# mrcabellom/InstantSfM

Hardware: AMD Instinct MI355X
Metric: LM-BA iterations/sec (+ final reprojection RMSE) (higher is better)
Workload: dtype f64

## Files before the change

include/insfm_ba_debug.h:

```cpp
#ifndef INSFM_BA_DEBUG_H
#define INSFM_BA_DEBUG_H

#include "insfm_ba.h"
#include "insfm_gp.h"

#ifdef __cplusplus
extern "C" {
#endif

int insfm_ba_debug_linearize(insfm_ba* h, const double* cam_params, const double* points);
int insfm_ba_debug_solve(insfm_ba* h, double f);
int64_t insfm_ba_debug_get(insfm_ba* h, int32_t which, double* host_out);
int insfm_ba_debug_time_kernel(insfm_ba* h, int32_t which, int32_t reps, double* us_per_launch);
int insfm_ba_debug_time_cgp(insfm_ba* h, int32_t reps, double* out);
int32_t insfm_ba_debug_stamps(insfm_ba* h, int64_t* host_out, int32_t max_steps);
int32_t insfm_ba_debug_clusters(const insfm_ba* h, int32_t* labels);
int64_t insfm_ba_nnzb(const insfm_ba* h);
int insfm_ba_debug_spd_inverse(int32_t m, const double* E, double* Einv, void* stream, int32_t reps,
                               double* us_per_inverse);

int insfm_gp_debug_linearize(insfm_ba* h, const double* positions, const double* points, const double* scales);
int64_t insfm_gp_debug_get_ds(insfm_ba* h, double* host_out);

int insfm_ba_cg_window(insfm_ba* h, void* ipc_handle);
int insfm_ba_cg_attach(insfm_ba* h, const void* handles);
int insfm_ba_cg_partition(const insfm_ba* h, int32_t* rows_begin_end);
int insfm_ba_debug_time_xchg(insfm_ba* h, int32_t reps, double* us);

#ifdef __cplusplus
}
#endif
#endif
```

instantsfm_amd/_capi.py:

```python
import ctypes
import os

_HERE = os.path.dirname(os.path.abspath(__file__))
LIB_PATH = os.path.join(_HERE, "_lib", "libinsfm_ba.so")

INSFM_BA_OK = 0
INSFM_BA_EINVAL = -22
INSFM_BA_ENOMEM = -12
INSFM_BA_EHIP = -100
INSFM_BA_ECOMM = -101
INSFM_BA_ESOLVER = -102

ALLREDUCE_FN = ctypes.CFUNCTYPE(ctypes.c_int, ctypes.c_void_p, ctypes.POINTER(ctypes.c_double), ctypes.c_int64)
ALLREDUCE_ASYNC_FN = ctypes.CFUNCTYPE(ctypes.c_int, ctypes.c_void_p, ctypes.POINTER(ctypes.c_double), ctypes.c_int64,
                                      ctypes.c_void_p)


class Desc(ctypes.Structure):
    _fields_ = [
        ("n_cams", ctypes.c_int32), ("n_points", ctypes.c_int32), ("n_obs", ctypes.c_int32),
        ("cam_model", ctypes.c_int32), ("optimize_poses", ctypes.c_int32), ("deterministic", ctypes.c_int32),
        ("huber_delta", ctypes.c_double),
        ("tr_radius", ctypes.c_double), ("tr_max", ctypes.c_double), ("tr_min", ctypes.c_double),
        ("tr_up", ctypes.c_double), ("tr_down", ctypes.c_double), ("tr_factor", ctypes.c_double),
        ("tr_high", ctypes.c_double), ("tr_low", ctypes.c_double),
        ("clamp_min", ctypes.c_double), ("clamp_max", ctypes.c_double),
        ("max_rejects", ctypes.c_int32), ("pcg_max_iter", ctypes.c_int32),
        ("pcg_tol", ctypes.c_double),
        ("world_size", ctypes.c_int32), ("rank", ctypes.c_int32),
        ("shard_point_begin", ctypes.c_int32), ("shard_point_end", ctypes.c_int32),
        ("allreduce", ALLREDUCE_FN), ("allreduce_ctx", ctypes.c_void_p),
        ("precond", ctypes.c_int32), ("cluster_size", ctypes.c_int32), ("schur_variant", ctypes.c_int32),
        ("allreduce_async", ALLREDUCE_ASYNC_FN), ("exchange_chunks", ctypes.c_int32),
    ]


class Stats(ctypes.Structure):
    _fields_ = [
        ("loss", ctypes.c_double), ("loss_before", ctypes.c_double), ("damping", ctypes.c_double),
        ("trials", ctypes.c_int32), ("rejects", ctypes.c_int32), ("pcg_iters_last", ctypes.c_int32),
        ("pcg_iters_total", ctypes.c_int32), ("solver_failed", ctypes.c_int32), ("cg_launches", ctypes.c_int32),
        ("time_ms", ctypes.c_double * 8), ("coarse_used", ctypes.c_int32),
    ]

    def as_dict(self):
        return dict(loss=self.loss, loss_before=self.loss_before, damping=self.damping, trials=self.trials,
                    rejects=self.rejects, pcg_iters=self.pcg_iters_last, pcg_total=self.pcg_iters_total,
                    failed=self.solver_failed, cg_launches=self.cg_launches, time_ms=list(self.time_ms),
                    coarse_used=self.coarse_used)


PUBLIC_SYMBOLS = ("insfm_build_info", "insfm_ba_default_desc", "insfm_ba_create", "insfm_ba_step", "insfm_ba_cost",
                  "insfm_ba_reset", "insfm_ba_destroy", "insfm_ba_last_error", "insfm_ba_exchange_count",
                  "insfm_ba_set_exchange", "insfm_ba_set_timing", "insfm_ba_release_cache",
                  "insfm_ba_set_ranks_per_device", "insfm_ba_cg_info", "insfm_ba_set_persistent_cg",
                  "insfm_ba_cg_fallbacks",
                  "insfm_gp_default_desc", "insfm_gp_create", "insfm_gp_step", "insfm_gp_cost",
                  "insfm_undistort", "insfm_filter_reproj_normalized", "insfm_filter_angle", "insfm_filter_tri_angle",
                  "insfm_filter_reproj_pixel", "insfm_reproj_candidates",
                  "insfm_tracks_establish", "insfm_covis_pairs", "insfm_pair_inliers")
DEBUG_SYMBOLS = ("insfm_ba_debug_linearize", "insfm_ba_debug_solve", "insfm_ba_debug_get", "insfm_ba_nnzb",
                 "insfm_ba_debug_time_kernel", "insfm_ba_debug_clusters", "insfm_ba_debug_spd_inverse",
                 "insfm_ba_debug_time_cgp", "insfm_ba_debug_stamps",
                 "insfm_gp_debug_linearize", "insfm_gp_debug_get_ds",
                 "insfm_ba_cg_window", "insfm_ba_cg_attach", "insfm_ba_cg_partition", "insfm_ba_debug_time_xchg")
SYMBOLS = PUBLIC_SYMBOLS + DEBUG_SYMBOLS

_lib = None


class BAError(RuntimeError):
    def __init__(self, code, msg):
        super().__init__(f"insfm_ba error {code}: {msg}")
        self.code = code


def build_info(L=None):
    L = L or load()
    L.insfm_build_info.argtypes = []
    L.insfm_build_info.restype = ctypes.c_char_p
    return L.insfm_build_info().decode()


def _check_provenance(L, path):
    from . import build as _b
    if not all(os.path.exists(p) for p in _b.SRCS + _b.HEADERS):
        return
    info = build_info(L)
    want = _b.source_hash()
    if f"src={want} " not in info + " ":
        raise RuntimeError(f"{path} was built from other sources ({info}; this tree hashes to src={want}): "
                           "rebuild it (python -c 'import __graft_entry__ as g; g.build()')")


def load(path=None):
    global _lib
    if _lib is not None:
        return _lib
    path = path or os.environ.get("INSFM_LIB") or LIB_PATH
    if not os.path.exists(path):
        raise RuntimeError(f"{path} not found: build the HIP extension first (python -c 'import __graft_entry__ as g; g.build()')")
    L = ctypes.CDLL(path)
    if not os.environ.get("INSFM_LIB"):
        _check_provenance(L, path)
    vp, dp = ctypes.c_void_p, ctypes.POINTER(ctypes.c_double)
    L.insfm_ba_default_desc.argtypes = [ctypes.POINTER(Desc)]
    L.insfm_ba_default_desc.restype = None
    L.insfm_ba_create.argtypes = [ctypes.POINTER(Desc), dp, ctypes.POINTER(ctypes.c_int32), ctypes.POINTER(ctypes.c_int32),
                                  dp, vp, ctypes.POINTER(vp)]
    L.insfm_ba_create.restype = ctypes.c_int
    L.insfm_ba_step.argtypes = [vp, vp, vp, ctypes.POINTER(Stats)]
    L.insfm_ba_step.restype = ctypes.c_int
    L.insfm_ba_cost.argtypes = [vp, vp, vp, dp, dp]
    L.insfm_ba_cost.restype = ctypes.c_int
    L.insfm_ba_reset.argtypes = [vp]
    L.insfm_ba_reset.restype = ctypes.c_int
    L.insfm_ba_destroy.argtypes = [vp]
    L.insfm_ba_destroy.restype = None
    L.insfm_ba_last_error.argtypes = [vp]
    L.insfm_ba_last_error.restype = ctypes.c_char_p
    L.insfm_ba_debug_linearize.argtypes = [vp, vp, vp]
    L.insfm_ba_debug_linearize.restype = ctypes.c_int
    L.insfm_ba_debug_solve.argtypes = [vp, ctypes.c_double]
    L.insfm_ba_debug_solve.restype = ctypes.c_int
    L.insfm_ba_debug_get.argtypes = [vp, ctypes.c_int32, dp]
    L.insfm_ba_debug_get.restype = ctypes.c_int64
    L.insfm_ba_nnzb.argtypes = [vp]
    L.insfm_ba_nnzb.restype = ctypes.c_int64
    L.insfm_ba_exchange_count.argtypes = [vp]
    L.insfm_ba_exchange_count.restype = ctypes.c_int64
    L.insfm_ba_set_exchange.argtypes = [vp, vp, ctypes.c_int64]
    L.insfm_ba_set_exchange.restype = ctypes.c_int
    L.insfm_ba_debug_time_kernel.argtypes = [vp, ctypes.c_int32, ctypes.c_int32, dp]
    L.insfm_ba_debug_time_kernel.restype = ctypes.c_int
    L.insfm_ba_debug_stamps.argtypes = [vp, ctypes.POINTER(ctypes.c_int64), ctypes.c_int32]
    L.insfm_ba_debug_stamps.restype = ctypes.c_int32
    L.insfm_ba_debug_time_cgp.argtypes = [vp, ctypes.c_int32, dp]
    L.insfm_ba_debug_time_cgp.restype = ctypes.c_int
    L.insfm_ba_set_timing.argtypes = [vp, ctypes.c_int32]
    L.insfm_ba_set_timing.restype = ctypes.c_int
    L.insfm_ba_debug_clusters.argtypes = [vp, ctypes.POINTER(ctypes.c_int32)]
    L.insfm_ba_debug_clusters.restype = ctypes.c_int32
    L.insfm_ba_debug_spd_inverse.argtypes = [ctypes.c_int32, vp, vp, vp, ctypes.c_int32, dp]
    L.insfm_ba_debug_spd_inverse.restype = ctypes.c_int
    L.insfm_ba_release_cache.argtypes = []
    L.insfm_ba_release_cache.restype = ctypes.c_int64
    L.insfm_ba_set_ranks_per_device.argtypes = [vp, ctypes.c_int32]
    L.insfm_ba_set_ranks_per_device.restype = ctypes.c_int
    L.insfm_ba_cg_info.argtypes = [vp, ctypes.POINTER(ctypes.c_int32)]
    L.insfm_ba_cg_info.restype = ctypes.c_int
    L.insfm_ba_set_persistent_cg.argtypes = [vp, ctypes.c_int32]
    L.insfm_ba_set_persistent_cg.restype = ctypes.c_int
    L.insfm_ba_cg_fallbacks.argtypes = [vp]
    L.insfm_ba_cg_fallbacks.restype = ctypes.c_int32
    L.insfm_ba_cg_window.argtypes = [vp, ctypes.c_char_p]
    L.insfm_ba_cg_window.restype = ctypes.c_int
    L.insfm_ba_cg_attach.argtypes = [vp, ctypes.c_char_p]
    L.insfm_ba_cg_attach.restype = ctypes.c_int
    L.insfm_ba_cg_partition.argtypes = [vp, ctypes.POINTER(ctypes.c_int32)]
    L.insfm_ba_cg_partition.restype = ctypes.c_int
    L.insfm_ba_debug_time_xchg.argtypes = [vp, ctypes.c_int32, dp]
    L.insfm_ba_debug_time_xchg.restype = ctypes.c_int
    ip = ctypes.POINTER(ctypes.c_int32)
    L.insfm_gp_default_desc.argtypes = [ctypes.POINTER(Desc)]
    L.insfm_gp_default_desc.restype = None
    L.insfm_gp_create.argtypes = [ctypes.POINTER(Desc), dp, ip, ip, dp, ip, vp, ctypes.POINTER(vp)]
    L.insfm_gp_create.restype = ctypes.c_int
    L.insfm_gp_step.argtypes = [vp, vp, vp, vp, ctypes.POINTER(Stats)]
    L.insfm_gp_step.restype = ctypes.c_int
    L.insfm_gp_cost.argtypes = [vp, vp, vp, vp, dp, dp]
    L.insfm_gp_cost.restype = ctypes.c_int
    L.insfm_gp_debug_linearize.argtypes = [vp, vp, vp, vp]
    L.insfm_gp_debug_linearize.restype = ctypes.c_int
    L.insfm_gp_debug_get_ds.argtypes = [vp, dp]
    L.insfm_gp_debug_get_ds.restype = ctypes.c_int64
    i64, f64, i32 = ctypes.c_int64, ctypes.c_double, ctypes.c_int32
    L.insfm_undistort.argtypes = [i64, vp, i32, vp, vp, vp, vp, vp]
    L.insfm_filter_reproj_normalized.argtypes = [i64, vp, vp, vp, vp, vp, vp, f64, vp, vp, vp]
    L.insfm_filter_angle.argtypes = [i64, vp, vp, vp, vp, vp, vp, f64, vp, vp]
    L.insfm_filter_tri_angle.argtypes = [i64, vp, vp, vp, vp, f64, vp, vp]
    L.insfm_filter_reproj_pixel.argtypes = [i64, vp, vp, vp, vp, i32, vp, vp, vp, vp, vp, f64, vp, vp, vp]
    L.insfm_reproj_candidates.argtypes = [i64, i32, vp, vp, vp, vp, i32, vp, vp, vp, f64, vp, vp, vp]
    L.insfm_tracks_establish.argtypes = [i64, vp, vp, i32, i64, vp, vp, f64, vp, vp, vp, vp, vp,
                                         ctypes.POINTER(ctypes.c_int64), vp]
    L.insfm_covis_pairs.argtypes = [i64, vp, vp, i32, i64, vp, vp, vp, vp, ctypes.POINTER(ctypes.c_int64), vp]
    L.insfm_covis_pairs.restype = ctypes.c_int
    L.insfm_pair_inliers.argtypes = [i64, vp, i64, vp, vp, i64, vp, i32, vp, i32, vp, vp, vp, vp, vp, vp, vp]
    L.insfm_pair_inliers.restype = ctypes.c_int
    for fn in ("insfm_tracks_establish", "insfm_undistort", "insfm_filter_reproj_normalized", "insfm_filter_angle", "insfm_filter_tri_angle",
               "insfm_filter_reproj_pixel", "insfm_reproj_candidates",
           "insfm_tracks_establish"):
        getattr(L, fn).restype = ctypes.c_int
    _lib = L
    return L


def default_desc():
    d = Desc()
    load().insfm_ba_default_desc(ctypes.byref(d))
    return d


def gp_default_desc():
    d = Desc()
    load().insfm_gp_default_desc(ctypes.byref(d))
    return d


def release_device_cache():
    return int(load().insfm_ba_release_cache())


def check(h, rc):
    if rc < 0:
        msg = load().insfm_ba_last_error(h).decode() if h else ""
        raise BAError(rc, msg)
    return rc
```

instantsfm_amd/csrc/ba_create.h:

```cpp
#pragma once
#include "ba_handle.h"
#include "cg_poll.h"
#include "create_plan.h"

namespace {

__global__ __launch_bounds__(kThreads) void k_derive_tracks(int Pl, const int* __restrict__ pt_ptr, const int* __restrict__ cam,
                                                            int* __restrict__ ptl, int* __restrict__ ustart) {
    const int p = blockIdx.x * kThreads + threadIdx.x;
    if (p >= Pl) return;
    const int b0 = pt_ptr[p], b1 = pt_ptr[p + 1];
    int u = b0, prev = -1;
    for (int o = b0; o < b1; ++o) {
        const int c = cam[o];
        if (c != prev) { u = o; prev = c; }
        ptl[o] = p;
        ustart[o] = u;
    }
}
__global__ __launch_bounds__(kThreads) void k_derive_cm(int Nl, const int* __restrict__ cam_obs, const int* __restrict__ ptl,
                                                        const int* __restrict__ ustart, const int* __restrict__ pt_ptr,
                                                        const double* __restrict__ uv, int4* __restrict__ sdesc,
                                                        int* __restrict__ cm_pt, double* __restrict__ cm_uv) {
    const int e = blockIdx.x * kThreads + threadIdx.x;
// ... 92 lines not shown
int upload_observations(insfm_ba* h, HostPool& pool, const double* obs, const double* cpar, const int32_t* sfree_in,
                        const TrackOrder& t, const CamMajor& cm) {
    const int C = h->C, Nl = h->Nl, Pl = h->Pl, kind = h->kind;
    const nivec<int>& lsrc = t.lsrc;
    int rc;
    if (kind == 1) {
        nivec<double> tl((size_t)3 * Nl);
        nivec<int> sl(Nl);
        pool.ranges(Nl, [&](int, long long a, long long b) {
            for (long long o = a; o < b; ++o) {
                for (int k = 0; k < 3; ++k) tl[3 * (size_t)o + k] = obs[3 * (size_t)lsrc[o] + k];
                sl[o] = sfree_in ? (sfree_in[lsrc[o]] != 0) : 1;
            }
        });
        if ((rc = upload(h, &h->trans, tl.data(), tl.size()))) return rc;
        if ((rc = upload(h, &h->sfree, sl.data(), sl.size()))) return rc;
        if ((rc = upload(h, &h->fcam, cpar, (size_t)C))) return rc;
        if ((rc = upload(h, &h->osrc, lsrc.data(), lsrc.size()))) return rc;
        h->osrc_host.assign(lsrc.begin(), lsrc.end());
        if ((rc = dd(h, &h->gobs, (size_t)Nl * kGO))) return rc;
        if ((rc = dd(h, &h->Up, (size_t)C * 9))) return rc;
        if ((rc = dd(h, &h->VY, (size_t)std::max(Pl, 1) * kVY))) return rc;
        if ((rc = dd(h, &h->gpc, (size_t)C * 3))) return rc;
        if ((rc = dd(h, &h->scl_cur, (size_t)std::max(Nl, 1)))) return rc;
        if ((rc = dd(h, &h->scl_new, (size_t)std::max(Nl, 1)))) return rc;
        if ((rc = dd(h, &h->ds, (size_t)std::max(Nl, 1)))) return rc;
    } else {
        nivec<double> uvl((size_t)2 * Nl);
        pool.ranges(Nl, [&](int, long long a, long long b) {
            for (long long o = a; o < b; ++o) {
                uvl[2 * (size_t)o] = obs[2 * (size_t)lsrc[o]];
                uvl[2 * (size_t)o + 1] = obs[2 * (size_t)lsrc[o] + 1];
            }
        });
        if ((rc = upload(h, &h->uv, uvl.data(), uvl.size()))) return rc;
        if ((rc = upload(h, &h->pp, cpar, (size_t)2 * C))) return rc;
    }
    if ((rc = upload(h, &h->cam, t.lcam.data(), t.lcam.size()))) return rc;
    if ((rc = upload(h, &h->pt_ptr, t.lptr.data(), t.lptr.size()))) return rc;
    if ((rc = upload(h, &h->cam_ptr, cm.cptr.data(), cm.cptr.size()))) return rc;
    if ((rc = upload(h, &h->cam_obs, cm.cobs.data(), cm.cobs.size()))) return rc;
    if ((rc = dalloc(h, (void**)&h->ptl, sizeof(int) * (size_t)std::max(Nl, 1)))) return rc;
    if ((rc = dalloc(h, (void**)&h->ustart, sizeof(int) * (size_t)std::max(Nl, 1)))) return rc;
    if ((rc = dalloc(h, (void**)&h->sdesc, sizeof(int4) * (size_t)std::max(Nl, 1)))) return rc;
    if (kind != 1) {
        if ((rc = dalloc(h, (void**)&h->cm_pt, sizeof(int) * (size_t)std::max(Nl, 1)))) return rc;
        if ((rc = dalloc(h, (void**)&h->cm_uv, sizeof(double) * 2 * (size_t)std::max(Nl, 1)))) return rc;
    }
    if (Pl > 0) k_derive_tracks<<<cdiv(Pl, kThreads), kThreads, 0, h->stream>>>(Pl, h->pt_ptr, h->cam, h->ptl, h->ustart);
    if (Nl > 0)
        k_derive_cm<<<cdiv(Nl, kThreads), kThreads, 0, h->stream>>>(Nl, h->cam_obs, h->ptl, h->ustart, h->pt_ptr,
                                                                    kind != 1 ? h->uv : nullptr, h->sdesc, h->cm_pt,
                                                                    h->cm_uv);
    return launch_err(h, "k_derive");
}

int device_pattern(insfm_ba* h, BlockPattern* out) {
    const int C = h->C;
    int rc;
    int *dcnt = nullptr, *doff = nullptr, *dnb = nullptr, *dwt = nullptr;
    const size_t lds = sizeof(int) * (size_t)C;
    std::vector<int> ulen(C), uoff(C + 1, 0);
    if ((rc = dalloc(h, (void**)&dcnt, sizeof(int) * (size_t)C))) return rc;
    if ((rc = dalloc(h, (void**)&doff, sizeof(int) * (size_t)(C + 1)))) return rc;
    hipError_t e = hipSuccess;
    {
        k_pattern<<<C, 256, lds, h->stream>>>(C, h->cam_ptr, h->cam_obs, h->ustart, h->ptl, h->pt_ptr, h->cam, dcnt,
                                              nullptr, nullptr, nullptr);
        e = hipGetLastError();
    }
    if (e == hipSuccess) e = hipMemcpyAsync(ulen.data(), dcnt, sizeof(int) * (size_t)C, hipMemcpyDeviceToHost, h->stream);
    if (e == hipSuccess) e = hipStreamSynchronize(h->stream);
    for (int i = 0; i < C && e == hipSuccess; ++i) uoff[i + 1] = uoff[i] + ulen[i];
    const int U = uoff[C];
    std::vector<int> unb(std::max(U, 1)), uwt(std::max(U, 1));
    if (e == hipSuccess && ((rc = dalloc(h, (void**)&dnb, sizeof(int) * (size_t)std::max(U, 1))) ||
                            (rc = dalloc(h, (void**)&dwt, sizeof(int) * (size_t)std::max(U, 1)))))
        return rc;
    if (e == hipSuccess) e = hipMemcpyAsync(doff, uoff.data(), sizeof(int) * (size_t)(C + 1), hipMemcpyHostToDevice, h->stream);
    if (e == hipSuccess) {
        k_pattern<<<C, 256, lds, h->stream>>>(C, h->cam_ptr, h->cam_obs, h->ustart, h->ptl, h->pt_ptr, h->cam, nullptr,
                                              doff, dnb, dwt);
        e = hipGetLastError();
    }
    if (e == hipSuccess && U > 0) e = hipMemcpyAsync(unb.data(), dnb, sizeof(int) * (size_t)U, hipMemcpyDeviceToHost, h->stream);
    if (e == hipSuccess && U > 0) e = hipMemcpyAsync(uwt.data(), dwt, sizeof(int) * (size_t)U, hipMemcpyDeviceToHost, h->stream);
    if (e == hipSuccess) e = hipStreamSynchronize(h->stream);
    if (e != hipSuccess) return create_err(h, INSFM_BA_EHIP, std::string("k_pattern: ") + hipGetErrorString(e));
    *out = plan_pattern_from_upper(C, ulen, uoff, unb, uwt);
    return 0;
}

int setup_exchange(insfm_ba* h, const std::vector<int>& rptr, const std::vector<Int4>& work) {
    ExchangeChunks x = plan_exchange(h->C, h->d.exchange_chunks, rptr, work);
    h->rptr_host = rptr;
    h->xr = std::move(x.xr);
    h->xw = std::move(x.xw);
    hipError_t e = hipStreamCreateWithFlags(&h->xstream, hipStreamNonBlocking);
    if (e == hipSuccess) e = hipEventCreateWithFlags(&h->ev_x, hipEventDisableTiming);
    if (e == hipSuccess) e = hipEventCreateWithFlags(&h->ev_xdone, hipEventDisableTiming);
    if (e != hipSuccess) return create_err(h, INSFM_BA_EHIP, std::string("exchange stream: ") + hipGetErrorString(e));
    return 0;
}

int setup_lin_stream(insfm_ba* h) {
    hipError_t e = helper_stream(1, 0, &h->aux);
    if (e == hipSuccess) e = hipEventCreateWithFlags(&h->ev_lin0, hipEventDisableTiming);
    if (e == hipSuccess) e = hipEventCreateWithFlags(&h->ev_lc, hipEventDisableTiming);
    if (e != hipSuccess) return create_err(h, INSFM_BA_EHIP, std::string("linearization stream: ") + hipGetErrorString(e));
    h->u_late = true;
    return 0;
}

int upload_structure(insfm_ba* h, const TrackOrder& t, const BlockPattern& pat, const LowerLists& low,
                     const NbrLists& nbr, const SchurWork& sw) {
    const int D = h->D;
    int rc;
    if (h->kind != 1) {
        const std::vector<int> lb = plan_lin_runs(h->Pl, t.lptr, kLinThreads);
        h->n_lin = (int)lb.size() - 1;
        if ((rc = upload(h, &h->lin_blk, lb.data(), lb.size()))) return rc;
    }
    if ((rc = upload(h, &h->row_ptr, pat.rptr.data(), pat.rptr.size()))) return rc;
    if ((rc = upload(h, &h->col, pat.cols.data(), pat.cols.size()))) return rc;
    if ((rc = upload(h, &h->blk_row, low.brow.data(), low.brow.size()))) return rc;
    if ((rc = upload(h, &h->nbr_ptr, nbr.nptr.data(), nbr.nptr.size()))) return rc;
    if ((rc = upload(h, &h->nbr_j, nbr.nj.data(), nbr.nj.size()))) return rc;
    if ((rc = upload(h, &h->pos_up, nbr.pup.data(), nbr.pup.size()))) return rc;
    h->pos_up_host = nbr.pup;
    if ((rc = upload(h, &h->pos_lo, nbr.plo.data(), nbr.plo.size()))) return rc;
    {
        const int DPd = D + (D & 1);
        const size_t snb = sizeof(double) * (size_t)std::max<int64_t>(h->n_nbr, 1) * D * DPd;
        if ((rc = dalloc(h, (void**)&h->Sn, snb))) return rc;
        if (hipMemsetAsync(h->Sn, 0, snb, h->stream) != hipSuccess) return create_err(h, INSFM_BA_EHIP, "Sn clear");
    }
    return upload_int4(h, &h->work, sw.work);
}

int alloc_numeric(insfm_ba* h) {
    const int C = h->C, D = h->D, Nl = h->Nl, Pl = h->Pl, kind = h->kind;
    const int maxit = h->d.pcg_max_iter;
    int rc;
    if ((rc = dd(h, &h->W, (size_t)Nl * D * 3 + 2))) return rc;
    if ((rc = dd(h, &h->V, (size_t)Pl * 6))) return rc;
    if ((rc = dd(h, &h->gp, (size_t)Pl * 3))) return rc;
    if ((rc = dd(h, &h->Vinv, (size_t)Pl * 6))) return rc;
    if ((rc = dd(h, &h->y, (size_t)Pl * 3))) return rc;
    if (kind == 0) {
        if ((rc = dd(h, &h->Rf, (size_t)Pl * 6))) return rc;
        if ((rc = dd(h, &h->Mp, (size_t)Pl * 6))) return rc;
    }
    if ((rc = dd(h, &h->dp, (size_t)Pl * 3))) return rc;
    h->xcount = (int64_t)h->nnzb * D * D + (int64_t)C * D + (int64_t)C * D * D + (int64_t)C * D + 8;
    if ((rc = dd(h, &h->xbuf, (size_t)h->xcount))) return rc;
    h->S = h->xbuf;
    h->b = h->S + (size_t)h->nnzb * D * D;
    h->U = h->b + (size_t)C * D;
    h->gc = h->U + (size_t)C * D * D;
    h->scal = h->gc + (size_t)C * D;
    if ((rc = dd(h, &h->Lf, (size_t)C * D * D))) return rc;
    if ((rc = dd(h, &h->Li, (size_t)C * D * D))) return rc;
    if ((rc = dd(h, &h->dc, (size_t)C * D))) return rc;
    h->cg_nwg = C;
    const size_t cd = (size_t)C * D;
    const size_t cgn = 8 * cd + 2 * 3 * (size_t)h->cg_nwg + 2 * ((size_t)maxit + 2) + 16;
    if ((rc = dd(h, &h->cgmem, cgn))) return rc;
    {
        double* m = h->cgmem;
        h->cg.r[0] = m; m += cd; h->cg.r[1] = m; m += cd;
        h->cg.w[0] = m; m += cd; h->cg.w[1] = m; m += cd;
        h->cg.s[0] = m; m += cd; h->cg.s[1] = m; m += cd;
        h->cg.p = m; m += cd; h->cg.x = m; m += cd;
        h->cg.part[0] = m; m += 3 * (size_t)h->cg_nwg; h->cg.part[1] = m; m += 3 * (size_t)h->cg_nwg;
        h->cg.hist = m; m += 2 * ((size_t)maxit + 2);
        h->cg.scal = m; m += 4;
    }
    if ((rc = dalloc(h, (void**)&h->cg.status, sizeof(int) * 4))) return rc;
    const int ST = h->stride;
    if ((rc = dd(h, &h->cams_cur, (size_t)C * ST))) return rc;
    if ((rc = dd(h, &h->cams_new, (size_t)C * ST))) return rc;
    if ((rc = dd(h, &h->pts_cur, (size_t)std::max(Pl, 1) * 3))) return rc;
    if ((rc = dd(h, &h->pts_new, (size_t)std::max(Pl, 1) * 3))) return rc;
    h->n_cost = std::max(1, cdiv(Nl, kind == 1 ? kThreads : kCostThreads));
    h->n_gp = std::max(1, cdiv(Pl, kThreads));
    h->n_gp_grp = std::max(1, cdiv((long long)Pl * kGPG, kThreads));
    if (kind == 1) h->n_gp = h->n_gp_grp;
    else h->n_gp = std::max(1, h->n_lin);
    h->n_gc = std::max(1, cdiv(C, kLinThreads));
    if ((rc = dd(h, &h->part_cost, 2 * (size_t)h->n_cost))) return rc;
    if ((rc = dd(h, &h->part_gp, (size_t)h->n_gp))) return rc;
    if ((rc = dd(h, &h->part_gc, (size_t)h->n_gc))) return rc;
    h->result = h->scal;
    return dalloc(h, (void**)&h->flags, sizeof(int) * 4);
}

int setup_host_sync(insfm_ba* h) {
    {
        hipError_t e = hipHostMalloc((void**)&h->host_res, 128, hipHostMallocDefault);
        if (e != hipSuccess) return create_err(h, INSFM_BA_ENOMEM, std::string("hipHostMalloc: ") + hipGetErrorString(e));
        void* pm = nullptr;
        if (hipHostMalloc(&pm, 16 * sizeof(double), hipHostMallocMapped) == hipSuccess) {
            void* dp = nullptr;
            if (hipHostGetDevicePointer(&dp, pm, 0) == hipSuccess) {
                h->pub_host = static_cast<double*>(pm);
                h->pub_dev = static_cast<double*>(dp);
                std::memset(pm, 0, 16 * sizeof(double));
            } else {
                (void)hipHostFree(pm);
            }
        }
    }
    for (auto& e : h->ev) {
        hipError_t x = hipEventCreate(&e);
        if (x != hipSuccess) return create_err(h, INSFM_BA_EHIP, std::string("hipEventCreate: ") + hipGetErrorString(x));
    }
    if (h->d.world_size > 1 || h->d.allreduce) {
        const hipError_t x = hipEventCreateWithFlags(&h->ev_pre, hipEventDisableTiming);
        if (x != hipSuccess) return create_err(h, INSFM_BA_EHIP, std::string("hipEventCreate: ") + hipGetErrorString(x));
    }
    {
        hipError_t e = hipMemsetAsync(h->part_gp, 0, sizeof(double) * h->n_gp, h->stream);
        if (e == hipSuccess) e = hipMemsetAsync(h->part_gc, 0, sizeof(double) * h->n_gc, h->stream);
        if (e == hipSuccess) e = hipMemsetAsync(h->flags, 0, sizeof(int) * 4, h->stream);
        if (e == hipSuccess) e = hipStreamSynchronize(h->stream);
        if (e != hipSuccess) return create_err(h, INSFM_BA_EHIP, std::string("init: ") + hipGetErrorString(e));
    }
    const bool det = h->d.deterministic != 0;
    for (const bool retry : {false, true})
        if (const SchurKernel k = schur_kernel(h->kind, h->D, det, retry))
            (void)hipFuncSetAttribute((const void*)k, hipFuncAttributeMaxDynamicSharedMemorySize, (int)h->schur_lds);
    if (h->kind == 1 && !det)
        (void)hipFuncSetAttribute((const void*)k_schur_gp<kSchurWaves, kGPSG>, hipFuncAttributeMaxDynamicSharedMemorySize,
                                  (int)h->schur_lds);
    return 0;
}

int upload_coarse_lists(insfm_ba* h, const CoarseLists& co) {
    TlBufs& tl = h->tl;
    int rc;
    int* ip = nullptr;
    if ((rc = upload(h, &ip, co.clp.data(), co.clp.size()))) return rc;
    tl.cl_ptr = ip;
    if ((rc = upload(h, &ip, co.clc.data(), co.clc.size()))) return rc;
    tl.cl_cams = ip;
    if ((rc = upload(h, &ip, co.cpos.data(), co.cpos.size()))) return rc;
    tl.cpos = ip;
    if ((rc = upload(h, &ip, co.alone.data(), co.alone.size()))) return rc;
    tl.alone = ip;
    if ((rc = upload(h, &ip, co.sperm.data(), co.sperm.size()))) return rc;
    tl.sperm = ip;
    if ((rc = upload(h, &ip, co.rsp.data(), co.rsp.size()))) return rc;
    tl.rseg_ptr = ip;
    if ((rc = upload(h, &ip, co.eptr.data(), co.eptr.size()))) return rc;
    tl.ered_ptr = ip;
    if ((rc = upload(h, &ip, co.eseg.data(), co.eseg.size()))) return rc;
    tl.ered_seg = ip;
    int4* sp = nullptr;
    if ((rc = upload_int4(h, &sp, co.segs))) return rc;
    tl.seg = sp;
    return 0;
}

int setup_two_level(insfm_ba* h, const Clusters& cl, const CoarseLists& co) {
    const int C = h->C, D = h->D, MC = D + 1, nc = cl.nc, m = nc * MC;
    const size_t cd = (size_t)C * D;
    const insfm_ba_desc* desc = &h->d;
    TlBufs& tl = h->tl;
    int rc;
    tl.nc = nc;
    tl.m = m;
    tl.maxmem = co.maxmem;
    const int ldE = gj_steps(m) * kGB;
    tl.ldE = ldE;
    if ((rc = upload_coarse_lists(h, co))) return rc;
    if ((rc = dd(h, &tl.u, cd))) return rc;
    if ((rc = dd(h, &tl.Zt, cd * MC))) return rc;
    if ((rc = dd(h, &tl.Ztc, cd * MC))) return rc;
    if ((rc = dd(h, &tl.vc, cd))) return rc;
    if ((rc = dd(h, &tl.Rc, (size_t)m))) return rc;
    if ((rc = dd(h, &tl.gd, 3 * (size_t)C))) return rc;
    {
        int* ip = nullptr;
        if ((rc = upload(h, &ip, cl.lab.data(), cl.lab.size()))) return rc;
        tl.clab = ip;
        tl.Racc = nullptr;
        tl.Gacc = nullptr;
        if (!desc->deterministic && desc->world_size <= 1 && !desc->allreduce) {
            if ((rc = hand(h, (void**)&tl.Racc, sizeof(double) * 3 * (size_t)m))) return rc;
            if ((rc = hand(h, (void**)&tl.Gacc, sizeof(double) * 3 * 3 * (size_t)nc))) return rc;
            if (hipMemsetAsync(tl.Racc, 0, sizeof(double) * 3 * (size_t)m, h->stream) != hipSuccess ||
                hipMemsetAsync(tl.Gacc, 0, sizeof(double) * 9 * (size_t)nc, h->stream) != hipSuccess)
                return create_err(h, INSFM_BA_EHIP, "Racc clear");
        }
    }
    if ((rc = dd(h, &tl.rowR, (size_t)C * MC + 2))) return rc;
    if ((rc = dd(h, &tl.Oseg, co.segs.size() * MC * MC))) return rc;
    {
        std::vector<double> eye((size_t)ldE * ldE, 0.0);
        for (int q = m; q < ldE; ++q) eye[(size_t)q * ldE + q] = 1.0;
        for (int sl = 0; sl < 2; ++sl) {
            if ((rc = upload(h, &h->Ebuf[sl], eye.data(), eye.size()))) return rc;
            if ((rc = dd(h, &h->Einvbuf[sl], (size_t)m * m))) return rc;
        }
    }
    if ((rc = dd(h, &h->gjW, (size_t)ldE * ldE))) return rc;
// ... 10 lines not shown
    int prio_lo = 0, prio_hi = 0;
    if (e == hipSuccess) e = hipDeviceGetStreamPriorityRange(&prio_lo, &prio_hi);
    const int side_prio = diag("side_hi") ? prio_hi : diag("side_normal") ? 0 : prio_lo;
    if (e == hipSuccess) e = helper_stream(0, side_prio, &h->side);
    if (e == hipSuccess) e = hipEventCreateWithFlags(&h->ev_E, hipEventDisableTiming);
    if (e == hipSuccess) e = hipEventCreateWithFlags(&h->ev_built, hipEventDisableTiming);
    for (int sl = 0; sl < 2 && e == hipSuccess; ++sl) e = hipEventCreateWithFlags(&h->ev_fact[sl], hipEventDisableTiming);
    if (e == hipSuccess) e = hipStreamSynchronize(h->stream);
    if (e != hipSuccess) return create_err(h, INSFM_BA_EHIP, std::string("two-level init: ") + hipGetErrorString(e));
    {
        const size_t fixed = sizeof(double) * ((size_t)MC * m + (size_t)m), budget = 144 * 1024;
        h->pc_rows = (int)std::min<size_t>((size_t)C, (budget - fixed) / (sizeof(double) * MC));
        h->pc_lds = fixed + sizeof(double) * (size_t)h->pc_rows * MC;
    }
    if (h->pc_lds > 150 * 1024)
        return create_err(h, INSFM_BA_EINVAL,
                          "two-level preconditioner: scene too connected for the LDS budget (use precond 0)");
    with_D(D, [&](auto dc_) -> int {
        constexpr int DV = decltype(dc_)::value;
        (void)hipFuncSetAttribute((const void*)k_tl_pc<DV>, hipFuncAttributeMaxDynamicSharedMemorySize,
                                  (int)h->pc_lds);
        return 0;
    });
    h->tlon = true;
    void* pm = nullptr;
    if (hipHostMalloc(&pm, sizeof(int) * 8, hipHostMallocMapped) == hipSuccess) {
        h->prog_host = static_cast<int*>(pm);
        void* dp = nullptr;
        if (hipHostGetDevicePointer(&dp, pm, 0) == hipSuccess) h->cg.prog = static_cast<int*>(dp);
        else { (void)hipHostFree(pm); h->prog_host = nullptr; }
    }
    return 0;
}

int setup_cgp(insfm_ba* h, const BlockPattern& pat, const LowerLists& low, const NbrLists& nbr, const CoarseLists& co) {
    const int C = h->C, D = h->D, MC = D + 1;
    const size_t cd = (size_t)C * D;
    TlBufs& tl = h->tl;
    int rc;
    const CgpFacts f = plan_cgp_facts(C, nbr, co, kCgpSegMax, diag("cgp128"));
    const int nb = f.nb, grid = (C + kCgpRows - 1) / kCgpRows;
    if (diag("create"))
        std::fprintf(stderr, "[insfm create] k_tl_cgp eligibility: D %d, atomic sums %d, progress %d, max row %d, "
                     "cluster order %d, max segments %d\n", D, tl.Racc != nullptr, h->prog_host != nullptr, f.maxlen,
                     (int)f.in_order, co.maxseg);
    const bool det = tl.Racc == nullptr || diag("cgp_det");
    const bool adef = h->d.precond == 2;
    if (!(D == 8 && h->prog_host && f.ok && !diag("no_cgp"))) return 0;
    int dev = 0, ncu = 0, per_cu = 0;
    hipError_t ce = hipGetDevice(&dev);
    if (ce == hipSuccess) ce = hipDeviceGetAttribute(&ncu, hipDeviceAttributeMultiprocessorCount, dev);
    if (ce == hipSuccess)
        ce = hipOccupancyMaxActiveBlocksPerMultiprocessor(&per_cu, (const void*)cgp_kernel(nb, det, adef), kCgpThreads, 0);
    if (!(ce == hipSuccess && per_cu >= 1 && grid <= ncu)) return 0;
    if ((rc = hand(h, (void**)&h->cgp_wx, sizeof(double) * 2 * cd))) return rc;
    if ((rc = hand(h, (void**)&h->cgp_yg, sizeof(unsigned long long) * 2 * kCoarseMax))) return rc;
    if (hipMemsetAsync(h->cgp_yg, 0, sizeof(unsigned long long) * 2 * kCoarseMax, h->stream) != hipSuccess)
        return create_err(h, INSFM_BA_EHIP, "cgp granules");
    if ((rc = hand(h, (void**)&h->cgp_sync, sizeof(unsigned) * kCgpSyncWords))) return rc;
    if (hipMemsetAsync(h->cgp_sync, 0, sizeof(unsigned) * kCgpSyncWords, h->stream) != hipSuccess)
        return create_err(h, INSFM_BA_EHIP, "cgp barrier words");
    if (diag("cgp_trace") && (rc = dd(h, &h->cgp_trace, kCgpTraceLen))) return rc;
    if ((rc = hand(h, (void**)&h->cgp_runs, sizeof(double) * 2 * 12 * (size_t)grid * kCgpRows))) return rc;
    {
        const std::vector<int> src = plan_cgp_src(pat.rptr, low, nbr, kCgpPadSlot);
        if ((rc = upload(h, &h->cgp_src, src.data(), src.size()))) return rc;
        if ((rc = dd(h, &tl.Gb, cd * MC))) return rc;
    }
    h->cgp_det = det;
    h->adef2 = adef;
    h->cgp_nb = nb;
    h->cgp_grid = grid;
    h->cgp_slots = per_cu * ncu;
    if (diag("create"))
        std::fprintf(stderr, "[insfm create] k_tl_cgp<%d>: %d workgroups, %d CUs, %d per CU\n", nb, grid, ncu, per_cu);
    return 0;
}

int create_impl(const insfm_ba_desc* desc, int kind, const double* obs, const int32_t* cam_idx, const int32_t* pt_idx,
                const double* cpar, const int32_t* sfree_in, void* stream, insfm_ba** out) {
    if (!desc || !out) return INSFM_BA_EINVAL;
    *out = nullptr;
    insfm_ba* h = new insfm_ba();
    h->d = *desc;
    h->kind = kind;
    h->stream = reinterpret_cast<hipStream_t>(stream);
    auto fail = [&](int rc, const std::string& msg) {
        if (!msg.empty()) h->err = msg;
        *out = h;
        return rc;
    };
    int rc;
    if ((rc = create_validate(h, desc, kind, obs, cam_idx, pt_idx, cpar))) return fail(rc, "");
    const int C = h->C, P = h->P, N = h->N, D = h->D;
    HostPool pool(host_pool_size());
    switch (plan_check_inputs(pool, C, P, N, cam_idx, pt_idx)) {
        case 1: return fail(INSFM_BA_EINVAL, "cam_idx out of range");
        case 2: return fail(INSFM_BA_EINVAL, "pt_idx out of range");
        case 3: return fail(INSFM_BA_EINVAL, "observations must be track-major (pt_idx nondecreasing)");
        default: break;
    }
    h->p0 = std::max(0, desc->shard_point_begin);
    h->p1 = desc->shard_point_end < 0 ? P : std::min(P, desc->shard_point_end);
    if (h->p1 < h->p0) return fail(INSFM_BA_EINVAL, "bad shard range");
    h->Pl = h->p1 - h->p0;
    static const bool ctrace = diag("create");
    const double ct0 = wall_seconds();
    auto tick = [&](const char* what) {
        if (ctrace) std::fprintf(stderr, "[insfm create] %-28s %8.1f ms\n", what, 1e3 * (wall_seconds() - ct0));
    };
    const TrackOrder trk = plan_track_order(pool, P, N, h->p0, h->p1, cam_idx, pt_idx);
    h->o0 = trk.o0;
    h->Nl = trk.Nl;
    const int o0 = h->o0, Nl = h->Nl, Pl = h->Pl;
    tick("local track order");
    const CamMajor cm = plan_cam_major(pool, C, trk, kSchurChunk * kSchurWaves * (64 / D));
    tick("camera-major lists");
    if ((rc = upload_observations(h, pool, obs, cpar, sfree_in, trk, cm))) return fail(rc, "");
    tick("uploads (observations)");
    static const bool pattern_host = diag("pattern_host");
    const bool gpu_pattern = !pattern_host && Pl == P && o0 == 0 && Nl == N && C <= kPatternMaxC && Nl > 0;
    BlockPattern pat;
    if (gpu_pattern) {
        if ((rc = device_pattern(h, &pat))) return fail(rc, "");
        pat.gcptr = cm.cptr;
    } else {
        pat = plan_pattern_host(pool, C, N, cam_idx, pt_idx, trk.gptr);
    }
    h->nnzb = pat.rptr[C];
    const LowerLists low = plan_lower(C, pat.rptr, pat.cols);
    if (gpu_pattern) plan_graph_from_upper(C, low, pat);
    tick("block pattern + covisibility");
    if (desc->precond < 0 || desc->precond > 2) return fail(INSFM_BA_EINVAL, "precond must be 0, 1 or 2");
    Clusters cl;
    if (desc->precond >= 1 && h->d.optimize_poses) cl = plan_clusters(pat.g, C, desc->cluster_size, D + 1, kCoarseMax);
    h->clab_host = cl.lab;
    tick("clusters");
    const NbrLists nbr = plan_nbr_lists(C, pat.rptr, pat.cols, low, cl.coarse_ok, cl.lab);
    h->nbr_stride = nbr.nbr_stride;
    h->n_nbr = nbr.n_nbr;
    tick("CG neighbour lists");
    const bool det_schur = desc->deterministic != 0;
    const SchurLimits lim{(size_t)kLdsBudget, det_schur ? (size_t)kLdsTargetDet : (size_t)kLdsTarget,
                          det_schur ? kDetWaves : kSchurWaves, schur_ws(D), schur_bs(D)};
    const SchurWork sw = plan_schur_work(C, D, lim, pat.gcptr, pat.rptr);
    if (!sw.fits) return fail(INSFM_BA_EINVAL, "too many cameras for LDS");
    h->nwork = (int)sw.work.size();
    h->max_chunk = sw.max_chunk;
    if (kind == 0 && desc->allreduce_async && (desc->world_size > 1 || desc->allreduce) && desc->exchange_chunks > 1 &&
        desc->optimize_poses && (rc = setup_exchange(h, pat.rptr, sw.work)))
        return fail(rc, "");
    h->schur_lds = sw.schur_lds;
    if (kind == 0 && desc->world_size <= 1 && !desc->allreduce && (rc = setup_lin_stream(h))) return fail(rc, "");
    if ((rc = upload_structure(h, trk, pat, low, nbr, sw))) return fail(rc, "");
    if ((rc = alloc_numeric(h))) return fail(rc, "");
    if ((rc = setup_host_sync(h))) return fail(rc, "");
    tick("uploads + allocations");
    if (cl.coarse_ok) {
        const CoarseLists co = plan_coarse(pool, C, cl.nc, cl.lab, nbr);
        tick("coarse segments");
        if ((rc = setup_two_level(h, cl, co))) return fail(rc, "");
        if ((rc = setup_cgp(h, pat, low, nbr, co))) return fail(rc, "");
    }
    tick("two-level setup (end)");
    if (kind == 0 && diag("stamps")) {
        const size_t n = (size_t)kStampSteps * kStKinds * 2;
        if ((rc = dalloc(h, (void**)&h->stamps, sizeof(long long) * n))) return fail(rc, "");
        if (hipMemsetAsync(h->stamps, 0, sizeof(long long) * n, h->stream) != hipSuccess) return fail(INSFM_BA_EHIP, "stamps");
    }
    h->damping = 1.0 / desc->tr_radius;
    h->down = desc->tr_down;
    *out = h;
    return INSFM_BA_OK;
}

}
```

instantsfm_amd/csrc/ba_debug_api.h:

```cpp
#pragma once
#include "ba_step.h"

extern "C" {

int32_t insfm_ba_debug_stamps(insfm_ba* h, int64_t* host_out, int32_t max_steps) {
    if (!h || !host_out || max_steps < 0) return INSFM_BA_EINVAL;
    if (!h->stamps) return 0;
    HIPCHK(hipStreamSynchronize(h->stream));
    const long long n = std::min<long long>(std::min<long long>(h->stamp_step, kStampSteps), max_steps);
    std::vector<long long> ring((size_t)kStampSteps * kStKinds * 2);
    HIPCHK(hipMemcpy(ring.data(), h->stamps, sizeof(long long) * ring.size(), hipMemcpyDeviceToHost));
    const long long first = h->stamp_step - n;
    for (long long q = 0; q < n; ++q) {
        const size_t src = (size_t)((first + q) % kStampSteps) * kStKinds * 2;
        std::memcpy(host_out + (size_t)q * kStKinds * 2, ring.data() + src, sizeof(long long) * kStKinds * 2);
    }
    return (int32_t)n;
}

int insfm_ba_cg_window(insfm_ba* h, void* ipc_handle) {
    if (!h || !ipc_handle) return INSFM_BA_EINVAL;
    if (h->kind != 0 || h->d.world_size < 2 || !h->tlon || h->tl.Racc || h->xwin) {
        h->err = "cg_window: needs a multi-rank two-level handle (precond 1) that has no window yet";
        return INSFM_BA_EINVAL;
// ... 58 lines not shown
    h->xq.assign(W + 1, C);
    h->xq[0] = 0;
    for (int r = 1; r < W; ++r) {
        const long long target = (long long)r * C / W;
        int best = bnd[0];
        for (int b : bnd)
            if (std::llabs(b - target) < std::llabs(best - target)) best = b;
        h->xq[r] = std::max(best, h->xq[r - 1]);
    }
    h->tl = tl_region(h, 1);
    HIPCHK(hipStreamSynchronize(h->stream));
    h->xpart = true;
    return INSFM_BA_OK;
}

int insfm_ba_debug_time_xchg(insfm_ba* h, int32_t reps, double* us) {
    if (!h || !us || !h->xpart || reps < 1) return INSFM_BA_EINVAL;
    HIPCHK(hipEventRecord(h->ev[kEvDebug], h->stream));
    for (int r = 0; r < reps; ++r) launch_xchg(h, 1);
    HIPCHK(hipEventRecord(h->ev[kEvDebugEnd], h->stream));
    HIPCHK(hipEventSynchronize(h->ev[kEvDebugEnd]));
    float ms = 0.0f;
    HIPCHK(hipEventElapsedTime(&ms, h->ev[kEvDebug], h->ev[kEvDebugEnd]));
    *us = 1e3 * ms / reps;
    return INSFM_BA_OK;
}

int insfm_ba_cg_partition(const insfm_ba* h, int32_t* rows_begin_end) {
    if (!h || !rows_begin_end || !h->xpart) return INSFM_BA_EINVAL;
    rows_begin_end[0] = h->xq[h->d.rank];
    rows_begin_end[1] = h->xq[h->d.rank + 1];
    return INSFM_BA_OK;
}

int insfm_ba_debug_linearize(insfm_ba* h, const double* cams, const double* pts) {
    if (!h || !cams || !pts || h->kind != 0) return INSFM_BA_EINVAL;
    cgp_drop_pending(h);
    h->keep_S = 1;
    HIPCHK(hipMemcpyAsync(h->cams_cur, cams, sizeof(double) * (size_t)h->C * h->stride, hipMemcpyDeviceToDevice, h->stream));
    if (h->Pl)
        HIPCHK(hipMemcpyAsync(h->pts_cur, pts + 3 * (size_t)h->p0, sizeof(double) * (size_t)h->Pl * 3, hipMemcpyDeviceToDevice,
                              h->stream));
    int rc = run_linearize(h, h->cams_cur, h->pts_cur);
    if (!rc) rc = lin_join(h);
    if (rc) return rc;
    HIPCHK(hipStreamSynchronize(h->stream));
    return 0;
}

int insfm_ba_debug_solve(insfm_ba* h, double f) {
    if (!h) return INSFM_BA_EINVAL;
    cgp_drop_pending(h);
    h->keep_S = 1;
    int it = run_solve(h, f, h->cams_cur, h->pts_cur, false);
    HIPCHK(hipStreamSynchronize(h->stream));
    return it;
}

int insfm_ba_debug_spd_inverse(int32_t m, const double* E, double* Einv, void* stream, int32_t reps,
                               double* us_per_inverse) {
    if (m < 1 || m > 4096 || !E || !Einv) return INSFM_BA_EINVAL;
    hipStream_t st = static_cast<hipStream_t>(stream);
    const int nB = gj_steps(m), ld = nB * kGB;
    const int n = reps > 0 && us_per_inverse ? reps : 1;
    std::vector<double> Eh((size_t)m * m), Ep((size_t)ld * ld, 0.0), dh(ld, 1.0);
    if (hipMemcpy(Eh.data(), E, sizeof(double) * Eh.size(), hipMemcpyDeviceToHost) != hipSuccess) return INSFM_BA_EHIP;
    for (int r = 0; r < ld; ++r)
        for (int c = 0; c < ld; ++c)
            Ep[(size_t)r * ld + c] = (r < m && c < m) ? Eh[(size_t)r * m + c] : (r == c ? 1.0 : 0.0);
    for (int r = 0; r < m; ++r) dh[r] = 1.0 / std::sqrt(Eh[(size_t)r * m + r]);
    double *Ew = nullptr, *Ww = nullptr, *dd = nullptr, *Pw = nullptr;
    int* ok = nullptr;
    hipEvent_t e0 = nullptr, e1 = nullptr;
    int okh = 0;
    float ms = 0.f;
    hipError_t e = hipMalloc(&Ew, sizeof(double) * (size_t)ld * ld);
    if (e == hipSuccess) e = hipMalloc(&Ww, sizeof(double) * (size_t)ld * ld);
    if (e == hipSuccess) e = hipMalloc(&dd, sizeof(double) * ld);
    if (e == hipSuccess) e = hipMalloc(&Pw, sizeof(double) * 2 * kGB * kGB);
    if (e == hipSuccess) e = hipMalloc(&ok, sizeof(int));
    if (e == hipSuccess) e = hipMemcpy(dd, dh.data(), sizeof(double) * ld, hipMemcpyHostToDevice);
    if (e == hipSuccess) e = hipEventCreate(&e0);
    if (e == hipSuccess) e = hipEventCreate(&e1);
    for (int r = 0; r < n && e == hipSuccess; ++r) {
        e = hipMemcpyAsync(Ew, Ep.data(), sizeof(double) * Ep.size(), hipMemcpyHostToDevice, st);
        if (e == hipSuccess) e = hipEventRecord(e0, st);
        for (int u = 0; u <= nB && e == hipSuccess; ++u) {
            launch_gj_unit(u, m, Ew, Ww, Pw, dd, Einv, ok, st);
            e = hipGetLastError();
        }
        if (e == hipSuccess) e = hipEventRecord(e1, st);
        if (e == hipSuccess) e = hipEventSynchronize(e1);
        float t = 0.f;
        if (e == hipSuccess) e = hipEventElapsedTime(&t, e0, e1);
        ms += t;
    }
    if (e == hipSuccess) e = hipMemcpy(&okh, ok, sizeof(int), hipMemcpyDeviceToHost);
    if (e0) (void)hipEventDestroy(e0);
    if (e1) (void)hipEventDestroy(e1);
    (void)hipFree(Ew); (void)hipFree(Ww); (void)hipFree(dd); (void)hipFree(Pw); (void)hipFree(ok);
    if (e != hipSuccess) return INSFM_BA_EHIP;
    if (us_per_inverse) *us_per_inverse = 1e3 * ms / n;
    return okh ? 1 : 0;
}

int insfm_ba_debug_time_kernel(insfm_ba* h, int32_t which, int32_t reps, double* us_per_launch) {
    if (!h || reps <= 0 || !us_per_launch || !h->d.optimize_poses) return INSFM_BA_EINVAL;
    HIPCHK(hipMemsetAsync(h->cg.status, 0, sizeof(int) * 4, h->stream));
    HIPCHK(hipMemsetAsync(h->cg.scal, 0, sizeof(double) * 4, h->stream));
    if (((which >= 2 && which <= 4) || which == 6 || which == 7) && !h->tlon) return INSFM_BA_EINVAL;
    if (which == 5 && (h->kind != 0 || !h->W)) return INSFM_BA_EINVAL;
    if (which < 0 || which > 7) return INSFM_BA_EINVAL;
    if (int rc0 = side_flush(h)) return rc0;
    if (int rc0 = lin_join(h)) return rc0;
    if (which != 1 && which != 5 && which != 6)
        if (int rc0 = ensure_sn(h)) return rc0;
    if (which == 2 && h->tl.Racc) {
        HIPCHK(hipMemsetAsync(h->tl.Racc + h->tl.m, 0, sizeof(double) * h->tl.m, h->stream));
        HIPCHK(hipMemsetAsync(h->tl.Gacc + 3 * h->tl.nc, 0, sizeof(double) * 3 * h->tl.nc, h->stream));
        with_D(h->D, [&](auto dc_) -> int {
            launch_pspmv<decltype(dc_)::value>(h, 0, h->C, h->tl);
            return 0;
        });
    }
    HIPCHK(hipEventRecord(h->ev[kEvDebug], h->stream));
    int rc = with_D(h->D, [&](auto dc_) -> int {
        constexpr int DV = decltype(dc_)::value;
        for (int r = 0; r < reps; ++r) {
            if (which == 2) {
                launch_tl_iter<DV>(h, 1, h->d.pcg_max_iter, 0.0);
            } else if (which == 3) {
                launch_pspmv<DV>(h, 1, h->C, h->tl);
            } else if (which == 4) {
                int rc2 = run_tl_basis(h, h->cams_cur, h->stream);
                if (!rc2) rc2 = run_tl_build(h, 0, h->stream);
                for (int u = 0; u <= gj_steps(h->tl.m) && !rc2; ++u) rc2 = run_tl_gj_unit(h, 0, u, h->stream);
                if (rc2) return rc2;
            } else if (which == 6) {
                for (int u = 1; u <= gj_steps(h->tl.m) + 1; ++u)
                    if (int rc2 = run_tl_gj_unit(h, 0, u - 1, h->stream)) return rc2;
            } else if (which == 7) {
                if (int rc2 = run_tl_build(h, 0, h->stream)) return rc2;
            } else if (which == 5 && h->kind == 0 && h->W) {
                with_model(h->model, [&](auto mc) -> int {
                    constexpr int M = decltype(mc)::value;
                    if (h->Pl > 0) launch_lin_points_w<M>(h, h->cams_new, h->pts_new, first_trial_prep(h));
                    return 0;
                });
            } else if (which == 0)
                k_cg_iter<DV><<<h->C, kCgThreads, 0, h->stream>>>(1, h->C, h->d.pcg_max_iter, 0.0, h->nbr_ptr, h->nbr_j, h->Sn,
                                                                h->Lf, h->cg);
            else {
                const int rc2 = launch_schur(h, 1.0, h->kind ? -1e308 : h->d.clamp_min,
                                             h->kind ? 1e308 : h->d.clamp_max, h->kind ? 1 : h->d.rank == 0, false);
                if (rc2) return rc2;
            }
        }
        return launch_err(h, "debug_time_kernel");
    });
    if (rc) return rc;
    HIPCHK(hipEventRecord(h->ev[kEvDebugEnd], h->stream));
    HIPCHK(hipEventSynchronize(h->ev[kEvDebugEnd]));
    float ms = 0.f;
    HIPCHK(hipEventElapsedTime(&ms, h->ev[kEvDebug], h->ev[kEvDebugEnd]));
    *us_per_launch = 1e3 * ms / reps;
    return INSFM_BA_OK;
}

int insfm_ba_debug_time_cgp(insfm_ba* h, int32_t reps, double* out) {
    if (!h || reps <= 0 || !out || !h->cgp_nb || h->kind != 0 || !h->prog_host) return INSFM_BA_EINVAL;
    cgp_drop_pending(h);
    if (int rc0 = side_flush(h)) return rc0;
    if (int rc0 = lin_join(h)) return rc0;
    double t_cg = 0.0, t_pc = 0.0, iters = 0.0;
    for (int r = 0; r < reps; ++r) {
        HIPCHK(hipMemsetAsync(h->cg.status, 0, sizeof(int) * 4, h->stream));
        if (int rc = refactor(h, h->last.basis_by_factor ? h->cams_new : nullptr)) return rc;
        if (!h->last.basis_by_factor)
            if (int rc = run_tl_basis(h, h->cams_new, h->stream)) return rc;
        volatile int* pg = h->prog_host;
        pg[0] = pg[1] = pg[2] = pg[3] = 0;
        std::atomic_thread_fence(std::memory_order_seq_cst);
        HIPCHK(hipEventRecord(h->ev[kEvDebug], h->stream));
        if (int rc2 = launch_tl_cgp(h, h->adef2, true)) return rc2;
        HIPCHK(hipEventRecord(h->ev[kEvDebugEnd], h->stream));
        HIPCHK(hipEventSynchronize(h->ev[kEvDebugEnd]));
        int st[3];
        if (int rc2 = cgp_complete(h, h->adef2, st)) return rc2;
        if (st[0] != 1) {
            h->err = "debug_time_cgp: the CG ended with status " + std::to_string(st[0]);
            return st[0] == 2 ? INSFM_BA_ESOLVER : INSFM_BA_EHIP;
        }
        float ms = 0.f;
        HIPCHK(hipEventElapsedTime(&ms, h->ev[kEvDebug], h->ev[kEvDebugEnd]));
        t_cg += ms;
        iters += st[1];
    }
    out[1] = t_pc;
    out[0] = 1e3 * t_cg / reps;
    out[2] = iters / reps;
    return INSFM_BA_OK;
}

int32_t insfm_ba_debug_clusters(const insfm_ba* h, int32_t* labels) {
    if (!h) return INSFM_BA_EINVAL;
    if (!h->tlon) return 0;
    if (labels) std::memcpy(labels, h->clab_host.data(), sizeof(int32_t) * h->C);
    return h->tl.nc;
}

int64_t insfm_ba_debug_get(insfm_ba* h, int32_t which, double* host) {
    if (!h || !host) return INSFM_BA_EINVAL;
    const size_t C = h->C, Pl = h->Pl, Nl = h->Nl, D = h->D;
    const double* src = nullptr;
    size_t n = 0;
    switch (which) {
        case 0: src = h->W; n = Nl * D * 3; break;
        case 1: src = h->V; n = Pl * 6; break;
        case 2: src = h->gp; n = Pl * 3; break;
        case 3: src = h->U; n = C * D * D; break;
        case 4: src = h->gc; n = C * D; break;
        case 5: {
            if (h->kind != 0 && h->kind != 1) return INSFM_BA_EINVAL;
            if (int rc0 = side_flush(h)) return rc0;
            if (int rc0 = ensure_sn(h)) return rc0;
            const size_t DP = D + (D & 1), nb = (size_t)h->nnzb;
            std::vector<double> sn((size_t)std::max<int64_t>(h->n_nbr, 1) * D * DP);
            if (h->n_nbr) HIPCHK(hipMemcpyAsync(sn.data(), h->Sn, sizeof(double) * h->n_nbr * D * DP, hipMemcpyDeviceToHost, h->stream));
            HIPCHK(hipStreamSynchronize(h->stream));
            std::vector<int> rp(C + 1);
            HIPCHK(hipMemcpy(rp.data(), h->row_ptr, sizeof(int) * (C + 1), hipMemcpyDeviceToHost));
            std::vector<char> diag_blk(nb, 0);
            for (size_t i = 0; i < C; ++i) diag_blk[rp[i]] = 1;
            for (size_t e = 0; e < nb; ++e)
                for (size_t a = 0; a < D; ++a)
                    for (size_t c = 0; c < D; ++c)
                        host[(e * D + a) * D + c] = diag_blk[e] ? (a == c ? 1.0 : 0.0)
                                                                : sn[((size_t)h->pos_up_host[e] * D + a) * DP + c];
            return (int64_t)(nb * D * D);
        }
        case 6: src = h->b; n = C * D; break;
        case 7: src = h->dc; n = C * D; break;
        case 8: src = h->dp; n = Pl * 3; break;
        case 9: src = h->tl.u; n = h->tlon ? C * D : 0; break;
        case 10: src = h->cg.w[0]; n = C * D; break;
        case 11: src = h->tl.rowR; n = h->tlon ? C * (D + 1) : 0; break;
        case 12: src = h->Einvbuf[0]; n = h->tlon ? (size_t)h->tl.m * h->tl.m : 0; break;
        case 13: src = h->Einvbuf[1]; n = h->tlon ? (size_t)h->tl.m * h->tl.m : 0; break;
        case 14: src = h->tl.gd; n = h->tlon ? 2 * C : 0; break;
        case 15: src = h->cg.r[0]; n = C * D; break;
        case 16: case 17: src = h->Ebuf[which - 16]; n = h->tlon ? (size_t)h->tl.ldE * h->tl.ldE : 0; break;
        default: return INSFM_BA_EINVAL;
    }
    if (int rc0 = side_flush(h)) return rc0;
    if (int rc0 = lin_join(h)) return rc0;
    if (n) HIPCHK(hipMemcpyAsync(host, src, n * sizeof(double), hipMemcpyDeviceToHost, h->stream));
    HIPCHK(hipStreamSynchronize(h->stream));
    return (int64_t)n;
}

int insfm_gp_debug_linearize(insfm_ba* h, const double* pos, const double* pts, const double* scales) {
    if (!h || !pos || !pts || !scales || h->kind != 1) return INSFM_BA_EINVAL;
    h->keep_S = 1;
    int rc = gp_io(h, 1, pos, pts, scales);
    if (rc) return rc;
    if ((rc = run_linearize(h, h->cams_cur, h->pts_cur))) return rc;
    HIPCHK(hipStreamSynchronize(h->stream));
    return 0;
}

int64_t insfm_gp_debug_get_ds(insfm_ba* h, double* host_out) {
    if (!h || !host_out || h->kind != 1) return INSFM_BA_EINVAL;
    std::vector<double> loc(h->Nl);
    if (h->Nl) HIPCHK(hipMemcpyAsync(loc.data(), h->ds, sizeof(double) * h->Nl, hipMemcpyDeviceToHost, h->stream));
    HIPCHK(hipStreamSynchronize(h->stream));
    std::memset(host_out, 0, sizeof(double) * (size_t)h->N);
    for (int o = 0; o < h->Nl; ++o) host_out[h->osrc_host[o]] = loc[o];
    return h->N;
}

}
```

instantsfm_amd/csrc/ba_handle.h:

```cpp
#pragma once
#include <hip/hip_runtime.h>

#include <algorithm>
#include <cstdint>
#include <cstdlib>
#include <cstring>
#include <map>
#include <mutex>
#include <string>
#include <type_traits>
#include <unordered_map>
#include <utility>
#include <vector>

#include "../../include/insfm_ba.h"
#include "ba_common.h"
#include "ba_twolevel.h"
#include "solve_policy.h"

struct SolveCarry {
    long long tl_solves = 0;
    bool tl_fresh = false;
    bool sn_valid = false;
    bool built_pending = false;
    bool lin_pending = false;
    bool flags_dirty = false;
    bool prep_valid = false;
    double prep_f = 0.0;
    bool chain_oseg = false;
    bool cgp_pending = false;
    bool cgp_lost = false;
    unsigned cgp_epochs = 0;
    unsigned cgp_tag = 1;
    int last_cg_iters = 16;
};

struct insfm_ba {
    insfm_ba_desc d{};
    int model = 0, ni = 0, D = 0, stride = 0;
    int C = 0, P = 0, N = 0;
    int p0 = 0, p1 = 0, Pl = 0, o0 = 0, Nl = 0;
    hipStream_t stream = nullptr;
    std::string err;
    double *uv = nullptr, *pp = nullptr;
    int *cam = nullptr, *ptl = nullptr, *pt_ptr = nullptr, *cam_ptr = nullptr, *cam_obs = nullptr;
    int *row_ptr = nullptr, *col = nullptr, *blk_row = nullptr, *ustart = nullptr;
    int *nbr_ptr = nullptr, *nbr_j = nullptr, *pos_up = nullptr, *pos_lo = nullptr;
    int4* sdesc = nullptr;
    int* cm_pt = nullptr;
    int* lin_blk = nullptr;
    int n_lin = 0;
    double* cm_uv = nullptr;
    double* Sn = nullptr;
    int64_t n_nbr = 0;
    int nbr_stride = 0;
    int keep_S = 0;
    std::vector<int> pos_up_host;
    int4* work = nullptr;
    int nwork = 0, nnzb = 0, max_chunk = 0;
    size_t schur_lds = 0;
    double *W = nullptr, *V = nullptr, *gp = nullptr, *Vinv = nullptr, *y = nullptr, *dp = nullptr;
    double *Rf = nullptr, *Mp = nullptr;
    double *xbuf = nullptr;
    double *S = nullptr, *b = nullptr, *U = nullptr, *gc = nullptr, *scal = nullptr;
    int64_t xcount = 0;
    double *Lf = nullptr, *Li = nullptr, *dc = nullptr;
    double* cgmem = nullptr;
    CgBufs cg{};
    int cg_nwg = 0;
    double *cams_cur = nullptr, *cams_new = nullptr, *pts_cur = nullptr, *pts_new = nullptr;
    bool ext_cur = false;
    bool trial_copied = false;
    double *part_cost = nullptr, *part_gp = nullptr, *part_gc = nullptr;
    int n_cost = 0, n_gp = 0, n_gc = 0;
    int n_gp_grp = 0;
    double* result = nullptr;
    int* flags = nullptr;
    double* host_res = nullptr;
    int* prog_host = nullptr;
    double* pub_host = nullptr;
    double* pub_dev = nullptr;
    unsigned pub_seq = 0;
    std::vector<void*> allocs;
    double damping = 0.0, down = 0.0, loss = 0.0;
    bool have_loss = false;
    SolveCarry ss;
    insfm::SolvePlan last;
    hipEvent_t ev[18]{};
    bool chain_timed[2]{};
    bool timing = false;
    double tms[8]{};
    int cg_launches = 0;
    bool want_timing = false;
    bool tlon = false;
    TlBufs tl{};
    std::vector<int> clab_host;
    size_t pc_lds = 0;
    int pc_rows = 0;
    int cgp_nb = 0, cgp_grid = 0;
    bool cgp_det = false;
    bool adef2 = false;
    int adef2_fallbacks = 0;
    double* cgp_runs = nullptr;
    int* cgp_src = nullptr;
    long long* stamps = nullptr;
    long long stamp_step = 0;
    int cgp_slots = 0;
    double* cgp_trace = nullptr;
    bool xpart = false;
    double* xwin = nullptr;
    size_t xwin_bytes = 0;
    long long xoff_region[2]{}, xoff_xg = 0, xoff_flags = 0;
    std::vector<void*> xopened;
    double** xbases = nullptr;
    unsigned** xpflags = nullptr;
    unsigned* xcnt = nullptr;
    std::vector<int> xq;
    double* cgp_wx = nullptr;
    unsigned long long* cgp_yg = nullptr;
    unsigned* cgp_sync = nullptr;
    double *Ebuf[2]{}, *Einvbuf[2]{};
    double* gjW = nullptr;
    double* gjP = nullptr;
    int* okbuf = nullptr;
    hipStream_t side = nullptr;
    hipEvent_t ev_E = nullptr, ev_built = nullptr, ev_fact[2]{};
    std::vector<int> xw, xr, rptr_host;
    hipStream_t xstream = nullptr;
    bool u_late = false;
    hipStream_t aux = nullptr;
    hipEvent_t ev_lin0 = nullptr, ev_lc = nullptr;
    hipEvent_t ev_x = nullptr, ev_xdone = nullptr;
    hipEvent_t ev_pre = nullptr;
    int coarse_used = 0;
    int kind = 0;
    double *trans = nullptr, *fcam = nullptr, *gobs = nullptr, *Up = nullptr, *gpc = nullptr, *VY = nullptr;
    int *sfree = nullptr, *osrc = nullptr;
    double *scl_cur = nullptr, *scl_new = nullptr, *ds = nullptr;
    std::vector<int> osrc_host;
    std::vector<std::pair<const char*, double>> hmarks;
};

namespace {

#define HIPCHK(expr)                                                                              \
    do {                                                                                          \
        hipError_t e_ = (expr);                                                                   \
        if (e_ != hipSuccess) {                                                                   \
            h->err = std::string(#expr) + " failed: " + hipGetErrorString(e_);                    \
            return INSFM_BA_EHIP;                                                                 \
        }                                                                                         \
    } while (0)

bool diag(const char* name) {
    static const std::string v = [] { const char* e = std::getenv("INSFM_DIAG"); return std::string(e ? e : ""); }();
    const size_t n = std::strlen(name);
    for (size_t a = 0; a <= v.size();) {
        size_t b = v.find(',', a);
        if (b == std::string::npos) b = v.size();
        if (b - a == n && v.compare(a, n, name) == 0) return true;
        a = b + 1;
    }
    return false;
}

struct DeviceCache {
    struct Buf {
        size_t bytes;
        int dev;
        bool uc;
    };
    std::mutex m;
    std::map<std::pair<int, size_t>, std::vector<void*>> free;
    size_t bytes = 0;
    std::unordered_map<void*, Buf> info;
};
DeviceCache& device_cache() {
    static DeviceCache* c = new DeviceCache();
    return *c;
}
size_t device_cache_cap() {
    static const size_t v = [] {
        const char* e = std::getenv("INSFM_DEVICE_CACHE_MB");
        return (size_t)(e ? std::max(0LL, std::atoll(e)) : 4096LL) << 20;
    }();
    return v;
}

size_t release_cache() {
    DeviceCache& c = device_cache();
    std::vector<std::pair<void*, int>> drop;
    size_t n = 0;
    {
        std::lock_guard<std::mutex> lk(c.m);
        for (auto& kv : c.free)
            for (void* q : kv.second) {
                drop.emplace_back(q, kv.first.first / 2);
                c.info.erase(q);
            }
        c.free.clear();
        n = c.bytes;
        c.bytes = 0;
    }
    int cur = 0;
    (void)hipGetDevice(&cur);
    for (auto& d : drop) {
        if (d.second != cur) (void)hipSetDevice(d.second);
        (void)hipFree(d.first);
        if (d.second != cur) (void)hipSetDevice(cur);
    }
    (void)hipGetLastError();
    return n;
}

std::mutex& stream_pool_mutex() {
// ... 158 lines not shown
```

instantsfm_amd/csrc/ba_lin.h:

```cpp
#pragma once
#include "ba_common.h"
#include "ba_device.h"

namespace {

constexpr int kLinThreads = 128;

struct PointPrep {
    double f = 1.0, cmin = 0.0, cmax = 0.0;
    double* Vinv = nullptr;
    double* y = nullptr;
    double* R = nullptr;
    int* flags = nullptr;
    int* status = nullptr;
};
__device__ __forceinline__ void point_prep_first(int p, const double V[6], const double g[3], const PointPrep& a,
                                                 double Ri[6]) {
    double s[6];
#pragma unroll
    for (int k = 0; k < 6; ++k) s[k] = V[k];
    s[0] = clampd(s[0], a.cmin, a.cmax) * a.f;
    s[3] = clampd(s[3], a.cmin, a.cmax) * a.f;
    s[5] = clampd(s[5], a.cmin, a.cmax) * a.f;
    double o[6], R[6];
    if (!spd3_factor(s, o, R, Ri)) {
        atomicOr(a.flags, 1);
#pragma unroll
        for (int k = 0; k < 6; ++k) o[k] = R[k] = Ri[k] = 0.0;
    }
#pragma unroll
    for (int k = 0; k < 6; ++k) a.Vinv[6 * (size_t)p + k] = o[k];
    if (a.R) {
#pragma unroll
        for (int k = 0; k < 6; ++k) a.R[6 * (size_t)p + k] = R[k];
        a.y[3 * (size_t)p + 0] = Ri[0] * g[0];
        a.y[3 * (size_t)p + 1] = Ri[1] * g[0] + Ri[3] * g[1];
        a.y[3 * (size_t)p + 2] = Ri[2] * g[0] + Ri[4] * g[1] + Ri[5] * g[2];
    } else {
        a.y[3 * (size_t)p + 0] = o[0] * g[0] + o[1] * g[1] + o[2] * g[2];
        a.y[3 * (size_t)p + 1] = o[1] * g[0] + o[3] * g[1] + o[4] * g[2];
        a.y[3 * (size_t)p + 2] = o[2] * g[0] + o[4] * g[1] + o[5] * g[2];
    }
}

template <int M>
__device__ __forceinline__ void lin_obs(int o, const int* __restrict__ cam, const int* __restrict__ ptl,
                                        const double* __restrict__ uv, const double* __restrict__ pp,
                                        const double* __restrict__ cams, const double* __restrict__ pts, double delta,
                                        double cv[9], double w[3 * kD<M>]) {
    constexpr int D = kD<M>, ST = kStride<M>;
    const int c = cam[o], p = ptl[o];
    const double X[3] = {pts[3 * (size_t)p], pts[3 * (size_t)p + 1], pts[3 * (size_t)p + 2]};
    const double2 z = reinterpret_cast<const double2*>(uv)[o];
    const double uvo[2] = {z.x, z.y};
    const double ppc[2] = {pp[2 * c], pp[2 * c + 1]};
    double r[2], Jc[2][D], Jp[2][3];
    eval_obs<M, true>(cams + (size_t)c * ST, X, ppc, uvo, r, Jc, Jp);
    const double sw = huber_weight_sqrt(r[0] * r[0] + r[1] * r[1], delta);
    r[0] *= sw; r[1] *= sw;
#pragma unroll
    for (int a = 0; a < D; ++a) { Jc[0][a] *= sw; Jc[1][a] *= sw; }
#pragma unroll
    for (int k = 0; k < 3; ++k) { Jp[0][k] *= sw; Jp[1][k] *= sw; }
    cv[0] = Jp[0][0] * Jp[0][0] + Jp[1][0] * Jp[1][0];
    cv[1] = Jp[0][0] * Jp[0][1] + Jp[1][0] * Jp[1][1];
    cv[2] = Jp[0][0] * Jp[0][2] + Jp[1][0] * Jp[1][2];
    cv[3] = Jp[0][1] * Jp[0][1] + Jp[1][1] * Jp[1][1];
    cv[4] = Jp[0][1] * Jp[0][2] + Jp[1][1] * Jp[1][2];
    cv[5] = Jp[0][2] * Jp[0][2] + Jp[1][2] * Jp[1][2];
#pragma unroll
    for (int k = 0; k < 3; ++k) cv[6 + k] = Jp[0][k] * r[0] + Jp[1][k] * r[1];
#pragma unroll
    for (int a = 0; a < D; ++a)
#pragma unroll
        for (int k = 0; k < 3; ++k) w[k * D + a] = Jc[0][a] * Jp[0][k] + Jc[1][a] * Jp[1][k];
}

template <int D>
__device__ __forceinline__ void y_from_w(double w[3 * D], const double Ri[6]) {
#pragma unroll
    for (int a = 0; a < D; ++a) {
        const double w0 = w[a], w1 = w[D + a], w2 = w[2 * D + a];
        w[a] = w0 * Ri[0];
        w[D + a] = w0 * Ri[1] + w1 * Ri[3];
        w[2 * D + a] = w0 * Ri[2] + w1 * Ri[4] + w2 * Ri[5];
    }
}

template <int WR, int WRP>
__device__ __forceinline__ void store_records(const double* wst, double* __restrict__ Y, int base, int n) {
    const int t = threadIdx.x;
    if constexpr ((WR & 1) == 0) {
        double2* dst = reinterpret_cast<double2*>(Y + (size_t)base * WR);
        for (int k2 = t; k2 < n * (WR / 2); k2 += kLinThreads) {
            const int k = 2 * k2, rec = k / WR, e = k - rec * WR;
            const double* src = wst + rec * WRP + e;
            typedef double nt_d2 __attribute__((ext_vector_type(2)));
            nt_d2 v2 = {src[0], src[1]};
            __builtin_nontemporal_store(v2, reinterpret_cast<nt_d2*>(dst + k2));
        }
    } else {
        double* dst = Y + (size_t)base * WR;
        for (int k = t; k < n * WR; k += kLinThreads) dst[k] = wst[(k / WR) * WRP + k % WR];
    }
}

template <int M>
__global__ __launch_bounds__(kLinThreads) void k_lin_points(const int* __restrict__ blk, const int* __restrict__ pt_ptr,
                                                         const int* __restrict__ cam, const int* __restrict__ ptl,
                                                         const double* __restrict__ uv, const double* __restrict__ pp,
                                                         const double* __restrict__ cams, const double* __restrict__ pts,
                                                         double delta, double* __restrict__ Y, double* __restrict__ V,
                                                         double* __restrict__ gp, PointPrep pp1, long long* stp) {
    constexpr int D = kD<M>, WR = 3 * D, WRP = WR | 1;
    static_assert(WRP >= 9, "the V / g terms reuse a record staging row");
    const StampScope stamp_(stp);
    __shared__ double wst[kLinThreads * WRP];
    const int t = threadIdx.x;
    const int tb = blk[blockIdx.x], te = blk[blockIdx.x + 1];
    const int ob = pt_ptr[tb], oe = pt_ptr[te];
    const bool one = oe - ob <= kLinThreads;
    double Vs[6] = {0, 0, 0, 0, 0, 0}, g[3] = {0, 0, 0};
    const int tr = tb + t;
    const int tlo = tr < te ? pt_ptr[tr] : 0, thi = tr < te ? pt_ptr[tr + 1] : 0;
    double w[WR];
    for (int base = ob; base < oe; base += kLinThreads) {
        const int o = base + t;
        double cv[9];
        if (o < oe) {
            lin_obs<M>(o, cam, ptl, uv, pp, cams, pts, delta, cv, w);
#pragma unroll
            for (int k = 0; k < 9; ++k) wst[(size_t)t * 9 + k] = cv[k];
        }
        __syncthreads();
        if (tr < te) {
            const int lo = max(tlo, base), hi = min(thi, base + kLinThreads);
            for (int q = lo; q < hi; ++q) {
                const double* cq = wst + (size_t)(q - base) * 9;
#pragma unroll
                for (int k = 0; k < 6; ++k) Vs[k] += cq[k];
#pragma unroll
                for (int k = 0; k < 3; ++k) g[k] -= cq[6 + k];
            }
        }
        __syncthreads();
    }
    double Ri[6];
    if (tr < te) {
#pragma unroll
        for (int k = 0; k < 6; ++k) V[6 * (size_t)tr + k] = Vs[k];
#pragma unroll
        for (int k = 0; k < 3; ++k) gp[3 * (size_t)tr + k] = g[k];
        point_prep_first(tr, Vs, g, pp1, Ri);
        if (Y) {
#pragma unroll
            for (int k = 0; k < 6; ++k) wst[(size_t)t * 6 + k] = Ri[k];
        }
    }
    if (blockIdx.x == 0 && threadIdx.x < 4) pp1.status[threadIdx.x] = 0;
    if (!Y) return;
    __syncthreads();
    if (one) {
        const int o = ob + t;
        if (o < oe) {
            const double* rq = wst + (size_t)(ptl[o] - tb) * 6;
            double r6[6];
#pragma unroll
            for (int k = 0; k < 6; ++k) r6[k] = rq[k];
            y_from_w<D>(w, r6);
        }
        __syncthreads();
        if (o < oe) {
#pragma unroll
            for (int a = 0; a < D; ++a)
#pragma unroll
                for (int k = 0; k < 3; ++k) wst[(size_t)t * WRP + k * D + a] = w[k * D + a];
        }
        __syncthreads();
        store_records<WR, WRP>(wst, Y, ob, oe - ob);
        return;
    }
    double r6[6];
#pragma unroll
    for (int k = 0; k < 6; ++k) r6[k] = wst[k];
    __syncthreads();
    for (int base = ob; base < oe; base += kLinThreads) {
        const int o = base + t;
        if (o < oe) {
            double cv[9];
            lin_obs<M>(o, cam, ptl, uv, pp, cams, pts, delta, cv, w);
            y_from_w<D>(w, r6);
#pragma unroll
            for (int a = 0; a < D; ++a)
#pragma unroll
                for (int k = 0; k < 3; ++k) wst[(size_t)t * WRP + k * D + a] = w[k * D + a];
        }
        __syncthreads();
        store_records<WR, WRP>(wst, Y, base, min(kLinThreads, oe - base));
        __syncthreads();
    }
}

template <int M>
__global__ __launch_bounds__(kThreads) void k_lin_cams(const int* __restrict__ cam_ptr, const int* __restrict__ cm_pt,
                                                       const double* __restrict__ cm_uv, const double* __restrict__ pp,
                                                       const double* __restrict__ cams, const double* __restrict__ pts,
                                                       double delta, double* __restrict__ U, double* __restrict__ gc) {
    constexpr int D = kD<M>, ST = kStride<M>;
    constexpr int RW = 2 * D + 2;
    constexpr int E = D * D + D;
    constexpr int EPT = (E + kThreads - 1) / kThreads;
    extern __shared__ __attribute__((aligned(16))) double sh[];
    const int c = blockIdx.x, t = threadIdx.x;
    const int eb = cam_ptr[c], ee = cam_ptr[c + 1];
    const double2* uv2 = reinterpret_cast<const double2*>(cm_uv);
    double camv[ST];
#pragma unroll
    for (int k = 0; k < ST; ++k) camv[k] = cams[(size_t)c * ST + k];
    const double ppc[2] = {pp[2 * c], pp[2 * c + 1]};
    double acc[EPT];
#pragma unroll
    for (int m = 0; m < EPT; ++m) acc[m] = 0.0;
    double X[3] = {0.0, 0.0, 0.0};
    double2 z = make_double2(0.0, 0.0), zn = z, znn = z;
    int pn = 0, pnn = 0;
    {
        const int e0 = eb + t, e1 = e0 + kThreads;
        if (e0 < ee) {
            const int p0 = cm_pt[e0];
            z = uv2[e0];
            X[0] = pts[3 * (size_t)p0]; X[1] = pts[3 * (size_t)p0 + 1]; X[2] = pts[3 * (size_t)p0 + 2];
        }
        if (e1 < ee) { pn = cm_pt[e1]; zn = uv2[e1]; }
    }
    for (int base = eb; base < ee; base += kThreads) {
        const int e = base + t;
        const bool has = e < ee, hn = e + kThreads < ee, hnn = e + 2 * kThreads < ee;
        double Xn[3] = {0.0, 0.0, 0.0};
        if (hn) { Xn[0] = pts[3 * (size_t)pn]; Xn[1] = pts[3 * (size_t)pn + 1]; Xn[2] = pts[3 * (size_t)pn + 2]; }
        if (hnn) { pnn = cm_pt[e + 2 * kThreads]; znn = uv2[e + 2 * kThreads]; }
        double* row = sh + (size_t)t * RW;
        if (has) {
            const double uvo[2] = {z.x, z.y};
            double r[2], Jc[2][D], Jp[2][3];
            eval_obs<M, true>(camv, X, ppc, uvo, r, Jc, Jp);
            const double sw = huber_weight_sqrt(r[0] * r[0] + r[1] * r[1], delta);
#pragma unroll
            for (int a = 0; a < D; ++a) { row[a] = Jc[0][a] * sw; row[D + a] = Jc[1][a] * sw; }
            row[2 * D] = r[0] * sw;
            row[2 * D + 1] = r[1] * sw;
        }
        __syncthreads();
        const int n = min(kThreads, ee - base);
#pragma unroll
        for (int m = 0; m < EPT; ++m) {
            const int ent = t + m * kThreads;
            if (ent < D * D) {
                const int a = ent / D, b = ent % D;
                double s = acc[m];
                for (int i = 0; i < n; ++i) {
                    const double* rw = sh + (size_t)i * RW;
                    s += rw[a] * rw[b] + rw[D + a] * rw[D + b];
                }
                acc[m] = s;
            } else if (ent < E) {
                const int a = ent - D * D;
                double s = acc[m];
                for (int i = 0; i < n; ++i) {
                    const double* rw = sh + (size_t)i * RW;
                    s -= rw[a] * rw[2 * D] + rw[D + a] * rw[2 * D + 1];
                }
                acc[m] = s;
            }
        }
        __syncthreads();
        X[0] = Xn[0]; X[1] = Xn[1]; X[2] = Xn[2];
        z = zn; pn = pnn; zn = znn;
    }
#pragma unroll
    for (int m = 0; m < EPT; ++m) {
        const int ent = t + m * kThreads;
        if (ent < D * D) U[(size_t)c * D * D + ent] = acc[m];
        else if (ent < E) gc[(size_t)c * D + (ent - D * D)] = acc[m];
    }
}

#ifndef LIN_CAMS_NT
#define LIN_CAMS_NT 128
#endif
template <int M, int NT = LIN_CAMS_NT>
__global__ __launch_bounds__(NT) void k_lin_cams_reg(const int* __restrict__ cam_ptr, const int* __restrict__ cm_pt,
                                                           const double* __restrict__ cm_uv, const double* __restrict__ pp,
                                                           const double* __restrict__ cams, const double* __restrict__ pts,
                                                           double delta, double* __restrict__ U, double* __restrict__ gc) {
    constexpr int D = kD<M>, ST = kStride<M>, NU = D * (D + 1) / 2, NE = NU + D;
    static_assert(D <= 9, "register accumulation is sized for D <= 9");
    constexpr int NW = NT / 64;
    __shared__ double red[NW][NE];
    const int c = blockIdx.x, t = threadIdx.x, lane = t & 63, wv = t >> 6;
    const int eb = cam_ptr[c], ee = cam_ptr[c + 1];
    const double2* uv2 = reinterpret_cast<const double2*>(cm_uv);
    double camv[ST];
#pragma unroll
    for (int k = 0; k < ST; ++k) camv[k] = cams[(size_t)c * ST + k];
    const double ppc[2] = {pp[2 * c], pp[2 * c + 1]};
    double acc[NE];
#pragma unroll
    for (int m = 0; m < NE; ++m) acc[m] = 0.0;
    double X[3] = {0.0, 0.0, 0.0};
    double2 z = make_double2(0.0, 0.0), zn = z, znn = z;
    int pn = 0, pnn = 0;
    {
        const int e0 = eb + t, e1 = e0 + NT;
        if (e0 < ee) {
            const int p0 = cm_pt[e0];
            z = uv2[e0];
            X[0] = pts[3 * (size_t)p0]; X[1] = pts[3 * (size_t)p0 + 1]; X[2] = pts[3 * (size_t)p0 + 2];
        }
        if (e1 < ee) { pn = cm_pt[e1]; zn = uv2[e1]; }
    }
    for (int e = eb + t; e < ee; e += NT) {
        const bool hn = e + NT < ee, hnn = e + 2 * NT < ee;
        double Xn[3] = {0.0, 0.0, 0.0};
        if (hn) { Xn[0] = pts[3 * (size_t)pn]; Xn[1] = pts[3 * (size_t)pn + 1]; Xn[2] = pts[3 * (size_t)pn + 2]; }
        if (hnn) { pnn = cm_pt[e + 2 * NT]; znn = uv2[e + 2 * NT]; }
        const double uvo[2] = {z.x, z.y};
        double r[2], Jc[2][D], Jp[2][3];
        eval_obs<M, true>(camv, X, ppc, uvo, r, Jc, Jp);
        const double sw = huber_weight_sqrt(r[0] * r[0] + r[1] * r[1], delta);
#pragma unroll
        for (int a = 0; a < D; ++a) { Jc[0][a] *= sw; Jc[1][a] *= sw; }
        r[0] *= sw; r[1] *= sw;
        int m = 0;
#pragma unroll
        for (int a = 0; a < D; ++a)
#pragma unroll
            for (int b = a; b < D; ++b, ++m) acc[m] += Jc[0][a] * Jc[0][b] + Jc[1][a] * Jc[1][b];
#pragma unroll
        for (int a = 0; a < D; ++a) acc[NU + a] -= Jc[0][a] * r[0] + Jc[1][a] * r[1];
        X[0] = Xn[0]; X[1] = Xn[1]; X[2] = Xn[2];
        z = zn; pn = pnn; zn = znn;
    }
#pragma unroll
    for (int m = 0; m < NE; ++m) {
        const double v = wave_sum(acc[m]);
        if (lane == 0) red[wv][m] = v;
    }
    __syncthreads();
    for (int m = t; m < NE; m += NT) {
        double s = red[0][m];
#pragma unroll
        for (int w = 1; w < NW; ++w) s += red[w][m];
        if (m < NU) {
            int a = 0, rem = m;
            while (rem >= D - a) { rem -= D - a; ++a; }
            const int b = a + rem;
            U[(size_t)c * D * D + a * D + b] = s;
            U[(size_t)c * D * D + b * D + a] = s;
        } else {
            gc[(size_t)c * D + (m - NU)] = s;
        }
    }
}

__global__ __launch_bounds__(kThreads) void k_point_prep(int Pl, const double* __restrict__ V, const double* __restrict__ gp,
                                                         double f, double cmin, double cmax, double* __restrict__ Vinv,
                                                         double* __restrict__ y, int* __restrict__ flags,
                                                         int* __restrict__ status, const double* __restrict__ R,
                                                         double* __restrict__ Mp) {
    const int p = blockIdx.x * kThreads + threadIdx.x;
    if (blockIdx.x == 0 && threadIdx.x < 4) status[threadIdx.x] = 0;
    if (p >= Pl) return;
    double s[6];
#pragma unroll
    for (int k = 0; k < 6; ++k) s[k] = V[6 * (size_t)p + k];
    s[0] = clampd(s[0], cmin, cmax) * f;
    s[3] = clampd(s[3], cmin, cmax) * f;
    s[5] = clampd(s[5], cmin, cmax) * f;
    double o[6];
    if (!spd3_inverse(s, o)) {
        atomicOr(flags, 1);
#pragma unroll
        for (int k = 0; k < 6; ++k) o[k] = 0.0;
    }
#pragma unroll
    for (int k = 0; k < 6; ++k) Vinv[6 * (size_t)p + k] = o[k];
    const double g0 = gp[3 * (size_t)p], g1 = gp[3 * (size_t)p + 1], g2 = gp[3 * (size_t)p + 2];
    const double y0 = o[0] * g0 + o[1] * g1 + o[2] * g2;
    const double y1 = o[1] * g0 + o[3] * g1 + o[4] * g2;
    const double y2 = o[2] * g0 + o[4] * g1 + o[5] * g2;
    if (!R) {
        y[3 * (size_t)p + 0] = y0;
        y[3 * (size_t)p + 1] = y1;
        y[3 * (size_t)p + 2] = y2;
        return;
    }
    const double* r = R + 6 * (size_t)p;
    const double r00 = r[0], r10 = r[1], r20 = r[2], r11 = r[3], r21 = r[4], r22 = r[5];
    const double Rm[3][3] = {{r00, 0.0, 0.0}, {r10, r11, 0.0}, {r20, r21, r22}};
    const double O[3][3] = {{o[0], o[1], o[2]}, {o[1], o[3], o[4]}, {o[2], o[4], o[5]}};
    double T[3][3];
#pragma unroll
    for (int a = 0; a < 3; ++a)
#pragma unroll
        for (int c = 0; c < 3; ++c) T[a][c] = O[a][0] * Rm[0][c] + O[a][1] * Rm[1][c] + O[a][2] * Rm[2][c];
    double Mq[3][3];
#pragma unroll
    for (int a = 0; a < 3; ++a)
#pragma unroll
        for (int c = 0; c < 3; ++c) Mq[a][c] = Rm[0][a] * T[0][c] + Rm[1][a] * T[1][c] + Rm[2][a] * T[2][c];
    double* mo = Mp + 6 * (size_t)p;
    mo[0] = Mq[0][0]; mo[1] = Mq[0][1]; mo[2] = Mq[0][2]; mo[3] = Mq[1][1]; mo[4] = Mq[1][2]; mo[5] = Mq[2][2];
    y[3 * (size_t)p + 0] = r00 * y0 + r10 * y1 + r20 * y2;
    y[3 * (size_t)p + 1] = r11 * y1 + r21 * y2;
    y[3 * (size_t)p + 2] = r22 * y2;
}

}
```

instantsfm_amd/csrc/ba_pcg.h:

```cpp
#pragma once
#include "ba_cgp.h"
#include "ba_common.h"
#include "ba_device.h"
#include "ba_twolevel.h"

namespace {

template <int D>
__device__ __forceinline__ void factor_camera(int i, int lane, const int* __restrict__ row_ptr, double* __restrict__ S,
                                              double* __restrict__ b, double* __restrict__ Lf, double* __restrict__ Li,
                                              CgBufs& cg, const double* __restrict__ Ul, const double* __restrict__ gcl,
                                              double f, double cmin, double cmax, double (&a)[D], double (&x)[D],
                                              double& r0out, bool& okout) {
    constexpr int DD = D * D;
    const int rl = min(lane, D - 1);
    double* blk = S + (size_t)row_ptr[i] * DD;
#pragma unroll
    for (int c = 0; c < D; ++c) a[c] = blk[rl * D + c];
    double bl = b[(size_t)i * D + rl];
    if (Ul) {
        const double* Ui = Ul + (size_t)i * DD + rl * D;
#pragma unroll
        for (int c = 0; c < D; ++c) {
            double u = Ui[c];
            if (c == rl) u = clampd(u, cmin, cmax) * f;
            a[c] += u;
        }
        bl = gcl[(size_t)i * D + rl] + bl;
        if (lane < D) {
#pragma unroll
            for (int c = 0; c < D; ++c) blk[rl * D + c] = a[c];
            b[(size_t)i * D + rl] = bl;
        }
    }
    bool ok = true;
#pragma unroll
    for (int j = 0; j < D; ++j) {
        double piv = readlane_d(a[j], j);
        if (!(piv > 0.0)) { ok = false; piv = 1.0; }
        const double ljj = sqrt(piv);
        const double lrj = (lane == j) ? ljj : ((lane > j) ? a[j] / ljj : 0.0);
        a[j] = lrj;
#pragma unroll
        for (int c = j + 1; c < D; ++c) {
            const double lcj = readlane_d(lrj, c);
            if (lane >= c) a[c] -= lrj * lcj;
        }
    }
#pragma unroll
    for (int c = 0; c < D; ++c)
        if (c > lane) a[c] = 0.0;
#pragma unroll
    for (int r = 0; r < D; ++r) {
        double s = 0.0;
#pragma unroll
        for (int k = 0; k < r; ++k) s -= readlane_d(a[k], r) * x[k];
        x[r] = (r >= lane) ? ((r == lane) ? 1.0 / readlane_d(a[r], r) : s / readlane_d(a[r], r)) : 0.0;
    }
    if (!ok && lane == 0) atomicMax(cg.status, 2);
    if (lane < D) {
#pragma unroll
        for (int c = 0; c < D; ++c) {
            Lf[(size_t)i * DD + lane * D + c] = a[c];
            Li[(size_t)i * DD + c * D + lane] = ok ? x[c] : 0.0;
        }
    }
    double r0 = 0.0;
#pragma unroll
    for (int aa = 0; aa < D; ++aa) {
        double sacc = 0.0;
#pragma unroll
        for (int k = 0; k <= aa; ++k) sacc += readlane_d(x[aa], k) * readlane_d(bl, k);
        if (lane == aa) r0 = sacc;
    }
    if (lane < D) {
        const size_t idx = (size_t)i * D + lane;
        cg.r[0][idx] = ok ? r0 : 0.0;
        cg.r[1][idx] = 0.0;
        cg.w[0][idx] = 0.0; cg.w[1][idx] = 0.0;
        cg.s[0][idx] = 0.0; cg.s[1][idx] = 0.0;
        cg.p[idx] = 0.0; cg.x[idx] = 0.0;
    }
    okout = ok;
    r0out = ok ? r0 : 0.0;
}

template <int D>
__global__ __launch_bounds__(kThreads) void k_cg_factor(int C, const int* __restrict__ row_ptr, double* __restrict__ S,
                                                        double* __restrict__ b, double* __restrict__ Lf,
                                                        double* __restrict__ Li, CgBufs cg, const double* __restrict__ Ul,
                                                        const double* __restrict__ gcl, double f, double cmin, double cmax,
                                                        long long* stp = nullptr) {
    const StampScope stamp_(stp);
    const int lane = threadIdx.x & 63, wv = threadIdx.x >> 6;
    const int i = blockIdx.x * kWaves + wv;
    if (i >= C) return;
    double a[D], x[D], r0;
    bool ok;
    factor_camera<D>(i, lane, row_ptr, S, b, Lf, Li, cg, Ul, gcl, f, cmin, cmax, a, x, r0, ok);
}

template <int D>
__global__ __launch_bounds__(kThreads) void k_cg_factor_basis(int C, const int* __restrict__ row_ptr, double* __restrict__ S,
                                                              double* __restrict__ b, double* __restrict__ Lf,
                                                              double* __restrict__ Li, CgBufs cg,
                                                              const double* __restrict__ Ul, const double* __restrict__ gcl,
                                                              double f, double cmin, double cmax,
                                                              const double* __restrict__ cams, TlBufs tl,
                                                              double* __restrict__ runs, long long* stp = nullptr) {
    static_assert(kWaves == kCgpRows, "k_cg_factor_basis's workgroups are k_tl_cgp's");
    const StampScope stamp_(stp);
    constexpr int MC = D + 1, ST = D + 1;
    __shared__ double prt[kWaves][MC];
    __shared__ int pcl[kWaves];
    const int lane = threadIdx.x & 63, wv = threadIdx.x >> 6;
    const int pos = blockIdx.x * kWaves + wv;
    const bool has = pos < C;
    const int i = has ? tl.cl_cams[pos] : 0;
    double rr = 0.0;
    if (has) {
        double a[D], x[D], r0;
        bool ok;
        factor_camera<D>(i, lane, row_ptr, S, b, Lf, Li, cg, Ul, gcl, f, cmin, cmax, a, x, r0, ok);
        const int k = min(lane, MC - 1);
        double col[D];
        basis_column<D>(k, cams + (size_t)i * ST, tl.alone[i] != 0, col);
        const bool st = lane < MC;
        const int cp = tl.cpos[i];
#pragma unroll
        for (int aa = 0; aa < D; ++aa) {
            double sz = 0.0;
#pragma unroll
            for (int l = aa; l < D; ++l) sz += readlane_d(a[aa], l) * col[l];
            if (st) {
                tl.Zt[((size_t)i * D + aa) * MC + k] = sz;
                if (tl.Gb) tl.Gb[((size_t)i * D + aa) * MC + k] = col[aa];
                tl.Ztc[((size_t)cp * D + aa) * MC + k] = sz;
            }
            rr += sz * readlane_d(r0, aa);
        }
        if (st) tl.rowR[(size_t)cp * MC + k] = rr;
        if (lane < D) tl.vc[(size_t)cp * D + lane] = r0;
    }
    if (lane < MC) prt[wv][lane] = rr;
    if (lane == 0) pcl[wv] = has ? tl.clab[i] : -1;
    __syncthreads();
    if (has && (wv == 0 || pcl[wv - 1] != pcl[wv]) && lane < MC) {
        double v = prt[wv][lane];
        for (int r2 = wv + 1; r2 < kWaves && pcl[r2] == pcl[wv]; ++r2) v += prt[r2][lane];
        runs[(size_t)pos * 12 + 3 + lane] = v;
    }
}

__host__ __device__ constexpr int scale_nb(int D) { return D * D <= 64 ? 4 : (D * D <= 144 ? 2 : 1); }
template <int D>
__global__ __launch_bounds__(kThreads) void k_cg_scale(int nnzb, const int* __restrict__ blk_row, const int* __restrict__ col,
                                                       const int* __restrict__ row_ptr, const int* __restrict__ pos_up,
                                                       const int* __restrict__ pos_lo, const double* __restrict__ Li,
                                                       double* __restrict__ S, double* __restrict__ Sn, int keep_S) {
    constexpr int DD = D * D;
    constexpr int DP = D + (D & 1);
    constexpr int NB = scale_nb(D);
    constexpr int UL = (DD + 63) / 64;
    __shared__ double T[kWaves][DD];
    __shared__ double Sb[kWaves][NB][DD];
    __shared__ double La[kWaves][NB][DD];
    __shared__ double Lb[kWaves][NB][DD];
    const int lane = threadIdx.x & 63, wv = threadIdx.x >> 6;
    const int e0 = (blockIdx.x * kWaves + wv) * NB;
    if (e0 >= nnzb) return;
    int ei[NB], ii[NB], jj[NB];
#pragma unroll
    for (int u = 0; u < NB; ++u) {
        ei[u] = min(e0 + u, nnzb - 1);
        ii[u] = blk_row[ei[u]];
        jj[u] = col[ei[u]];
    }
    double sv[NB][UL], av[NB][UL], bv[NB][UL];
#pragma unroll
    for (int u = 0; u < NB; ++u)
#pragma unroll
        for (int q = 0; q < UL; ++q) {
            const int k = min(lane + 64 * q, DD - 1);
            sv[u][q] = S[(size_t)ei[u] * DD + k];
            av[u][q] = Li[(size_t)ii[u] * DD + k];
            bv[u][q] = Li[(size_t)jj[u] * DD + k];
        }
#pragma unroll
    for (int u = 0; u < NB; ++u)
#pragma unroll
        for (int q = 0; q < UL; ++q) {
            const int k = lane + 64 * q;
            if (k < DD) { Sb[wv][u][k] = sv[u][q]; La[wv][u][k] = av[u][q]; Lb[wv][u][k] = bv[u][q]; }
        }
    __builtin_amdgcn_wave_barrier();
    __builtin_amdgcn_fence(__ATOMIC_SEQ_CST, "wavefront");
#pragma unroll
    for (int u = 0; u < NB; ++u) {
        const int e = e0 + u;
        if (e >= nnzb) break;
        const int i = ii[u];
        double* blk = S + (size_t)e * DD;
        if (e == row_ptr[i]) {
            if (keep_S)
                for (int k = lane; k < DD; k += 64) blk[k] = (k / D == k % D) ? 1.0 : 0.0;
            continue;
        }
        for (int k = lane; k < DD; k += 64) {
            const int a = k / D, bb = k % D;
            double s = 0.0;
            for (int m = 0; m <= a; ++m) s += La[wv][u][a * D + m] * Sb[wv][u][m * D + bb];
            T[wv][k] = s;
        }
        __builtin_amdgcn_wave_barrier();
        __builtin_amdgcn_fence(__ATOMIC_SEQ_CST, "wavefront");
        double* up = Sn + (size_t)pos_up[e] * D * DP;
        double* lo = Sn + (size_t)pos_lo[e] * D * DP;
        for (int k = lane; k < D * DP; k += 64) {
            const int a = k / DP, bb = k % DP;
            double v = 0.0;
            if (bb < D) {
                for (int m = 0; m <= bb; ++m) v += T[wv][a * D + m] * Lb[wv][u][bb * D + m];
                if (keep_S) blk[a * D + bb] = v;
                Sb[wv][u][a * D + bb] = v;
            }
            up[k] = v;
        }
        __builtin_amdgcn_wave_barrier();
        __builtin_amdgcn_fence(__ATOMIC_SEQ_CST, "wavefront");
        for (int k = lane; k < D * DP; k += 64) {
            const int a = k / DP, bb = k % DP;
            lo[k] = (bb < D) ? Sb[wv][u][bb * D + a] : 0.0;
        }
        __builtin_amdgcn_wave_barrier();
        __builtin_amdgcn_fence(__ATOMIC_SEQ_CST, "wavefront");
    }
}

__global__ __launch_bounds__(64) void k_cg_dots(int it, int C, int maxit, double tol2_rel, CgBufs cg) {
    const int lane = threadIdx.x;
    if (cg.status[0] != 0) return;
    const int i = it - 1;
    const double* P0 = cg.part[it & 1 ? 0 : 1];
    const double* P1 = P0 + C;
    const double* P2 = P1 + C;
    double g0 = 0.0, g1 = 0.0, g2 = 0.0;
    for (int base = lane; base < C; base += 64 * 16) {
        double a0[16], a1[16], a2[16];
#pragma unroll
        for (int u = 0; u < 16; ++u) {
            const int k = base + 64 * u;
            const bool ok = k < C;
            a0[u] = ok ? P0[k] : 0.0;
            a1[u] = ok ? P1[k] : 0.0;
            a2[u] = ok ? P2[k] : 0.0;
        }
#pragma unroll
        for (int u = 0; u < 16; ++u) { g0 += a0[u]; g1 += a1[u]; g2 += a2[u]; }
    }
    g0 = wave_sum(g0); g1 = wave_sum(g1); g2 = wave_sum(g2);
    const double h_alpha = (i >= 1) ? cg.hist[2 * (i - 1)] : 1.0;
    const double h_gam = (i >= 1) ? cg.hist[2 * (i - 1) + 1] : 1.0;
    const double h_bb = cg.hist[2 * (maxit + 1)];
    if (lane == 0) {
        const double gam = g0, del = g1, rho = g2;
        const double bb = (i == 0) ? rho : h_bb;
        double flag = 0.0, al = 0.0, be = 0.0;
        if (rho <= tol2_rel * bb || i >= maxit) {
            flag = 1.0;
            cg.status[0] = 1; cg.status[1] = i;
        } else {
            double den;
            if (i == 0) { be = 0.0; den = del; }
            else {
                be = gam / h_gam;
                den = del - be * gam / h_alpha;
// ... 173 lines not shown
```

instantsfm_amd/csrc/ba_schur.h:

```cpp
#pragma once
#include "ba_common.h"
#include "ba_device.h"

namespace {

constexpr int kLdsBudget = 96 * 1024;
#ifndef SCHUR_LDS_KB
#define SCHUR_LDS_KB 96
#endif
constexpr int kLdsTarget = SCHUR_LDS_KB * 1024;
#ifndef SCHUR_LDS_KB_DET
#define SCHUR_LDS_KB_DET 52
#endif
constexpr int kLdsTargetDet = SCHUR_LDS_KB_DET * 1024;
#ifndef INSFM_SCHUR_WAVES
#define INSFM_SCHUR_WAVES 8
#endif
constexpr int kSchurWaves = INSFM_SCHUR_WAVES;
constexpr int kSchurChunk = 4;
#ifndef SCHUR_MINW
#define SCHUR_MINW 1
#endif
#ifndef SCHUR_UP
#define SCHUR_UP 10
#endif
#ifndef SCHUR_DET_WAVES
#define SCHUR_DET_WAVES 4
#endif
#ifndef SCHUR_UP_DET
#define SCHUR_UP_DET 5
#endif
#define SCHUR_DET_ORD (SCHUR_DET_WAVES > 1)
constexpr int kDetWaves = SCHUR_DET_WAVES;

__host__ __device__ constexpr int schur_bs(int D) { return D * D + ((D * D) % 16 == 0 ? 8 : 0); }
__host__ __device__ constexpr int schur_ws(int D) { return D * 4 + 1; }

template <int D, bool GPW>
__device__ __forceinline__ void load_wcol(const double* __restrict__ W, int o, int cb, double& w0, double& w1, double& w2) {
    if constexpr (GPW) {
        const double4 r = reinterpret_cast<const double4*>(W)[o];
        const double uc = cb == 0 ? r.x : (cb == 1 ? r.y : r.z);
        w0 = -r.w * ((cb == 0 ? 1.0 : 0.0) - r.x * uc);
        w1 = -r.w * ((cb == 1 ? 1.0 : 0.0) - r.y * uc);
        w2 = -r.w * ((cb == 2 ? 1.0 : 0.0) - r.z * uc);
    } else {
        const double* wo = W + (size_t)o * D * 3 + cb;
        w0 = wo[0]; w1 = wo[D]; w2 = wo[2 * D];
    }
}

template <int D, int WAVES, bool GPW = false, bool RETRY = false, bool ORD = false>
__global__ __launch_bounds__(WAVES * 64, SCHUR_MINW) void k_schur(const int4* __restrict__ work, const int* __restrict__ row_ptr,
                                                      const int* __restrict__ col, int C, const int* __restrict__ cam_ptr,
                                                      const int* __restrict__ cam_obs, const int* __restrict__ ptl,
                                                      const int* __restrict__ pt_ptr, const int* __restrict__ ustart,
                                                      const int4* __restrict__ sdesc,
                                                      const int* __restrict__ cam, const double* __restrict__ W,
                                                      const double* __restrict__ Vinv, const double* __restrict__ y,
                                                      const double* __restrict__ U, const double* __restrict__ gc, double f,
                                                      double cmin, double cmax, int add_diag, double* __restrict__ S,
                                                      double* __restrict__ b, long long* stp) {
    const StampScope stamp_(stp);
    constexpr int DD = D * D;
    constexpr int BS = schur_bs(D);
    constexpr int WS = schur_ws(D);
    constexpr int NG = 64 / D;
    constexpr int NT = WAVES * 64;
    extern __shared__ __attribute__((aligned(16))) double sh[];
    __shared__ int rnd_sh[ORD ? 2 * WAVES : 1];
    const int4 wk = work[blockIdx.x];
    const int i = wk.x, kb = wk.y, ke = wk.z, nb = ke - kb;
    double* acc = sh;
    double* wsh = acc + (size_t)nb * BS;
    double* bacc = wsh + (size_t)WAVES * NG * WS;
    int* slot = reinterpret_cast<int*>(bacc + D + 12);
    const int t = threadIdx.x, lane = t & 63, wv = t >> 6;
    for (int k = t; k < nb * BS; k += NT) acc[k] = 0.0;
    for (int k = t; k < C; k += NT) slot[k] = -1;
    if (t < D) bacc[t] = 0.0;
    __syncthreads();
    for (int e = kb + t; e < ke; e += NT) slot[col[e]] = e - kb;
    __syncthreads();
    const bool diag_chunk = (kb == row_ptr[i]);
    const int g = lane / D, cb = lane - g * D;
    const bool active = g < NG;
    double* my_wh = wsh + (size_t)(wv * NG + (active ? g : 0)) * WS;
    double breg = 0.0;
    const int ob = cam_ptr[i], oe = cam_ptr[i + 1];
    int4 dnext = make_int4(0, 0, 0, 0);
    constexpr int UP = ORD ? SCHUR_UP_DET : SCHUR_UP;
    {
        const int e0 = ob + wv * NG + g;
        if (active && e0 < oe) dnext = sdesc[e0];
        if constexpr (ORD) {
            const int n0 = (active && e0 < oe) ? dnext.w - dnext.z : 0;
            int nr0 = 0;
            while (__builtin_amdgcn_ballot_w64(nr0 * UP < n0) != 0) ++nr0;
            if (lane == 0) rnd_sh[wv] = nr0;
            __syncthreads();
        }
    }
    const int nround = ORD ? (oe - ob + WAVES * NG - 1) / (WAVES * NG) : 0;
    for (int base = ob + wv * NG, rd = 0; ORD ? rd < nround : base < oe; base += WAVES * NG, ++rd) {
        const int e = base + g;
        const bool has = active && e < oe;
        const int4 dcur = dnext;
        {
            const int en = e + WAVES * NG;
            if (active && en < oe) dnext = sdesc[en];
        }
        const int qs = has ? dcur.z : 0, qe = has ? dcur.w : 0;
        const int n = qe - qs;
        double w0 = 0.0, w1 = 0.0, w2 = 0.0, v00 = 0.0, v01 = 0.0, v02 = 0.0, v11 = 0.0, v12 = 0.0, v22 = 0.0;
        if (has) {
            if constexpr (GPW || RETRY) {
                const double* vi = Vinv + 6 * (size_t)dcur.y;
                v00 = vi[0]; v01 = vi[1]; v02 = vi[2]; v11 = vi[3]; v12 = vi[4]; v22 = vi[5];
            }
            load_wcol<D, GPW>(W, dcur.x, cb, w0, w1, w2);
        }
        double x[UP][3];
        int cj[UP];
#pragma unroll
        for (int u = 0; u < UP; ++u) {
            cj[u] = -1;
            if (u < n) {
                load_wcol<D, GPW>(W, qs + u, cb, x[u][0], x[u][1], x[u][2]);
                cj[u] = cam[qs + u];
            }
        }
        if (has) {
            if constexpr (GPW || RETRY) {
                my_wh[cb * 4 + 0] = -(w0 * v00 + w1 * v01 + w2 * v02);
                my_wh[cb * 4 + 1] = -(w0 * v01 + w1 * v11 + w2 * v12);
                my_wh[cb * 4 + 2] = -(w0 * v02 + w1 * v12 + w2 * v22);
            } else {
                my_wh[cb * 4 + 0] = -w0;
                my_wh[cb * 4 + 1] = -w1;
                my_wh[cb * 4 + 2] = -w2;
            }
            if (diag_chunk) {
                const double* yp = y + 3 * (size_t)dcur.y;
                breg -= w0 * yp[0] + w1 * yp[1] + w2 * yp[2];
            }
        }
        __builtin_amdgcn_fence(__ATOMIC_RELEASE, "wavefront");
        __builtin_amdgcn_wave_barrier();
        __builtin_amdgcn_fence(__ATOMIC_ACQUIRE, "wavefront");
        double wh[D][3];
        if (has) {
#pragma unroll
            for (int a2 = 0; a2 < D; ++a2) {
                wh[a2][0] = my_wh[a2 * 4 + 0];
                wh[a2][1] = my_wh[a2 * 4 + 1];
                wh[a2][2] = my_wh[a2 * 4 + 2];
            }
        }
        int nrd = 0;
        if constexpr (ORD) {
#pragma unroll
            for (int w2 = 0; w2 < WAVES; ++w2) nrd = max(nrd, rnd_sh[(rd & 1) * WAVES + w2]);
            const int en = e + WAVES * NG;
            const int nn = (active && en < oe) ? dnext.w - dnext.z : 0;
            int nrn = 0;
            while (__builtin_amdgcn_ballot_w64(nrn * UP < nn) != 0) ++nrn;
            if (lane == 0) rnd_sh[((rd + 1) & 1) * WAVES + wv] = nrn;
        }
        for (int k0 = 0; ORD ? k0 < nrd * UP : __builtin_amdgcn_ballot_w64(k0 < n) != 0; k0 += UP) {
            if (k0 > 0) {
#pragma unroll
                for (int u = 0; u < UP; ++u) {
                    cj[u] = -1;
                    if (k0 + u < n) {
                        const int q = qs + k0 + u;
                        load_wcol<D, GPW>(W, q, cb, x[u][0], x[u][1], x[u][2]);
                        cj[u] = cam[q];
                    }
                }
            }
            int slv[UP];
#pragma unroll
            for (int u = 0; u < UP; ++u) slv[u] = slot[cj[u] >= 0 ? cj[u] : 0];
            __builtin_amdgcn_s_waitcnt(0xC07F);
            __builtin_amdgcn_sched_barrier(0);
            if constexpr (ORD)
                for (int k = 0; k < wv; ++k) __syncthreads();
#pragma unroll
            for (int u = 0; u < UP; ++u) {
                if (cj[u] >= 0) {
                    const int sl = slv[u];
                    if (sl >= 0) {
                        double* dst = acc + (size_t)sl * BS + cb;
                        const double y0 = x[u][0], y1 = x[u][1], y2 = x[u][2];
#pragma unroll
                        for (int a2 = 0; a2 < D; ++a2)
                            atomicAdd(dst + a2 * D, wh[a2][0] * y0 + wh[a2][1] * y1 + wh[a2][2] * y2);
                    }
                }
            }
            if constexpr (ORD)
                for (int k = wv; k < WAVES; ++k) __syncthreads();
        }
        if (ORD && nrd == 0) __syncthreads();
        __builtin_amdgcn_wave_barrier();
    }
    if constexpr (ORD)
        for (int k = 0; k < wv; ++k) __syncthreads();
    if (diag_chunk && active) atomicAdd(bacc + cb, breg);
    if constexpr (ORD)
        for (int k = wv; k < WAVES; ++k) __syncthreads();
    __syncthreads();
    double* Sout = S + (size_t)kb * DD;
    const double* Ui = U + (size_t)i * DD;
    for (int k = t; k < nb * DD; k += NT) {
        double v = acc[(k / DD) * BS + k % DD];
        if (diag_chunk && add_diag && k < DD) {
            const int a2 = k / D, bb = k % D;
            double u = Ui[k];
            if (a2 == bb) u = clampd(u, cmin, cmax) * f;
            v += u;
        }
        Sout[k] = v;
    }
    if (diag_chunk && t < D) b[(size_t)i * D + t] = (add_diag ? gc[(size_t)i * D + t] : 0.0) + bacc[t];
}

}
```

instantsfm_amd/csrc/ba_solve.h:

```cpp
#pragma once
#include "ba_handle.h"
#include "cg_poll.h"
#include "solve_policy.h"

namespace {

enum Ev {
    kEvLinearize = 0, kEvTrial = 1, kEvBacksub = 3, kEvCost = 4, kEvTrialEnd = 5, kEvSchur = 6, kEvSchurEnd = 7,
    kEvCg = 8, kEvCgEnd = 9, kEvDebug = 10, kEvDebugEnd = 11, kEvChain = 12, kEvChainEnd = 14, kEvXchg = 16,
    kEvXchgEnd = 17
};
enum Phase { kPhLinearize, kPhSchur, kPhSolve, kPhBacksub, kPhCost, kPhCgLaunches, kPhSideChain, kPhExchange };

int allreduce(insfm_ba* h, double* buf, int64_t n) {
    if (h->d.world_size <= 1 && !h->d.allreduce) return 0;
    if (!h->d.allreduce) { h->err = "world_size > 1 needs an allreduce callback"; return INSFM_BA_ECOMM; }
    int rc = h->d.allreduce(h->d.allreduce_ctx, buf, n);
    if (rc) { h->err = "allreduce callback failed (" + std::to_string(rc) + ")"; return INSFM_BA_ECOMM; }
    return 0;
}

int allreduce_async(insfm_ba* h, double* buf, int64_t n) {
    int rc = h->d.allreduce_async(h->d.allreduce_ctx, buf, n, h->xstream);
    if (rc) { h->err = "allreduce_async callback failed (" + std::to_string(rc) + ")"; return INSFM_BA_ECOMM; }
    return 0;
}

long long* stamp_ptr(const insfm_ba* h, int kind) {
    if (!h->stamps) return nullptr;
    return h->stamps + ((size_t)(h->stamp_step % kStampSteps) * kStKinds + kind) * 2;
}

void rec(insfm_ba* h, Ev k) {
    if (h->timing) (void)hipEventRecord(h->ev[k], h->stream);
}

bool host_trace2() {
    static const bool v = diag("trace2");
    return v;
}
void hmark(insfm_ba* h, const char* what) {
    if (host_trace2()) h->hmarks.emplace_back(what, wall_seconds());
}
void print_hmarks(insfm_ba* h) {
    if (!host_trace2() || h->hmarks.empty()) return;
    hmark(h, "step end");
    std::string line = "[insfm host2]";
    for (auto& m : h->hmarks)
        line += " " + std::string(m.first) + "=" + std::to_string((int)(1e6 * (m.second - h->hmarks[0].second)));
    std::fprintf(stderr, "%s\n", line.c_str());
}

void acc_time(insfm_ba* h, Ev a, Ev b, Phase slot) {
    if (!h->timing) return;
    float ms = 0.f;
    if (hipEventElapsedTime(&ms, h->ev[a], h->ev[b]) == hipSuccess) h->tms[slot] += ms;
}

int lin_join(insfm_ba* h) {
    if (!h->ss.lin_pending) return 0;
    HIPCHK(hipStreamWaitEvent(h->stream, h->ev_lc, 0));
    h->ss.lin_pending = false;
    return 0;
}

PointPrep first_trial_prep(insfm_ba* h) {
    PointPrep pp1;
    pp1.f = 1.0 + h->damping;
    pp1.cmin = h->d.clamp_min;
    pp1.cmax = h->d.clamp_max;
    pp1.Vinv = h->Vinv;
    pp1.y = h->y;
    pp1.R = h->d.optimize_poses ? h->Rf : nullptr;
    pp1.flags = h->flags;
    pp1.status = h->cg.status;
    return pp1;
}

template <int M>
void launch_lin_points_w(insfm_ba* h, const double* cams, const double* pts_local, const PointPrep& pp1) {
    k_lin_points<M><<<h->n_lin, kLinThreads, 0, h->stream>>>(h->lin_blk, h->pt_ptr, h->cam, h->ptl, h->uv, h->pp, cams,
                                                         pts_local, h->d.huber_delta, pp1.R ? h->W : nullptr, h->V, h->gp,
                                                         pp1, stamp_ptr(h, kStLinPoints));
}

template <int M>
void launch_lin_cams(insfm_ba* h, hipStream_t stream, const double* cams, const double* pts_local) {
    constexpr int D = kD<M>;
    if constexpr (D <= 9) {
        k_lin_cams_reg<M><<<h->C, LIN_CAMS_NT, 0, stream>>>(h->cam_ptr, h->cm_pt, h->cm_uv, h->pp, cams, pts_local,
                                                         h->d.huber_delta, h->U, h->gc);
    } else {
        const size_t lds = sizeof(double) * kThreads * (2 * D + 2);
        k_lin_cams<M><<<h->C, kThreads, lds, stream>>>(h->cam_ptr, h->cm_pt, h->cm_uv, h->pp, cams, pts_local,
                                                       h->d.huber_delta, h->U, h->gc);
    }
}

int launch_zero_words(insfm_ba* h) {
    k_zero_words<<<1, 64, 0, h->stream>>>(h->flags, h->cg.status);
    return launch_err(h, "k_zero_words");
}

int run_linearize(insfm_ba* h, const double* cams, const double* pts_local) {
    h->ss.tl_fresh = true;
    if (h->kind == 1) {
        if (h->Nl > 0)
            k_gp_lin<<<cdiv(h->Nl, kThreads), kThreads, 0, h->stream>>>(h->Nl, h->cam, h->ptl, h->trans, h->fcam, h->sfree,
                                                                       cams, pts_local, h->scl_cur, h->d.huber_delta, h->gobs);
        k_gp_lin_cams<<<h->C, kThreads, 0, h->stream>>>(h->C, h->cam_ptr, h->cam_obs, h->gobs, h->U, h->gc);
        int rc = launch_err(h, "k_gp_lin");
        if (rc) return rc;
        return allreduce(h, h->U, (int64_t)h->C * h->D * h->D + (int64_t)h->C * h->D);
    }
    if (int rc0 = lin_join(h)) return rc0;
    const PointPrep pp1 = first_trial_prep(h);
    h->ss.prep_valid = false;
    if (h->kind == 0 && h->Pl > 0) {
        if (h->ss.flags_dirty) {
            if (int e = launch_zero_words(h)) return e;
            h->ss.flags_dirty = false;
        }
        h->ss.prep_valid = true;
        h->ss.prep_f = pp1.f;
    }
    int rc = with_model(h->model, [&](auto mc) -> int {
        constexpr int M = decltype(mc)::value;
        if (h->Pl > 0) launch_lin_points_w<M>(h, cams, pts_local, pp1);
        if (!h->u_late) {
            launch_lin_cams<M>(h, h->stream, cams, pts_local);
            return launch_err(h, "linearize");
        }
        HIPCHK(hipEventRecord(h->ev_lin0, h->stream));
        HIPCHK(hipStreamWaitEvent(h->aux, h->ev_lin0, 0));
        launch_lin_cams<M>(h, h->aux, cams, pts_local);
        if (int e = launch_err(h, "k_lin_cams")) return e;
        HIPCHK(hipEventRecord(h->ev_lc, h->aux));
        h->ss.lin_pending = true;
        return launch_err(h, "k_lin_points");
    });
    if (rc) return rc;
    return allreduce(h, h->U, (int64_t)h->C * h->D * h->D + (int64_t)h->C * h->D);
}

int run_tl_basis(insfm_ba* h, const double* cams, hipStream_t stream) {
    const int C = h->C;
    if (h->kind == 1) {
        k_tl_basis<kGP><<<h->tl.nc, kThreads, 0, stream>>>(C, cams, h->Lf, h->tl, h->cg.r[0]);
        return launch_err(h, "k_tl_basis");
    }
    return with_model(h->model, [&](auto mc) -> int {
        constexpr int M = decltype(mc)::value;
        k_tl_basis<M><<<h->tl.nc, kThreads, 0, stream>>>(C, cams, h->Lf, h->tl, h->cg.r[0], stamp_ptr(h, kStBasis));
        return launch_err(h, "k_tl_basis");
    });
}

constexpr int kErowGrid = 256;
int run_tl_build(insfm_ba* h, int slot, hipStream_t stream, bool have_oseg = false) {
    const int C = h->C, m = h->tl.m;
    TlBufs tl = h->tl;
    tl.E = h->Ebuf[slot];
    return with_D(h->D, [&](auto dc_) -> int {
        constexpr int DV = decltype(dc_)::value;
        const int grid = stream != h->stream ? std::min(C, kErowGrid) : C;
        if (!have_oseg)
            k_tl_erow<DV><<<grid, kThreads, 0, stream>>>(C, h->nbr_ptr, h->nbr_j, h->Sn, tl);
        k_tl_ereduce<DV><<<cdiv(m * m, kThreads), kThreads, 0, stream>>>(tl);
        return launch_err(h, "k_tl_erow/ereduce");
    });
}

int run_tl_gj_unit(insfm_ba* h, int slot, int u, hipStream_t stream) {
    launch_gj_unit(u, h->tl.m, h->Ebuf[slot], h->gjW, h->gjP, h->tl.Ed, h->Einvbuf[slot], h->okbuf + slot, stream);
    return launch_err(h, "k_gj_pinv0/k_gj_step");
}

#ifndef CG_AHEAD
#define CG_AHEAD 1
#endif
#ifndef CG_INIT_BACK
#define CG_INIT_BACK 2
#endif
constexpr int kCgAhead = CG_AHEAD;

void harvest_chain_time(insfm_ba* h) {
    for (int sl = 0; sl < 2; ++sl) {
        if (!h->chain_timed[sl] || hipEventQuery(h->ev[kEvChainEnd + sl]) != hipSuccess) continue;
        float ms = 0.f;
        if (hipEventElapsedTime(&ms, h->ev[kEvChain + sl], h->ev[kEvChainEnd + sl]) == hipSuccess) h->tms[kPhSideChain] += ms;
        h->chain_timed[sl] = false;
    }
}

int issue_side_chain(insfm_ba* h, int slot, bool have_oseg = false) {
    hipStream_t fs = h->side;
    HIPCHK(hipStreamWaitEvent(fs, h->ev_E, 0));
    const bool tm = h->timing && !h->chain_timed[slot];
    if (tm) HIPCHK(hipEventRecord(h->ev[kEvChain + slot], fs));
    if (int rc = run_tl_build(h, slot, fs, have_oseg)) return rc;
    h->ss.chain_oseg = have_oseg;
    HIPCHK(hipEventRecord(h->ev_built, fs));
    h->ss.built_pending = true;
    for (int u = 0; u <= gj_steps(h->tl.m); ++u)
        if (int rc = run_tl_gj_unit(h, slot, u, fs)) return rc;
    HIPCHK(hipEventRecord(h->ev_fact[slot], fs));
    if (tm) {
        HIPCHK(hipEventRecord(h->ev[kEvChainEnd + slot], fs));
        h->chain_timed[slot] = true;
    }
    return 0;
}

int side_flush(insfm_ba* h) {
    if (h->side) HIPCHK(hipStreamSynchronize(h->side));
    return 0;
}

int run_tl_setup(insfm_ba* h, const SolvePlan& p, const double* cams) {
    if (h->timing) harvest_chain_time(h);
    if (int rc = p.basis_by_factor ? 0 : run_tl_basis(h, cams, h->stream)) return rc;
    h->ss.tl_fresh = false;
    if (!p.defer_chain) {
        HIPCHK(hipEventRecord(h->ev_E, h->stream));
        if (int rc = issue_side_chain(h, p.slot)) return rc;
    }
    if (p.must_wait_fact || hipEventQuery(h->ev_fact[p.use]) != hipSuccess)
        HIPCHK(hipStreamWaitEvent(h->stream, h->ev_fact[p.use], 0));
    h->tl.Einv = h->Einvbuf[p.use];
    h->tl.ok = h->okbuf + p.use;
    ++h->ss.tl_solves;
    return 0;
}

template <int D>
void launch_pc(insfm_ba* h, int it, int maxit, double tol2, const TlBufs& tl) {
    k_tl_pc<D><<<h->tl.nc, kPcThreads, h->pc_lds, h->stream>>>(it, h->C, maxit, tol2, h->pc_rows, h->cg, tl, h->tl.Einv);
}
template <int D>
void launch_pspmv(insfm_ba* h, int it, int rows, const TlBufs& tl, const XPart& xp = XPart{}) {
    k_tl_pspmv<D><<<rows, kPspmvThreads, 0, h->stream>>>(it, h->C, h->nbr_stride, h->nbr_ptr, h->nbr_j, h->Sn, h->Lf,
                                                          h->cg, tl, xp);
}

template <int D>
void launch_tl_iter(insfm_ba* h, int it, int maxit, double tol2) {
    if (it == 0) {
        launch_pc<D>(h, -1, maxit, tol2, h->tl);
        launch_pspmv<D>(h, -1, h->C, h->tl);
    }
    if (h->tl.Racc)
        k_tl_pc_cl<D><<<h->tl.nc, kPcThreads, 0, h->stream>>>(it, h->C, maxit, tol2, h->cg, h->tl, h->tl.Einv);
    else
        launch_pc<D>(h, it, maxit, tol2, h->tl);
    launch_pspmv<D>(h, it, h->C, h->tl);
}

TlBufs tl_region(const insfm_ba* h, int q) {
    TlBufs t = h->tl;
    const int C = h->C, D = h->D;
    double* base = h->xwin + h->xoff_region[q];
    t.vc = base;
    t.gd = base + (size_t)C * D;
    t.rowR = base + (size_t)C * D + 3 * (size_t)C;
    return t;
}

XPart xpart_region(const insfm_ba* h, int q) {
    XPart xp;
    xp.win = h->xbases;
    xp.world = h->d.world_size;
    xp.q0 = h->xq[h->d.rank];
    xp.off_vc = h->xoff_region[q];
    xp.off_gd = xp.off_vc + (long long)h->C * h->D;
    xp.off_rowR = xp.off_gd + 3LL * h->C;
    return xp;
}

void launch_xchg(insfm_ba* h, int slot) {
    k_xsignal<<<1, 64, 0, h->stream>>>(h->cg.status, h->xcnt, h->xpflags, h->d.world_size, h->d.rank, slot);
    k_xwait<<<1, 64, 0, h->stream>>>(h->cg.status, h->cg.prog, h->xcnt,
                                     reinterpret_cast<unsigned*>(h->xwin + h->xoff_flags), h->d.world_size, slot);
}

template <int D>
void launch_tl_iter_x(insfm_ba* h, int it, int maxit, double tol2) {
    const int nrows = h->xq[h->d.rank + 1] - h->xq[h->d.rank];
    auto pspmv = [&](int i) {
        if (nrows > 0) launch_pspmv<D>(h, i, nrows, tl_region(h, i & 1), xpart_region(h, (i + 1) & 1));
        launch_xchg(h, 0);
    };
    if (it == 0) {
        launch_pc<D>(h, -1, maxit, tol2, tl_region(h, 1));
        pspmv(-1);
    }
    launch_pc<D>(h, it, maxit, tol2, tl_region(h, it & 1));
    pspmv(it);
}

template <int D>
void launch_tl_iters(insfm_ba* h, int from, int to, int maxit, double tol2) {
    for (int k = from; k < to; ++k)
        if (h->xpart) launch_tl_iter_x<D>(h, k, maxit, tol2);
        else launch_tl_iter<D>(h, k, maxit, tol2);
}

using CgpKernel = decltype(&k_tl_cgp<64, false, false>);
CgpKernel cgp_kernel(int nb, bool det, bool adef) {
    if (nb == 64) {
        if (det) return adef ? k_tl_cgp<64, true, true> : k_tl_cgp<64, true, false>;
        return adef ? k_tl_cgp<64, false, true> : k_tl_cgp<64, false, false>;
    }
    if (det) return adef ? k_tl_cgp<128, true, true> : k_tl_cgp<128, true, false>;
    return adef ? k_tl_cgp<128, false, true> : k_tl_cgp<128, false, false>;
}

int cgp_reset_barriers(insfm_ba* h) {
    HIPCHK(hipMemsetAsync(h->cgp_sync, 0, sizeof(unsigned) * kCgpSyncWords, h->stream));
    h->ss.cgp_epochs = 0;
    return 0;
}

int launch_tl_cgp(insfm_ba* h, bool adef2, bool write_segments) {
    const int maxit = h->d.pcg_max_iter;
    const double tol2 = h->d.pcg_tol * h->d.pcg_tol;
    if (h->ss.cgp_epochs > (1u << 24))
        if (int rc = cgp_reset_barriers(h)) return rc;
    static std::atomic<int> faults{diag("cgp_fault") ? 1 : 0};
    const bool fault = faults.load() > 0 && faults.fetch_sub(1) > 0;
    static std::atomic<int> bkdn{diag("adef2_breakdown") ? 1 : 0};
    const bool breakdown = adef2 && bkdn.load() > 0 && bkdn.fetch_sub(1) > 0;
    hipLaunchKernelGGL(cgp_kernel(h->cgp_nb, h->cgp_det, adef2), dim3(h->cgp_grid), dim3(kCgpThreads), 0, h->stream,
                       h->C, h->nbr_ptr, h->nbr_j, (const double*)h->S, (const int*)h->cgp_src, (const double*)h->Li,
                       (const double*)h->Lf, h->cg, h->tl, (const double*)h->tl.Einv, maxit, tol2, h->cgp_wx, h->cgp_yg,
                       h->ss.cgp_tag, h->cgp_sync, h->ss.cgp_epochs,
                       cgp_flag_word(write_segments, fault, breakdown, !h->last.basis_by_factor), h->cgp_runs,
                       h->cgp_trace, h->dc, stamp_ptr(h, kStCgp));
    if (int rc = launch_err(h, "k_tl_cgp")) return rc;
    h->ss.cgp_tag += (unsigned)maxit + 3u;
    return 0;
}

using SchurKernel = decltype(&k_schur<8, kSchurWaves>);
SchurKernel schur_kernel(int kind, int D, bool det, bool retry) {
    if (kind == 1) return det ? k_schur<3, kDetWaves, true, false, SCHUR_DET_ORD> : nullptr;
    SchurKernel k = nullptr;
    with_ba_D(D, [&](auto dc_) -> int {
        constexpr int DV = decltype(dc_)::value;
        if (det) k = retry ? k_schur<DV, kDetWaves, false, true, SCHUR_DET_ORD> : k_schur<DV, kDetWaves, false, false, SCHUR_DET_ORD>;
        else k = retry ? k_schur<DV, kSchurWaves, false, true> : k_schur<DV, kSchurWaves>;
        return 0;
    });
    return k;
}

int launch_schur(insfm_ba* h, double sf, double smin, double smax, int sdiag, bool retry, int w0 = 0, int w1 = -1) {
    const bool det = h->d.deterministic != 0, gpk = h->kind == 1;
    const double *Uin = gpk ? h->Up : h->U, *gcin = gpk ? h->gpc : h->gc;
    if (w1 < 0) w1 = h->nwork;
    const int nt = det ? kDetWaves * 64 : kSchurWaves * 64;
    const SchurKernel kern = schur_kernel(h->kind, h->D, det, retry);
    if (gpk && !kern) {
        k_schur_gp<kSchurWaves, kGPSG><<<h->nwork, nt, h->schur_lds, h->stream>>>(
            h->work, h->row_ptr, h->col, h->C, h->cam_ptr, h->sdesc, h->cam, h->W, h->VY, Uin, gcin, h->S, h->b);
        return launch_err(h, "k_schur");
    }
    if (!kern) return INSFM_BA_EINVAL;
    if (!gpk && w1 <= w0) return 0;
    hipLaunchKernelGGL(kern, dim3(w1 - w0), dim3(nt), h->schur_lds, h->stream, h->work + w0, h->row_ptr, h->col, h->C,
                       h->cam_ptr, h->cam_obs, h->ptl, h->pt_ptr, h->ustart, h->sdesc, h->cam, h->W,
                       gpk ? h->Vinv : h->Mp, h->y, Uin, gcin, sf, smin, smax, sdiag, h->S, h->b,
                       gpk ? nullptr : stamp_ptr(h, kStSchur));
    return launch_err(h, "k_schur");
}

int print_cgp_trace(insfm_ba* h, const int* st) {
    double tr[kCgpTraceLen];
    HIPCHK(hipMemcpy(tr, h->cgp_trace, sizeof(tr), hipMemcpyDeviceToHost));
    const int n = std::min(st[1], 63);
    std::fprintf(stderr, "[insfm cgp] status %d iterations %d coarse %d: setup %.1f us (blocks + tables %.1f, A %.1f, "
                 "rest %.1f), iterations %.1f us (%.2f us each)\n",
                 st[0], st[1], st[2], 0.01 * (tr[257] - tr[256]), 0.01 * (tr[578] - tr[256]),
                 0.01 * (tr[579] - tr[578]), 0.01 * (tr[257] - tr[579]), 0.01 * (tr[258 + n] - tr[257]),
                 n > 0 ? 0.01 * (tr[258 + n] - tr[258]) / n : 0.0);
    for (int k = 0; k <= n; ++k) {
        std::fprintf(stderr, "[insfm cgp]   it %d gamma %.17g delta %.17g rho %.17g done %g t %.1f us | loads %.2f P1 %.2f y %.2f "
                     "P2 %.2f B2 %.2f\n", k, tr[4 * k], tr[4 * k + 1], tr[4 * k + 2], tr[4 * k + 3], 0.01 * (tr[258 + k] - tr[256]),
                     k > 0 ? 0.01 * (tr[258 + k] - tr[322 + 4 * (k - 1) + 3]) : 0.0,
                     0.01 * (tr[322 + 4 * k] - tr[258 + k]), 0.01 * (tr[323 + 4 * k] - tr[322 + 4 * k]),
                     0.01 * (tr[324 + 4 * k] - tr[323 + 4 * k]), 0.01 * (tr[325 + 4 * k] - tr[324 + 4 * k]));
        if (k < n)
            std::fprintf(stderr, "[insfm cgp]        P1 split: fills + workgroup barrier %.2f, y %.2f, S~w %.2f; "
                         "scalar partials in %.2f after the barrier\n",
                         0.01 * (tr[580 + 3 * k] - tr[258 + k]), 0.01 * (tr[581 + 3 * k] - tr[580 + 3 * k]),
                         0.01 * (tr[322 + 4 * k] - tr[581 + 3 * k]),
                         k > 0 ? 0.01 * (tr[582 + 3 * k] - tr[322 + 4 * (k - 1) + 3]) : 0.0);
    }
    const int G = std::min(h->cgp_grid, 256);
    if (st[1] > kCgpTraceIt + 1 && G > 0) {
        double s0 = tr[772], s1 = tr[772];
        for (int b = 0; b < G; ++b) { s0 = std::min(s0, tr[772 + b]); s1 = std::max(s1, tr[772 + b]); }
        std::vector<int> ord(G);
        for (int b = 0; b < G; ++b) ord[b] = b;
        std::sort(ord.begin(), ord.end(), [&](int a, int b) { return tr[1028 + a] > tr[1028 + b]; });
        std::fprintf(stderr, "[insfm cgp] it %d per workgroup: starts within %.2f us; arrival at the barrier "
                     "(us after the first start): median %.2f, last %.2f; latest:", kCgpTraceIt, 0.01 * (s1 - s0),
                     0.01 * (tr[1028 + ord[G / 2]] - s0), 0.01 * (tr[1028 + ord[0]] - s0));
        for (int q = 0; q < std::min(G, 8); ++q)
            std::fprintf(stderr, " wg %d (%.2f, start %.2f)", ord[q], 0.01 * (tr[1028 + ord[q]] - s0),
                         0.01 * (tr[772 + ord[q]] - s0));
        std::fprintf(stderr, "\n");
    }
    return 0;
}

int cgp_complete(insfm_ba* h, bool adef2, int* st) {
    std::atomic_thread_fence(std::memory_order_seq_cst);
    volatile int* pg = h->prog_host;
    st[0] = pg[1]; st[1] = pg[2]; st[2] = pg[3];
    if (st[0] == 1 || st[0] == 2) {
        h->ss.cgp_epochs += cgp_barriers(adef2, st[1]);
    } else {
        HIPCHK(hipStreamSynchronize(h->stream));
        if (int rc = cgp_reset_barriers(h)) return rc;
        if (st[0] == 4 && h->d.world_size <= 1 && !h->xpart) {
            std::fprintf(stderr, "[insfm] k_tl_cgp: a grid barrier timed out (the GPU is shared with another "
                                 "process?); this handle continues on the launch-per-iteration CG\n");
            h->cgp_nb = 0;
            h->ss.cgp_lost = true;
        }
    }
    return h->cgp_trace ? print_cgp_trace(h, st) : 0;
}

struct CgStart {
    bool gated = false, htrace = false;
    double t_sol0 = 0.0, t_enq = 0.0, m_enq = 0.0;
    int n_enq = 0;
};

int cg_begin(insfm_ba* h, CgStart& cs) {
    volatile int* pg = h->prog_host;
    pg[0] = pg[1] = pg[2] = pg[3] = 0;
    std::atomic_thread_fence(std::memory_order_seq_cst);
    static const bool htrace = diag("trace");
    cs.htrace = htrace;
    cs.t_sol0 = htrace ? wall_seconds() : 0.0;
    rec(h, kEvCg);
    cs.gated = h->d.world_size > 1 || h->d.allreduce;
    if (cs.gated) HIPCHK(hipEventRecord(h->ev_pre, h->stream));
    return 0;
}

template <typename Enqueue>
int cg_wait(insfm_ba* h, CgStart& cs, int* enq, Enqueue&& enqueue) {
    volatile int* pg = h->prog_host;
    CgPoll poll;
    poll.enq = *enq;
    const double stall_s = cg_stall_limit();
    int erc = 0;
    const int pr = cg_poll(
        poll, h->d.pcg_max_iter + 2, kCgAhead, stall_s, cg_gate_limit_s(stall_s), [&] { return (int)pg[1]; },
        [&] { return (int)pg[0]; }, enqueue,
        [&] {
            const hipError_t q = hipStreamQuery(h->stream);
            if (q == hipSuccess) { std::atomic_thread_fence(std::memory_order_seq_cst); return 0; }
            return q == hipErrorNotReady ? 1 : -1;
        },
        wall_seconds, [] { cpu_relax(); },
        [&] { return !cs.gated || hipEventQuery(h->ev_pre) != hipErrorNotReady; }, &erc);
    hmark(h, "cg converged");
    if (cs.htrace)
        std::fprintf(stderr, "[insfm host] solve %.1f us: %d iterations enqueued in %.1f us (max %.1f per iteration)\n",
                     1e6 * (wall_seconds() - cs.t_sol0), cs.n_enq, 1e6 * cs.t_enq, 1e6 * cs.m_enq);
    *enq = poll.enq;
    if (pr == CgPoll::kEnqueueError) return erc;
    if (pr == CgPoll::kStreamError) {
        h->err = std::string("PCG: ") + hipGetErrorString(hipStreamQuery(h->stream));
        return INSFM_BA_EHIP;
    }
    if (pr == CgPoll::kStalled || pr == CgPoll::kGateStalled) {
        h->err = std::string(pr == CgPoll::kGateStalled ? "PCG: the cross-rank exchange in front of the CG did not "
                                                          "complete within "
                                                        : "PCG: no progress from the device for ") +
                 std::to_string(poll.stalled_s) + " s (iterations started " + std::to_string(pg[0]) + ", status " +
                 std::to_string(pg[1]) + ", enqueued " + std::to_string(*enq) +
                 "); set INSFM_CG_STALL_S to change the limit";
        return INSFM_BA_EHIP;
    }
    std::atomic_thread_fence(std::memory_order_seq_cst);
    rec(h, kEvCgEnd);
    if (h->timing) {
        HIPCHK(hipStreamSynchronize(h->stream));
        acc_time(h, kEvCg, kEvCgEnd, kPhCgLaunches);
    }
    return 0;
}

int run_cgp(insfm_ba* h, bool adef2, bool defer_chain, bool async, int* st) {
    CgStart cs;
    if (int rc = cg_begin(h, cs)) return rc;
    if (int rc = launch_tl_cgp(h, adef2, defer_chain)) return rc;
    if (defer_chain) {
        static const bool hold = diag("chain_hold");
        if (!hold) HIPCHK(hipEventRecord(h->ev_E, h->stream));
        if (hold) h->ss.chain_oseg = false;
        else if (int rc = issue_side_chain(h, h->last.slot, true)) return rc;
    }
    if (async) {
        rec(h, kEvCgEnd);
        h->cg_launches += 1;
        h->ss.cgp_pending = true;
        st[0] = 1; st[1] = 0; st[2] = 1;
        return 0;
    }
    int enq = h->d.pcg_max_iter + 2;
    if (int rc = cg_wait(h, cs, &enq, [](int, int) { return 0; })) return rc;
    h->cg_launches += 1;
    return cgp_complete(h, adef2, st);
}

int run_launch_cg(insfm_ba* h, int* st) {
    const int maxit = h->d.pcg_max_iter;
    const double tol2 = h->d.pcg_tol * h->d.pcg_tol;
    CgStart cs;
    if (int rc = cg_begin(h, cs)) return rc;
    auto enqueue = [&](int from, int to) -> int {
        const double t0 = cs.htrace ? wall_seconds() : 0.0;
        const int r = with_D(h->D, [&](auto dc_) -> int {
            launch_tl_iters<decltype(dc_)::value>(h, from, to, maxit, tol2);
            return launch_err(h, "k_tl_pc/k_tl_pspmv");
        });
        if (cs.htrace) {
            const double dt = wall_seconds() - t0;
            cs.t_enq += dt; cs.m_enq = std::max(cs.m_enq, dt / std::max(1, to - from)); cs.n_enq += to - from;
        }
        return r;
    };
    int enq = cg_first_batch(h->ss.last_cg_iters, maxit, kCgAhead, CG_INIT_BACK);
    if (int rc = enqueue(0, enq)) return rc;
    if (int rc = cg_wait(h, cs, &enq, enqueue)) return rc;
    h->cg_launches += enq;
    volatile int* pg = h->prog_host;
    st[0] = pg[1]; st[1] = pg[2]; st[2] = pg[3];
    return 0;
}

int run_bj_cg(insfm_ba* h, int* st) {
    const int D = h->D, maxit = h->d.pcg_max_iter;
    const double tol2 = h->d.pcg_tol * h->d.pcg_tol;
    int it = 0;
    for (;;) {
        const int chunk = (it == 0) ? std::max(8, h->ss.last_cg_iters + 6) : 8;
        const int stop = std::min(it + chunk, maxit + 2);
        rec(h, kEvCg);
        const int rc = with_D(D, [&](auto dc_) -> int {
            constexpr int DV = decltype(dc_)::value;
            if (h->tlon) launch_tl_iters<DV>(h, it, stop, maxit, tol2);
            else for (int k = it; k < stop; ++k) {
                if (k > 0) k_cg_dots<<<1, 64, 0, h->stream>>>(k, h->C, maxit, tol2, h->cg);
                k_cg_iter<DV><<<h->C, kCgThreads, 0, h->stream>>>(k, h->C, maxit, tol2, h->nbr_ptr, h->nbr_j, h->Sn,
                                                                h->Lf, h->cg);
            }
            return launch_err(h, "k_cg_iter");
        });
        if (rc) return rc;
        rec(h, kEvCgEnd);
        h->cg_launches += stop - it;
        it = stop;
        HIPCHK(hipMemcpyAsync(st, h->cg.status, sizeof(int) * 3, hipMemcpyDeviceToHost, h->stream));
        HIPCHK(hipStreamSynchronize(h->stream));
        acc_time(h, kEvCg, kEvCgEnd, kPhCgLaunches);
        if (st[0] != 0 || it >= maxit + 2) break;
    }
    return 0;
}

int cg_tail(insfm_ba* h, bool dc_by_cgp, int* st) {
    const int D = h->D;
    int rc = 0;
    if (st[0] != 1) {
        h->err = pcg_status_message(st[0], st[1], h->tlon ? st[2] : kCoarseOff);
        return st[0] == 4 ? INSFM_BA_EHIP : INSFM_BA_ESOLVER;
    }
    if (!h->ss.cgp_pending) {
        h->coarse_used = h->tlon ? st[2] : 0;
        h->ss.last_cg_iters = st[1];
    }
    if (h->xpart) {
        const int n = h->xq[h->d.rank + 1] - h->xq[h->d.rank];
        if (n > 0)
            k_xput_x<<<cdiv((long long)n * D, 256), 256, 0, h->stream>>>(n, D, h->tl.cl_cams, h->cg.x,
                                                                        xpart_region(h, 0), h->xoff_xg);
        launch_xchg(h, 1);
        HIPCHK(hipMemcpyAsync(h->cg.x, h->xwin + h->xoff_xg, sizeof(double) * (size_t)h->C * D,
                              hipMemcpyDeviceToDevice, h->stream));
        if ((rc = launch_err(h, "partitioned CG gather"))) return rc;
        int sw[2] = {0, 0};
        HIPCHK(hipMemcpyAsync(sw, h->cg.status, sizeof(sw), hipMemcpyDeviceToHost, h->stream));
        HIPCHK(hipStreamSynchronize(h->stream));
        if (sw[0] == 4) {
            h->err = "partitioned CG: the solution gather across ranks timed out";
            return INSFM_BA_EHIP;
        }
    }
    if (dc_by_cgp) return h->ss.cgp_pending ? 0 : st[1];
    rc = with_D(D, [&](auto dc_) -> int {
        constexpr int DV = decltype(dc_)::value;
        k_cg_finish<DV><<<cdiv((long long)h->C * DV, kThreads), kThreads, 0, h->stream>>>(h->C, h->Li, h->cg.x,
                                                                                        h->dc, stamp_ptr(h, kStCgFinish));
        return launch_err(h, "k_cg_finish");
    });
    if (rc) return rc;
    hmark(h, "cg_finish");
    return h->ss.cgp_pending ? 0 : st[1];
}

template <int DV>
void launch_scale(insfm_ba* h) {
    k_cg_scale<DV><<<cdiv(h->nnzb, kWaves * scale_nb(DV)), kThreads, 0, h->stream>>>(
        h->nnzb, h->blk_row, h->col, h->row_ptr, h->pos_up, h->pos_lo, h->Li, h->S, h->Sn, 0);
}

int ensure_sn(insfm_ba* h) {
    if (h->ss.sn_valid || h->kind != 0 || !h->d.optimize_poses) return 0;
    const int rc = with_D(h->D, [&](auto dc_) -> int {
        launch_scale<decltype(dc_)::value>(h);
        return launch_err(h, "k_cg_scale");
    });
    if (!rc) h->ss.sn_valid = true;
    return rc;
}

int reissue_chain(insfm_ba* h) {
    if (!h->ss.chain_oseg) return 0;
    h->ss.chain_oseg = false;
    HIPCHK(hipEventRecord(h->ev_E, h->stream));
    return issue_side_chain(h, h->last.slot);
}

template <int DV>
void launch_factor(insfm_ba* h, double f, bool add_U, const double* basis_cams, bool first = false) {
    const double *U = add_U ? h->U : nullptr, *gc = add_U ? h->gc : nullptr;
    const double cmin = first ? h->d.clamp_min : 0.0, cmax = first ? h->d.clamp_max : 0.0;
    long long* stamp = first ? stamp_ptr(h, kStFactor) : nullptr;
    if constexpr (DV != 3) {
        if (basis_cams) {
            k_cg_factor_basis<DV><<<cdiv(h->C, kWaves), kThreads, 0, h->stream>>>(
                h->C, h->row_ptr, h->S, h->b, h->Lf, h->Li, h->cg, U, gc, f, cmin, cmax, basis_cams, h->tl,
                h->cgp_runs + (size_t)h->cgp_grid * kCgpRows * 12, stamp);
            return;
        }
    }
    k_cg_factor<DV><<<cdiv(h->C, kWaves), kThreads, 0, h->stream>>>(h->C, h->row_ptr, h->S, h->b, h->Lf, h->Li, h->cg, U,
                                                                   gc, f, cmin, cmax, stamp);
}

int solve_tail(insfm_ba* h, double f, const double* cams, const double* pts_local, const double* dcp) {
    const bool gpk = h->kind == 1;
    rec(h, kEvBacksub);
    if (gpk) {
        if (h->Pl > 0)
            k_gp_backsub<kGPG><<<h->n_gp_grp, kThreads, 0, h->stream>>>(h->Pl, h->pt_ptr, h->cam, h->gobs, dcp, h->Vinv, h->gp,
                                                              pts_local, h->scl_cur, f, h->d.clamp_min, h->d.clamp_max, h->dp,
                                                              h->pts_new, h->scl_new, h->ds, h->part_gp);
        k_gp_update_cams<<<cdiv(3 * h->C, kThreads), kThreads, 0, h->stream>>>(3 * h->C, cams, dcp, h->cams_new);
        return launch_err(h, "k_gp_backsub/update");
    }
    if (int rc0 = lin_join(h)) return rc0;
    const int rc = with_model(h->model, [&](auto mc) -> int {
        constexpr int M = decltype(mc)::value;
        const int nrun = h->Pl > 0 ? h->n_lin : 0;
        k_backsub_rc<M><<<nrun + h->n_gc, kLinThreads, 0, h->stream>>>(
            h->lin_blk, h->pt_ptr, h->cam, h->ptl, h->uv, h->pp, cams, h->d.huber_delta, dcp, h->V, h->Vinv, h->gp,
            pts_local, h->dp, h->pts_new, h->part_gp, nrun, h->C, h->U, h->gc, h->d.rank == 0, h->cams_new, h->part_gc,
            stamp_ptr(h, kStBacksub));
        return launch_err(h, "k_backsub_rc");
    });
    if (rc) return rc;
    hmark(h, "backsub");
    return 0;
}

int refactor(insfm_ba* h, const double* basis_cams) {
    return with_D(h->D, [&](auto dc_) -> int {
        launch_factor<decltype(dc_)::value>(h, 1.0, false, basis_cams);
        return launch_err(h, basis_cams ? "k_cg_factor_basis" : "k_cg_factor");
    });
}

int repeat_cg(insfm_ba* h, const RepeatRecipe& r, int* st) {
    const auto has = [&](RepeatStep s) { return (r.steps & s) != 0; };
    int rc = 0;
    h->ss.cgp_lost = false;
    if (has(kStepLeavePersistent)) {
        h->cgp_nb = 0;
        HIPCHK(hipStreamSynchronize(h->stream));
        if ((rc = cgp_reset_barriers(h))) return rc;
    }
    if (has(kStepZeroStatus)) HIPCHK(hipMemsetAsync(h->cg.status, 0, sizeof(int) * 4, h->stream));
    if (has(kStepFactorize) && (rc = refactor(h, r.factor_with_cams ? h->cams_cur : nullptr))) return rc;
    if (has(kStepEnsureSn) && (rc = ensure_sn(h))) return rc;
    if (has(kStepBasis) && (rc = run_tl_basis(h, h->cams_cur, h->stream))) return rc;
    if (has(kStepReissueChain) && (rc = reissue_chain(h))) return rc;
    if (!has(kStepRunCg)) return 0;
    return r.additive ? run_cgp(h, false, false, false, st) : run_launch_cg(h, st);
}

SolveFacts solve_facts(const insfm_ba* h, bool async_status) {
    SolveFacts s;
    s.kind = h->kind; s.optimize_poses = h->d.optimize_poses != 0; s.tlon = h->tlon;
    s.prog_host = h->prog_host != nullptr; s.cgp = h->cgp_nb != 0; s.u_late = h->u_late;
    s.rank0 = h->d.rank == 0; s.has_points = h->Pl > 0; s.keep_S = h->keep_S != 0;
    s.clamp_min = h->d.clamp_min; s.clamp_max = h->d.clamp_max;
    s.flags_dirty = h->ss.flags_dirty; s.prep_valid = h->ss.prep_valid; s.prep_f = h->ss.prep_f;
    s.tl_solves = h->ss.tl_solves; s.tl_fresh = h->ss.tl_fresh; s.async_status = async_status;
    return s;
}

int run_solve(insfm_ba* h, double f, const double* cams, const double* pts_local, bool async_status) {
    const int D = h->D;
    const SolvePlan p = h->last = plan_solve(solve_facts(h, async_status), f);
    h->ss.prep_valid = false;
    if (int rc0 = p.zero_words ? launch_zero_words(h) : 0) return rc0;
    h->ss.flags_dirty = true;
    if (h->kind == 1) {
        if (h->Pl > 0)
            k_gp_prep_points<kGPG><<<cdiv((long long)h->Pl * kGPG, kThreads), kThreads, 0, h->stream>>>(h->Pl, h->pt_ptr, h->gobs, f, h->d.clamp_min,
                                                                               h->d.clamp_max, h->W, h->V, h->gp, h->Vinv,
                                                                               h->y, h->VY, h->flags);
        k_gp_prep_cams<<<h->C, kThreads, 0, h->stream>>>(h->C, h->cam_ptr, h->cam_obs, h->gobs, h->U, h->gc, f,
                                                                     h->d.clamp_min, h->d.clamp_max, h->d.rank == 0, h->Up,
                                                                     h->gpc);
    } else if (h->Pl > 0 && !p.prepared && (hmark(h, "point_prep"), true))
        k_point_prep<<<cdiv(h->Pl, kThreads), kThreads, 0, h->stream>>>(h->Pl, h->V, h->gp, f, h->d.clamp_min, h->d.clamp_max,
                                                                       h->Vinv, h->y, h->flags, h->cg.status,
                                                                       h->d.optimize_poses ? h->Rf : nullptr, h->Mp);
    int iters = 0;
    if (p.cg != kCgNone) {
        rec(h, kEvSchur);
        int rc = 0;
        if (h->xstream) {
            const int K = (int)h->xw.size() - 1;
            for (int c = 0; c < K; ++c) {
                if ((rc = launch_schur(h, p.sf, p.smin, p.smax, p.sdiag, !p.prepared, h->xw[c], h->xw[c + 1]))) return rc;
                const int64_t b0 = h->rptr_host[h->xr[c]], b1 = h->rptr_host[h->xr[c + 1]];
                HIPCHK(hipEventRecord(h->ev_x, h->stream));
                HIPCHK(hipStreamWaitEvent(h->xstream, h->ev_x, 0));
                if (h->timing && c == 0) HIPCHK(hipEventRecord(h->ev[kEvXchg], h->xstream));
                if (b1 > b0 && (rc = allreduce_async(h, h->S + b0 * D * D, (b1 - b0) * D * D))) return rc;
            }
            if ((rc = allreduce_async(h, h->b, (int64_t)h->C * D))) return rc;
            HIPCHK(hipEventRecord(h->ev_xdone, h->xstream));
            if (h->timing) HIPCHK(hipEventRecord(h->ev[kEvXchgEnd], h->xstream));
            HIPCHK(hipStreamWaitEvent(h->stream, h->ev_xdone, 0));
            rec(h, kEvSchurEnd);
        } else {
            if ((rc = launch_schur(h, p.sf, p.smin, p.smax, p.sdiag, !p.prepared))) return rc;
            hmark(h, "schur");
            rec(h, kEvSchurEnd);
            if ((rc = allreduce(h, h->S, (int64_t)h->nnzb * D * D + (int64_t)h->C * D))) return rc;
        }
        if (h->ss.built_pending) {
            HIPCHK(hipStreamWaitEvent(h->stream, h->ev_built, 0));
            h->ss.built_pending = false;
        }
        if ((rc = lin_join(h))) return rc;
        rc = with_D(D, [&](auto dc_) -> int {
            constexpr int DV = decltype(dc_)::value;
            launch_factor<DV>(h, f, p.add_U_in_factor, p.basis_by_factor ? cams : nullptr, true);
            if (p.scale) launch_scale<DV>(h);
            return launch_err(h, "k_cg_factor/scale");
        });
        h->ss.sn_valid = p.scale;
        if (rc) return rc;
        hmark(h, "factor/scale");
        if (h->tlon && (rc = run_tl_setup(h, p, cams))) return rc;
        hmark(h, "tl setup");
        int* st = reinterpret_cast<int*>(h->host_res + 8);
        bool dc_by_cgp = p.dc_by_cgp;
        if (p.cg == kCgBlockJacobi) rc = run_bj_cg(h, st);
        else if (p.cg == kCgLaunchPath) rc = run_launch_cg(h, st);
        else rc = run_cgp(h, h->adef2, p.defer_chain, p.cg == kCgPersistentAsync, st);
        if (rc) return rc;
        if (h->ss.cgp_lost) {
            if ((rc = repeat_cg(h, repeat_recipe(kRepeatLaunchPath, p.basis_by_factor), st))) return rc;
            dc_by_cgp = false;
        }
        if ((iters = cg_tail(h, dc_by_cgp, st)) < 0) return iters;
    }
    if (int rb = solve_tail(h, f, cams, pts_local, p.cg != kCgNone ? h->dc : nullptr)) return rb;
    return iters;
}

}
```

instantsfm_amd/csrc/create_plan.h:

```cpp
#pragma once
#include <algorithm>
#include <cstdint>
#include <vector>

#include "create_host.h"

namespace insfm {

struct Int4 {
    int x, y, z, w;
};
static_assert(sizeof(Int4) == 16, "Int4 is uploaded as int4");

inline int plan_check_inputs(HostPool& pool, int C, int P, int N, const int32_t* cam_idx, const int32_t* pt_idx) {
    std::vector<int> bad(pool.size(), 0);
    pool.ranges(N, [&](int t, long long a, long long b) {
        for (long long i = a; i < b; ++i) {
            if (cam_idx[i] < 0 || cam_idx[i] >= C) { bad[t] = 1; return; }
            if (pt_idx[i] < 0 || pt_idx[i] >= P) { bad[t] = 2; return; }
            if (i && pt_idx[i] < pt_idx[i - 1]) { bad[t] = 3; return; }
        }
    });
    for (int e : bad)
        if (e) return e;
    return 0;
}

struct TrackOrder {
    std::vector<int> gptr, lptr;
    nivec<int> lptl, lcam, lsrc, lust, key;
    int o0 = 0, Nl = 0;
};
inline TrackOrder plan_track_order(HostPool& pool, int P, int N, int p0, int p1, const int32_t* cam_idx,
                                   const int32_t* pt_idx) {
    TrackOrder t;
    t.gptr.assign(P + 1, 0);
    pool.ranges(P + 1, [&](int, long long a, long long b) {
        for (long long p = a; p < b; ++p) t.gptr[p] = (int)(std::lower_bound(pt_idx, pt_idx + N, (int32_t)p) - pt_idx);
    });
    t.o0 = t.gptr[p0];
    t.Nl = t.gptr[p1] - t.o0;
    const int o0 = t.o0, Nl = t.Nl, Pl = p1 - p0;
    t.lptr.resize(Pl + 1);
    t.lptl.resize(Nl); t.lcam.resize(Nl); t.lsrc.resize(Nl); t.lust.resize(Nl); t.key.resize(Nl);
    for (int p = 0; p <= Pl; ++p) t.lptr[p] = t.gptr[p0 + p] - o0;
    pool.ranges(Pl, [&](int, long long pa, long long pb) {
        for (long long p = pa; p < pb; ++p) {
            const int b0 = t.lptr[p], b1 = t.lptr[p + 1];
            for (int o = b0; o < b1; ++o) {
                const int x = o0 + o, cx = cam_idx[x];
                int u = o;
                while (u > b0 && cam_idx[t.lsrc[u - 1]] > cx) { t.lsrc[u] = t.lsrc[u - 1]; --u; }
                t.lsrc[u] = x;
            }
            int u = b0;
            for (int o = b0; o < b1; ++o) {
                t.lcam[o] = cam_idx[t.lsrc[o]];
                t.lptl[o] = (int)p;
                if (o > b0 && t.lcam[o] != t.lcam[o - 1]) u = o;
                t.lust[o] = u;
                t.key[o] = b1 - u;
            }
        }
    });
    return t;
}

struct CamMajor {
    std::vector<int> cptr;
    nivec<int> cobs;
};
inline CamMajor plan_cam_major(HostPool& pool, int C, const TrackOrder& t, int chunk) {
    CamMajor m;
    pcount_sort(pool, t.Nl, C, nullptr, [&](int o) { return t.lcam[o]; }, m.cobs, m.cptr);
    pool.ranges(C, [&](int, long long i0, long long i1) {
        for (long long i = i0; i < i1; ++i)
            for (int a = m.cptr[i]; a < m.cptr[i + 1]; a += chunk) {
                const int e = std::min(a + chunk, m.cptr[i + 1]);
                std::stable_sort(m.cobs.data() + a, m.cobs.data() + e, [&](int x, int y) { return t.key[x] > t.key[y]; });
            }
    });
    return m;
}

struct CovisGraph {
    std::vector<int> ptr, nb;
    std::vector<long long> w;
};
struct BlockPattern {
    std::vector<int> gcptr, rptr, cols, upw;
    CovisGraph g;
};

inline BlockPattern plan_pattern_host(HostPool& pool, int C, int N, const int32_t* cam_idx, const int32_t* pt_idx,
                                      const std::vector<int>& gptr) {
    BlockPattern b;
    CovisGraph& g = b.g;
    b.rptr.assign(C + 1, 0);
    nivec<int> gcpt;
    pcount_sort(pool, N, C, nullptr, [&](int i) { return cam_idx[i]; }, gcpt, b.gcptr, [&](int i) { return pt_idx[i]; });
    const int T = pool.size();
    std::vector<std::vector<int>> pnb(T);
    std::vector<std::vector<long long>> pw(T);
    std::vector<int> nlen(C, 0), ulen(C, 0);
    pool.ranges(C, [&](int t, long long i0, long long i1) {
        std::vector<int> mark(C, -1), buf;
        std::vector<long long> acc(C, 0);
        for (int i = (int)i0; i < (int)i1; ++i) {
            buf.clear();
            for (int e = b.gcptr[i]; e < b.gcptr[i + 1]; ++e) {
                const int p = gcpt[e];
                for (int q = gptr[p]; q < gptr[p + 1]; ++q) {
                    const int j = cam_idx[q];
                    if (j == i) continue;
                    if (mark[j] != i) { mark[j] = i; acc[j] = 0; buf.push_back(j); }
                    acc[j] += 1;
                }
            }
            std::sort(buf.begin(), buf.end());
            int up = 0;
            for (int j : buf) { pnb[t].push_back(j); pw[t].push_back(acc[j]); up += j > i; }
            nlen[i] = (int)buf.size();
            ulen[i] = up;
        }
    });
    g.ptr.assign(C + 1, 0);
    for (int i = 0; i < C; ++i) {
        g.ptr[i + 1] = g.ptr[i] + nlen[i];
        b.rptr[i + 1] = b.rptr[i] + 1 + ulen[i];
    }
    g.nb.reserve(g.ptr[C]);
    g.w.reserve(g.ptr[C]);
    for (int t = 0; t < T; ++t) {
        g.nb.insert(g.nb.end(), pnb[t].begin(), pnb[t].end());
        g.w.insert(g.w.end(), pw[t].begin(), pw[t].end());
    }
    b.cols.resize(b.rptr[C]);
    pool.ranges(C, [&](int, long long i0, long long i1) {
        for (int i = (int)i0; i < (int)i1; ++i) {
            int k = b.rptr[i];
            b.cols[k++] = i;
            for (int e = g.ptr[i]; e < g.ptr[i + 1]; ++e)
                if (g.nb[e] > i) b.cols[k++] = g.nb[e];
        }
    });
    return b;
}

inline BlockPattern plan_pattern_from_upper(int C, const std::vector<int>& ulen, const std::vector<int>& uoff,
                                            const std::vector<int>& unb, const std::vector<int>& uwt) {
    BlockPattern b;
    b.rptr.assign(C + 1, 0);
    for (int i = 0; i < C; ++i) b.rptr[i + 1] = b.rptr[i] + 1 + ulen[i];
    b.cols.resize(b.rptr[C]);
    b.upw.assign(b.rptr[C], 0);
    for (int i = 0; i < C; ++i) {
        b.cols[b.rptr[i]] = i;
        for (int k = 0; k < ulen[i]; ++k) {
            b.cols[b.rptr[i] + 1 + k] = unb[uoff[i] + k];
            b.upw[b.rptr[i] + 1 + k] = uwt[uoff[i] + k];
        }
    }
    return b;
}

struct LowerLists {
    std::vector<int> brow, lop, locol, loblk;
};
inline LowerLists plan_lower(int C, const std::vector<int>& rptr, const std::vector<int>& cols) {
    LowerLists l;
    l.brow.resize(rptr[C]);
    for (int i = 0; i < C; ++i)
        for (int e = rptr[i]; e < rptr[i + 1]; ++e) l.brow[e] = i;
    l.lop.assign(C + 1, 0);
    for (int i = 0; i < C; ++i)
        for (int e = rptr[i] + 1; e < rptr[i + 1]; ++e) l.lop[cols[e] + 1]++;
    for (int c = 0; c < C; ++c) l.lop[c + 1] += l.lop[c];
    l.locol.resize(std::max(1, l.lop[C]));
    l.loblk.resize(std::max(1, l.lop[C]));
    std::vector<int> fill(l.lop.begin(), l.lop.end() - 1);
    for (int i = 0; i < C; ++i)
        for (int e = rptr[i] + 1; e < rptr[i + 1]; ++e) {
            const int k = fill[cols[e]]++;
            l.locol[k] = i;
            l.loblk[k] = e;
        }
    return l;
}

inline void plan_graph_from_upper(int C, const LowerLists& l, BlockPattern& b) {
    CovisGraph& g = b.g;
    const std::vector<int>&rptr = b.rptr, &cols = b.cols, &upw = b.upw;
    g.ptr.assign(C + 1, 0);
    for (int i = 0; i < C; ++i) g.ptr[i + 1] = g.ptr[i] + (l.lop[i + 1] - l.lop[i]) + (rptr[i + 1] - rptr[i] - 1);
    g.nb.resize(g.ptr[C]);
    g.w.resize(g.ptr[C]);
    for (int i = 0; i < C; ++i) {
        int k = g.ptr[i];
        for (int q = l.lop[i]; q < l.lop[i + 1]; ++q, ++k) { g.nb[k] = l.locol[q]; g.w[k] = upw[l.loblk[q]]; }
        for (int e2 = rptr[i] + 1; e2 < rptr[i + 1]; ++e2, ++k) { g.nb[k] = cols[e2]; g.w[k] = upw[e2]; }
    }
}

inline int aggregate(const CovisGraph& g, int C, int K, std::vector<int>& lab) {
    lab.assign(C, -1);
    std::vector<long long> score(C, 0);
    std::vector<char> incand(C, 0);
    std::vector<int> cand, asize;
    int nagg = 0;
    for (int seed = 0; seed < C; ++seed) {
        if (lab[seed] >= 0) continue;
        cand.clear();
        int size = 0, cur = seed;
        for (;;) {
            lab[cur] = nagg;
            ++size;
            for (int e = g.ptr[cur]; e < g.ptr[cur + 1]; ++e) {
                const int j = g.nb[e];
// ... 305 lines not shown
```

instantsfm_amd/csrc/solve_policy.h:

```cpp
#pragma once
#include "lm_policy.h"

namespace insfm {

struct SolveFacts {
    int kind = 0;
    bool optimize_poses = true;
    bool tlon = false;
    bool prog_host = false;
    bool cgp = false;
    bool u_late = false;
    bool rank0 = true;
    bool has_points = true;
    bool keep_S = false;
    double clamp_min = 0.0, clamp_max = 0.0;
    bool flags_dirty = false;
    bool prep_valid = false;
    double prep_f = 0.0;
    long long tl_solves = 0;
    bool tl_fresh = false;
    bool async_status = false;
};

enum CgRun {
    kCgNone,
    kCgBlockJacobi,
    kCgLaunchPath,
    kCgPersistent,
    kCgPersistentAsync
};

struct SolvePlan {
    bool prepared = false;
    bool zero_words = false;
    double sf = 1.0, smin = 0.0, smax = 0.0;
    int sdiag = 0;
    bool add_U_in_factor = false;
    bool scale = true;
    bool basis_by_factor = false;
    CgRun cg = kCgNone;
    bool dc_by_cgp = false;
    int slot = 0, use = 0;
    bool defer_chain = false, must_wait_fact = true;
};

inline SolvePlan plan_solve(const SolveFacts& s, double f) {
    SolvePlan p;
    const bool gpk = s.kind == 1;
    p.prepared = s.prep_valid && s.prep_f == f && s.kind == 0;
    p.zero_words = s.flags_dirty || !s.has_points || gpk;
    p.sf = gpk ? 1.0 : f;
    p.smin = gpk ? -1.0e308 : s.clamp_min;
    p.smax = gpk ? 1.0e308 : s.clamp_max;
    p.sdiag = gpk ? 1 : (s.u_late ? 0 : (s.rank0 ? 1 : 0));
    p.add_U_in_factor = s.u_late && !gpk;
    p.scale = !(s.tlon && s.cgp && s.tl_solves > 0 && s.tl_fresh && !s.keep_S);
    p.basis_by_factor = s.tlon && s.cgp && !gpk;
    if (!s.optimize_poses) p.cg = kCgNone;
    else if (!(s.tlon && s.prog_host)) p.cg = kCgBlockJacobi;
    else if (!s.cgp) p.cg = kCgLaunchPath;
    else p.cg = s.async_status ? kCgPersistentAsync : kCgPersistent;
    p.dc_by_cgp = p.cg == kCgPersistent || p.cg == kCgPersistentAsync;
    p.slot = (int)(s.tl_solves & 1);
    p.use = (s.tl_solves > 0 && s.tl_fresh) ? (p.slot ^ 1) : p.slot;
    p.defer_chain = s.cgp && p.use != p.slot;
    p.must_wait_fact = p.use == p.slot;
    return p;
}

enum CgpFlag : int {
    kCgpWriteSegments = 1,
    kCgpTestFault = 2,
    kCgpTestBreakdown = 4,
    kCgpRestrictionFromBasis = 8
};
inline int cgp_flag_word(bool write_segments, bool test_fault, bool test_breakdown, bool restriction_from_basis) {
    return (write_segments ? kCgpWriteSegments : 0) | (test_fault ? kCgpTestFault : 0) |
           (test_breakdown ? kCgpTestBreakdown : 0) | (restriction_from_basis ? kCgpRestrictionFromBasis : 0);
}

inline int cg_path_code(bool xpart, int nb, bool det, bool adef2) {
    if (xpart) return 3;
    if (!nb) return 0;
    return det ? (adef2 ? 5 : 2) : (adef2 ? 4 : 1);
}

enum RepeatStep : unsigned {
    kStepLeavePersistent = 1u << 0,
    kStepZeroStatus = 1u << 1,
    kStepFactorize = 1u << 2,
    kStepEnsureSn = 1u << 3,
    kStepBasis = 1u << 4,
    kStepReissueChain = 1u << 5,
    kStepRunCg = 1u << 6
};
struct RepeatRecipe {
    bool valid = false;
    unsigned steps = 0;
    bool additive = false;
    bool factor_with_cams = false;
};

inline RepeatRecipe repeat_recipe(CgpNext how, bool basis_by_factor) {
    RepeatRecipe r;
    r.valid = true;
    if (how == kRepeatCollective) {
        r.steps = kStepLeavePersistent | kStepZeroStatus | kStepFactorize | kStepEnsureSn | kStepBasis |
                  kStepReissueChain | kStepRunCg;
    } else if (how == kRepeatLaunchPath) {
        r.steps = kStepZeroStatus | kStepEnsureSn | kStepBasis | kStepReissueChain | kStepRunCg;
    } else if (how == kRepeatAdditive) {
        r.steps = kStepZeroStatus | kStepFactorize | (basis_by_factor ? 0u : (unsigned)kStepBasis) | kStepRunCg;
        r.additive = true;
        r.factor_with_cams = basis_by_factor;
    } else {
        r.valid = false;
    }
    return r;
}

}
```

instantsfm_amd/engine.py:

```python
import ctypes
import time

import numpy as np
import torch

from . import _capi

LM_DEFAULTS = dict(tr_radius=1e4, tr_max=1e10, tr_min=1e-6, tr_up=2.0, tr_down=0.5 ** 4, tr_factor=0.25,
                   tr_high=0.5, tr_low=1e-3, clamp_min=1e-6, clamp_max=1e32, max_rejects=30, pcg_tol=1e-5,
                   pcg_max_iter=500, precond=2, cluster_size=24, exchange_chunks=4)


STAMP_KERNELS = ("k_lin_points", "k_schur", "k_tl_cgp", "k_cg_finish", "k_publish", "k_cg_factor", "k_tl_basis",
                 "k_backsub_rc", "k_cost", "k_final")
CG_PATHS = {0: "launch-per-iteration two-level CG", 1: "k_tl_cgp (persistent, atomic cluster sums)",
            2: "k_tl_cgp (persistent, fixed-order)", 3: "row-partitioned CG",
            4: "k_tl_cgp (persistent, atomic cluster sums, A-DEF2 coarse correction: precond 2)",
            5: "k_tl_cgp (persistent, fixed-order, A-DEF2 coarse correction: precond 2)"}
CGP_PATHS = (1, 2, 4, 5)
CGP_DET_PATHS = (2, 5)


def effective_precond(requested, path):
    if path in (4, 5):
# ... 114 lines not shown
        self.lib = lib_stream
        self.ctx = None
        self.caller = None

    def __enter__(self):
        self.caller = torch.cuda.current_stream(self.lib.device)
        self.ctx = None
        if self.caller != self.lib:
            self.lib.wait_stream(self.caller)
            self.ctx = torch.cuda.stream(self.lib)
            self.ctx.__enter__()
        return self

    def __exit__(self, *exc):
        if self.ctx is not None:
            self.ctx.__exit__(*exc)
            self.caller.wait_stream(self.lib)
        return False


class BundleAdjuster:

    def __init__(self, model, uv, cam_idx, pt_idx, pp, n_cams, n_points, device="cuda:0", optimize_poses=True,
                 huber_delta=1.0, deterministic=False, world_size=1, rank=0, shard=None, process_group=None,
                 force_exchange=False, **lm):
        self.device = _require_gpu(device)
        L = _capi.load()
        opts = dict(LM_DEFAULTS, **lm)
        uv = np.ascontiguousarray(uv, dtype=np.float64).reshape(-1, 2)
        cam_idx = np.ascontiguousarray(cam_idx, dtype=np.int32).reshape(-1)
        pt_idx = np.ascontiguousarray(pt_idx, dtype=np.int32).reshape(-1)
        pp = np.ascontiguousarray(pp, dtype=np.float64).reshape(-1, 2)
        d = _capi.default_desc()
        d.n_cams, d.n_points, d.n_obs = int(n_cams), int(n_points), int(uv.shape[0])
        d.cam_model = int(model)
        d.optimize_poses = int(bool(optimize_poses))
        d.deterministic = int(bool(deterministic))
        d.huber_delta = float(huber_delta)
        for k, v in opts.items():
            setattr(d, k, type(getattr(d, k))(v))
        d.world_size, d.rank = int(world_size), int(rank)
        d.shard_point_begin, d.shard_point_end = (0, -1) if shard is None else (int(shard[0]), int(shard[1]))
        self._xbuf = None
        self._cb = None
        self._errors = []
        self.exchange_calls = [0, 0.0]
        exchange = world_size > 1 or force_exchange
        if exchange:
            self._cb = _capi.ALLREDUCE_FN(make_allreduce_callback(lambda: self._xbuf, process_group, self._errors,
                                                                  self.exchange_calls))
            d.allreduce = self._cb
            if d.exchange_chunks > 1:
                self._cb_async = _capi.ALLREDUCE_ASYNC_FN(make_allreduce_async_callback(
                    lambda: self._xbuf, process_group, self._errors, self.exchange_calls))
                d.allreduce_async = self._cb_async
        self._stream = torch.cuda.current_stream(self.device)
        stream = self._stream.cuda_stream
        h = ctypes.c_void_p()
        rc = L.insfm_ba_create(ctypes.byref(d), uv.ctypes.data_as(ctypes.POINTER(ctypes.c_double)),
                               cam_idx.ctypes.data_as(ctypes.POINTER(ctypes.c_int32)),
                               pt_idx.ctypes.data_as(ctypes.POINTER(ctypes.c_int32)),
                               pp.ctypes.data_as(ctypes.POINTER(ctypes.c_double)), ctypes.c_void_p(stream), ctypes.byref(h))
        if rc != 0:
            msg = L.insfm_ba_last_error(h).decode() if h.value else ""
            if h.value:
                L.insfm_ba_destroy(h)
            raise _capi.BAError(rc, msg)
        self._h = h
        self.desc = d
        self.n_cams, self.n_points, self.n_obs = d.n_cams, d.n_points, d.n_obs
        self.D = 6 + {0: 1, 1: 2, 2: 2, 3: 3, 4: 6, 5: 6, 6: 10, 8: 2, 9: 3}[int(model)]
        if exchange:
            n = L.insfm_ba_exchange_count(h)
            self._xbuf = torch.zeros(int(n), dtype=torch.float64, device=self.device)
            _capi.check(h, L.insfm_ba_set_exchange(h, ctypes.c_void_p(self._xbuf.data_ptr()), n))
        self.cg_path = self.cg_info()[0]
        if world_size > 1:
            self.ranks_per_device, self.cg_path = agree_cg_path(h, self.device, process_group)

    def close(self):
        if getattr(self, "_h", None) is not None and self._h.value:
            _capi.load().insfm_ba_destroy(self._h)
            self._h = None

    def __del__(self):
        try:
            self.close()
        except Exception:
            pass

    def partition_cg(self, process_group=None):
        import torch.distributed as dist
        L = _capi.load()
        hbuf = ctypes.create_string_buffer(64)
        _capi.check(self._h, L.insfm_ba_cg_window(self._h, hbuf))
        world = dist.get_world_size(process_group)
        handles = [None] * world
        dist.all_gather_object(handles, bytes(hbuf.raw), group=process_group)
        _capi.check(self._h, L.insfm_ba_cg_attach(self._h, b"".join(handles)))
        rows = (ctypes.c_int32 * 2)()
        _capi.check(self._h, L.insfm_ba_cg_partition(self._h, rows))
        return int(rows[0]), int(rows[1])

    def debug_time_exchange(self, reps=200):
        us = ctypes.c_double()
        _capi.check(self._h, _capi.load().insfm_ba_debug_time_xchg(self._h, int(reps), ctypes.byref(us)))
        return us.value

    def last_error(self):
        return _capi.load().insfm_ba_last_error(self._h).decode() if getattr(self, "_h", None) is not None else ""

    def _ptr(self, t, shape):
        if not (t.is_cuda and t.dtype == torch.float64 and t.is_contiguous()):
            raise ValueError("parameters must be contiguous float64 tensors on the GPU")
        if tuple(t.shape) != tuple(shape):
            raise ValueError(f"expected shape {shape}, got {tuple(t.shape)}")
        return ctypes.c_void_p(t.data_ptr())

    def _on_stream(self):
        return _LibraryStream(self._stream)

    def step(self, cam_params, points):
        st = _capi.Stats()
        L = _capi.load()
        with self._on_stream():
            rc = L.insfm_ba_step(self._h, self._ptr(cam_params, (self.n_cams, self.D + 1)),
                                 self._ptr(points, (self.n_points, 3)), ctypes.byref(st))
        _capi.check(self._h, rc)
        return st.loss, st.as_dict()

    def cost(self, cam_params, points):
        loss, rmse = ctypes.c_double(), ctypes.c_double()
        L = _capi.load()
        with self._on_stream():
            rc = L.insfm_ba_cost(self._h, self._ptr(cam_params, (self.n_cams, self.D + 1)),
                                 self._ptr(points, (self.n_points, 3)), ctypes.byref(loss), ctypes.byref(rmse))
        _capi.check(self._h, rc)
        return loss.value, rmse.value

    def set_timing(self, on):
        _capi.check(self._h, _capi.load().insfm_ba_set_timing(self._h, int(bool(on))))

    def reset(self):
        _capi.check(self._h, _capi.load().insfm_ba_reset(self._h))

    def debug_linearize(self, cam_params, points):
        L = _capi.load()
        _capi.check(self._h, L.insfm_ba_debug_linearize(self._h, self._ptr(cam_params, (self.n_cams, self.D + 1)),
                                                        self._ptr(points, (self.n_points, 3))))

    def debug_solve(self, f):
        return _capi.check(self._h, _capi.load().insfm_ba_debug_solve(self._h, float(f)))

    def debug_time_kernel(self, which, reps=50):
        us = ctypes.c_double()
        _capi.check(self._h, _capi.load().insfm_ba_debug_time_kernel(self._h, int(which), int(reps), ctypes.byref(us)))
        return us.value

    def debug_stamps(self, max_steps=1024):
        out = np.zeros((max_steps, len(STAMP_KERNELS), 2), dtype=np.int64)
        n = _capi.load().insfm_ba_debug_stamps(self._h, out.ctypes.data_as(ctypes.POINTER(ctypes.c_int64)), max_steps)
        _capi.check(self._h, n)
        return out[:n]

    def cg_info(self):
        info = (ctypes.c_int32 * 4)()
        _capi.check(self._h, _capi.load().insfm_ba_cg_info(self._h, info))
        return tuple(int(x) for x in info)

    def debug_time_cgp(self, reps=10):
        out = (ctypes.c_double * 3)()
        rc = _capi.load().insfm_ba_debug_time_cgp(self._h, int(reps), out)
        if rc == _capi.INSFM_BA_EINVAL:
            return None
        _capi.check(self._h, rc)
        return float(out[0]), float(out[1]), float(out[2])

    def adef2_fallbacks(self):
        return int(_capi.check(self._h, _capi.load().insfm_ba_cg_fallbacks(self._h)))

    def nnzb(self):
        return int(_capi.load().insfm_ba_nnzb(self._h))

    def coarse_dim(self):
        return self.clusters()[1] * (self.D + 1)

    def clusters(self):
        lab = np.zeros(self.n_cams, dtype=np.int32)
        nc = _capi.load().insfm_ba_debug_clusters(self._h, lab.ctypes.data_as(ctypes.POINTER(ctypes.c_int32)))
        _capi.check(self._h, nc)
        return lab, int(nc)

    def debug_get(self, which, shape):
        out = np.zeros(shape, dtype=np.float64)
        n = _capi.load().insfm_ba_debug_get(self._h, int(which), out.ctypes.data_as(ctypes.POINTER(ctypes.c_double)))
        _capi.check(self._h, n)
        assert n == out.size, (n, out.shape)
        return out


GP_DEFAULTS = dict(LM_DEFAULTS, tr_radius=1e3, tr_max=1e8, precond=1)


class GlobalPositioner(BundleAdjuster):

    def __init__(self, trans, cam_idx, pt_idx, cam_factor, scale_free, n_cams, n_points, device="cuda:0",
                 huber_delta=0.1, deterministic=False, world_size=1, rank=0, shard=None, process_group=None, **lm):
        self.device = _require_gpu(device)
        L = _capi.load()
        opts = dict(GP_DEFAULTS, **lm)
        trans = np.ascontiguousarray(trans, dtype=np.float64).reshape(-1, 3)
        cam_idx = np.ascontiguousarray(cam_idx, dtype=np.int32).reshape(-1)
        pt_idx = np.ascontiguousarray(pt_idx, dtype=np.int32).reshape(-1)
        cam_factor = np.ascontiguousarray(cam_factor, dtype=np.float64).reshape(-1)
        sf = None if scale_free is None else np.ascontiguousarray(scale_free, dtype=np.int32).reshape(-1)
        d = _capi.gp_default_desc()
        d.n_cams, d.n_points, d.n_obs = int(n_cams), int(n_points), int(trans.shape[0])
        d.deterministic = int(bool(deterministic))
        d.huber_delta = float(huber_delta)
        for k, v in opts.items():
            setattr(d, k, type(getattr(d, k))(v))
        d.world_size, d.rank = int(world_size), int(rank)
        d.shard_point_begin, d.shard_point_end = (0, -1) if shard is None else (int(shard[0]), int(shard[1]))
        self._xbuf = None
        self._cb = None
        self._errors = []
        self.exchange_calls = [0]
        if world_size > 1:
            self._cb = _capi.ALLREDUCE_FN(make_allreduce_callback(lambda: self._xbuf, process_group, self._errors,
                                                                  self.exchange_calls))
            d.allreduce = self._cb
        self._stream = torch.cuda.current_stream(self.device)
        stream = self._stream.cuda_stream
        h = ctypes.c_void_p()
        dp, ip = ctypes.POINTER(ctypes.c_double), ctypes.POINTER(ctypes.c_int32)
        rc = L.insfm_gp_create(ctypes.byref(d), trans.ctypes.data_as(dp), cam_idx.ctypes.data_as(ip),
                               pt_idx.ctypes.data_as(ip), cam_factor.ctypes.data_as(dp),
                               None if sf is None else sf.ctypes.data_as(ip), ctypes.c_void_p(stream), ctypes.byref(h))
        if rc != 0:
            msg = L.insfm_ba_last_error(h).decode() if h.value else ""
            if h.value:
                L.insfm_ba_destroy(h)
            raise _capi.BAError(rc, msg)
        self._h = h
        self.desc = d
        self.n_cams, self.n_points, self.n_obs = d.n_cams, d.n_points, d.n_obs
        self.D = 3
        if world_size > 1:
            n = L.insfm_ba_exchange_count(h)
            self._xbuf = torch.zeros(int(n), dtype=torch.float64, device=self.device)
            _capi.check(h, L.insfm_ba_set_exchange(h, ctypes.c_void_p(self._xbuf.data_ptr()), n))

    def _args(self, positions, points, scales):
        return (self._ptr(positions, (self.n_cams, 3)), self._ptr(points, (self.n_points, 3)),
                self._ptr(scales, (self.n_obs,)))

    def step(self, positions, points, scales):
        st = _capi.Stats()
        with self._on_stream():
            rc = _capi.load().insfm_gp_step(self._h, *self._args(positions, points, scales), ctypes.byref(st))
        _capi.check(self._h, rc)
        return st.loss, st.as_dict()

    def cost(self, positions, points, scales):
        loss, rmse = ctypes.c_double(), ctypes.c_double()
        with self._on_stream():
            rc = _capi.load().insfm_gp_cost(self._h, *self._args(positions, points, scales), ctypes.byref(loss),
                                            ctypes.byref(rmse))
        _capi.check(self._h, rc)
        return loss.value, rmse.value

    def debug_linearize(self, positions, points, scales):
        _capi.check(self._h, _capi.load().insfm_gp_debug_linearize(self._h, *self._args(positions, points, scales)))

    def debug_ds(self):
        out = np.zeros(self.n_obs, dtype=np.float64)
        _capi.check(self._h, _capi.load().insfm_gp_debug_get_ds(self._h, out.ctypes.data_as(ctypes.POINTER(ctypes.c_double))))
        return out
```

Before: 755.6.

## Compute Schur diagonal self-term per camera during linearization, skip in Schur kernel

Adds an optional path where a second camera-linearization kernel accumulates, for each camera, the diagonal Schur self-contribution W Vinv W^T from the point inverse Cholesky factors. The Schur kernel can then skip the diagonal self-term and the factor kernel subtracts the precomputed block instead. This moves diagonal work out of the Schur assembly into the already-overlapped camera stream. It adds an extra kernel launch, extra buffers and extra reads of Rinv. It is enabled only when each track's cameras are distinct, the run is non-deterministic and a 'self_lin' diag flag is set.

```diff
diff --git a/include/insfm_ba_debug.h b/include/insfm_ba_debug.h
--- a/include/insfm_ba_debug.h
+++ b/include/insfm_ba_debug.h
@@ -14,6 +14,8 @@
 int insfm_ba_debug_time_kernel(insfm_ba* h, int32_t which, int32_t reps, double* us_per_launch);
 int insfm_ba_debug_time_cgp(insfm_ba* h, int32_t reps, double* out);
 int32_t insfm_ba_debug_stamps(insfm_ba* h, int64_t* host_out, int32_t max_steps);
+int32_t insfm_ba_debug_self_diag(const insfm_ba* h);
+int insfm_ba_debug_set_self_diag(insfm_ba* h, int32_t on);
 int32_t insfm_ba_debug_clusters(const insfm_ba* h, int32_t* labels);
 int64_t insfm_ba_nnzb(const insfm_ba* h);
 int insfm_ba_debug_spd_inverse(int32_t m, const double* E, double* Einv, void* stream, int32_t reps,
diff --git a/instantsfm_amd/_capi.py b/instantsfm_amd/_capi.py
--- a/instantsfm_amd/_capi.py
+++ b/instantsfm_amd/_capi.py
@@ -61,7 +61,8 @@
                   "insfm_tracks_establish", "insfm_covis_pairs", "insfm_pair_inliers")
 DEBUG_SYMBOLS = ("insfm_ba_debug_linearize", "insfm_ba_debug_solve", "insfm_ba_debug_get", "insfm_ba_nnzb",
                  "insfm_ba_debug_time_kernel", "insfm_ba_debug_clusters", "insfm_ba_debug_spd_inverse",
-                 "insfm_ba_debug_time_cgp", "insfm_ba_debug_stamps",
+                 "insfm_ba_debug_time_cgp", "insfm_ba_debug_stamps", "insfm_ba_debug_self_diag",
+                 "insfm_ba_debug_set_self_diag",
                  "insfm_gp_debug_linearize", "insfm_gp_debug_get_ds",
                  "insfm_ba_cg_window", "insfm_ba_cg_attach", "insfm_ba_cg_partition", "insfm_ba_debug_time_xchg")
 SYMBOLS = PUBLIC_SYMBOLS + DEBUG_SYMBOLS
@@ -135,6 +136,11 @@
     L.insfm_ba_debug_time_kernel.restype = ctypes.c_int
     L.insfm_ba_debug_stamps.argtypes = [vp, ctypes.POINTER(ctypes.c_int64), ctypes.c_int32]
     L.insfm_ba_debug_stamps.restype = ctypes.c_int32
+    if hasattr(L, "insfm_ba_debug_self_diag"):
+        L.insfm_ba_debug_self_diag.argtypes = [vp]
+        L.insfm_ba_debug_self_diag.restype = ctypes.c_int32
+        L.insfm_ba_debug_set_self_diag.argtypes = [vp, ctypes.c_int32]
+        L.insfm_ba_debug_set_self_diag.restype = ctypes.c_int
     L.insfm_ba_debug_time_cgp.argtypes = [vp, ctypes.c_int32, dp]
     L.insfm_ba_debug_time_cgp.restype = ctypes.c_int
     L.insfm_ba_set_timing.argtypes = [vp, ctypes.c_int32]
diff --git a/instantsfm_amd/csrc/ba_create.h b/instantsfm_amd/csrc/ba_create.h
--- a/instantsfm_amd/csrc/ba_create.h
+++ b/instantsfm_amd/csrc/ba_create.h
@@ -268,6 +268,10 @@
         if ((rc = dd(h, &h->Mp, (size_t)Pl * 6))) return rc;
     }
     if ((rc = dd(h, &h->dp, (size_t)Pl * 3))) return rc;
+    if (h->self_ok) {
+        if ((rc = dd(h, &h->Rinv, (size_t)Pl * 6))) return rc;
+        if ((rc = dd(h, &h->Dself, (size_t)C * D * D))) return rc;
+    }
     h->xcount = (int64_t)h->nnzb * D * D + (int64_t)C * D + (int64_t)C * D * D + (int64_t)C * D + 8;
     if ((rc = dd(h, &h->xbuf, (size_t)h->xcount))) return rc;
     h->S = h->xbuf;
@@ -584,6 +588,9 @@
         return fail(rc, "");
     h->schur_lds = sw.schur_lds;
     if (kind == 0 && desc->world_size <= 1 && !desc->allreduce && (rc = setup_lin_stream(h))) return fail(rc, "");
+    h->self_ok = kind == 0 && desc->optimize_poses && h->u_late && !desc->deterministic && D <= 9 && Pl > 0 &&
+                 plan_distinct_track_cams(Pl, trk.lptr, trk.lcam);
+    h->self_on = h->self_ok && diag("self_lin");
     if ((rc = upload_structure(h, trk, pat, low, nbr, sw))) return fail(rc, "");
     if ((rc = alloc_numeric(h))) return fail(rc, "");
     if ((rc = setup_host_sync(h))) return fail(rc, "");
diff --git a/instantsfm_amd/csrc/ba_debug_api.h b/instantsfm_amd/csrc/ba_debug_api.h
--- a/instantsfm_amd/csrc/ba_debug_api.h
+++ b/instantsfm_amd/csrc/ba_debug_api.h
@@ -234,7 +234,8 @@
                                                                 h->Lf, h->cg);
             else {
                 const int rc2 = launch_schur(h, 1.0, h->kind ? -1e308 : h->d.clamp_min,
-                                             h->kind ? 1e308 : h->d.clamp_max, h->kind ? 1 : h->d.rank == 0, false);
+                                             h->kind ? 1e308 : h->d.clamp_max, h->kind ? 1 : h->d.rank == 0, false,
+                                             h->self_on);
                 if (rc2) return rc2;
             }
         }
@@ -281,6 +282,17 @@
     out[1] = t_pc;
     out[0] = 1e3 * t_cg / reps;
     out[2] = iters / reps;
+    return INSFM_BA_OK;
+}
+
+int32_t insfm_ba_debug_self_diag(const insfm_ba* h) {
+    if (!h) return INSFM_BA_EINVAL;
+    return h->self_on ? 1 : 0;
+}
+
+int insfm_ba_debug_set_self_diag(insfm_ba* h, int32_t on) {
+    if (!h || (on && !h->self_ok)) return INSFM_BA_EINVAL;
+    h->self_on = on != 0;
     return INSFM_BA_OK;
 }
 
@@ -331,6 +343,7 @@
         case 13: src = h->Einvbuf[1]; n = h->tlon ? (size_t)h->tl.m * h->tl.m : 0; break;
         case 14: src = h->tl.gd; n = h->tlon ? 2 * C : 0; break;
         case 15: src = h->cg.r[0]; n = C * D; break;
+        case 18: src = h->Dself; n = h->ss.dself_valid ? C * D * D : 0; break;
         case 16: case 17: src = h->Ebuf[which - 16]; n = h->tlon ? (size_t)h->tl.ldE * h->tl.ldE : 0; break;
         default: return INSFM_BA_EINVAL;
     }
diff --git a/instantsfm_amd/csrc/ba_handle.h b/instantsfm_amd/csrc/ba_handle.h
--- a/instantsfm_amd/csrc/ba_handle.h
+++ b/instantsfm_amd/csrc/ba_handle.h
@@ -30,6 +30,7 @@
     bool chain_oseg = false;
     bool cgp_pending = false;
     bool cgp_lost = false;
+    bool dself_valid = false;
     unsigned cgp_epochs = 0;
     unsigned cgp_tag = 1;
     int last_cg_iters = 16;
@@ -61,6 +62,8 @@
     size_t schur_lds = 0;
     double *W = nullptr, *V = nullptr, *gp = nullptr, *Vinv = nullptr, *y = nullptr, *dp = nullptr;
     double *Rf = nullptr, *Mp = nullptr;
+    double *Rinv = nullptr, *Dself = nullptr;
+    bool self_ok = false, self_on = false;
     double *xbuf = nullptr;
     double *S = nullptr, *b = nullptr, *U = nullptr, *gc = nullptr, *scal = nullptr;
     int64_t xcount = 0;
diff --git a/instantsfm_amd/csrc/ba_lin.h b/instantsfm_amd/csrc/ba_lin.h
--- a/instantsfm_amd/csrc/ba_lin.h
+++ b/instantsfm_amd/csrc/ba_lin.h
@@ -11,6 +11,7 @@
     double* Vinv = nullptr;
     double* y = nullptr;
     double* R = nullptr;
+    double* Ri = nullptr;
     int* flags = nullptr;
     int* status = nullptr;
 };
@@ -33,6 +34,10 @@
     if (a.R) {
 #pragma unroll
         for (int k = 0; k < 6; ++k) a.R[6 * (size_t)p + k] = R[k];
+        if (a.Ri) {
+#pragma unroll
+            for (int k = 0; k < 6; ++k) a.Ri[6 * (size_t)p + k] = Ri[k];
+        }
         a.y[3 * (size_t)p + 0] = Ri[0] * g[0];
         a.y[3 * (size_t)p + 1] = Ri[1] * g[0] + Ri[3] * g[1];
         a.y[3 * (size_t)p + 2] = Ri[2] * g[0] + Ri[4] * g[1] + Ri[5] * g[2];
@@ -41,6 +46,14 @@
         a.y[3 * (size_t)p + 1] = o[1] * g[0] + o[3] * g[1] + o[4] * g[2];
         a.y[3 * (size_t)p + 2] = o[2] * g[0] + o[4] * g[1] + o[5] * g[2];
     }
+}
+
+template <int D>
+__device__ __forceinline__ void w_from_jac(const double Jc[2][D], const double Jp[2][3], double w[3 * D]) {
+#pragma unroll
+    for (int a = 0; a < D; ++a)
+#pragma unroll
+        for (int k = 0; k < 3; ++k) w[k * D + a] = Jc[0][a] * Jp[0][k] + Jc[1][a] * Jp[1][k];
 }
 
 template <int M>
@@ -70,10 +83,7 @@
     cv[5] = Jp[0][2] * Jp[0][2] + Jp[1][2] * Jp[1][2];
 #pragma unroll
     for (int k = 0; k < 3; ++k) cv[6 + k] = Jp[0][k] * r[0] + Jp[1][k] * r[1];
-#pragma unroll
-    for (int a = 0; a < D; ++a)
-#pragma unroll
-        for (int k = 0; k < 3; ++k) w[k * D + a] = Jc[0][a] * Jp[0][k] + Jc[1][a] * Jp[1][k];
+    w_from_jac<D>(Jc, Jp, w);
 }
 
 template <int D>
@@ -288,12 +298,17 @@
 #ifndef LIN_CAMS_NT
 #define LIN_CAMS_NT 128
 #endif
-template <int M, int NT = LIN_CAMS_NT>
+template <int M, bool SELF = false, int NT = LIN_CAMS_NT>
 __global__ __launch_bounds__(NT) void k_lin_cams_reg(const int* __restrict__ cam_ptr, const int* __restrict__ cm_pt,
                                                            const double* __restrict__ cm_uv, const double* __restrict__ pp,
                                                            const double* __restrict__ cams, const double* __restrict__ pts,
-                                                           double delta, double* __restrict__ U, double* __restrict__ gc) {
-    constexpr int D = kD<M>, ST = kStride<M>, NU = D * (D + 1) / 2, NE = NU + D;
+                                                           const double* __restrict__ Rinv, double delta,
+                                                           double* __restrict__ U, double* __restrict__ gc,
+                                                           double* __restrict__ Dself) {
+    constexpr bool CAMU = !SELF;
+    constexpr int D = kD<M>, ST = kStride<M>, NU = D * (D + 1) / 2;
+    constexpr int OS = CAMU ? NU + D : 0, NE = OS + (SELF ? NU : 0);
+    constexpr int NR = SELF ? 6 : 1;
     static_assert(D <= 9, "register accumulation is sized for D <= 9");
     constexpr int NW = NT / 64;
     __shared__ double red[NW][NE];
@@ -307,7 +322,7 @@
     double acc[NE];
 #pragma unroll
     for (int m = 0; m < NE; ++m) acc[m] = 0.0;
-    double X[3] = {0.0, 0.0, 0.0};
+    double X[3] = {0.0, 0.0, 0.0}, Ri[NR] = {};
     double2 z = make_double2(0.0, 0.0), zn = z, znn = z;
     int pn = 0, pnn = 0;
     {
@@ -316,13 +331,23 @@
             const int p0 = cm_pt[e0];
             z = uv2[e0];
             X[0] = pts[3 * (size_t)p0]; X[1] = pts[3 * (size_t)p0 + 1]; X[2] = pts[3 * (size_t)p0 + 2];
+            if constexpr (SELF) {
+#pragma unroll
+                for (int k = 0; k < 6; ++k) Ri[k] = Rinv[6 * (size_t)p0 + k];
+            }
         }
         if (e1 < ee) { pn = cm_pt[e1]; zn = uv2[e1]; }
     }
     for (int e = eb + t; e < ee; e += NT) {
         const bool hn = e + NT < ee, hnn = e + 2 * NT < ee;
-        double Xn[3] = {0.0, 0.0, 0.0};
-        if (hn) { Xn[0] = pts[3 * (size_t)pn]; Xn[1] = pts[3 * (size_t)pn + 1]; Xn[2] = pts[3 * (size_t)pn + 2]; }
+        double Xn[3] = {0.0, 0.0, 0.0}, Rin[NR] = {};
+        if (hn) {
+            Xn[0] = pts[3 * (size_t)pn]; Xn[1] = pts[3 * (size_t)pn + 1]; Xn[2] = pts[3 * (size_t)pn + 2];
+            if constexpr (SELF) {
+#pragma unroll
+                for (int k = 0; k < 6; ++k) Rin[k] = Rinv[6 * (size_t)pn + k];
+            }
+        }
         if (hnn) { pnn = cm_pt[e + 2 * NT]; znn = uv2[e + 2 * NT]; }
         const double uvo[2] = {z.x, z.y};
         double r[2], Jc[2][D], Jp[2][3];
@@ -330,15 +355,31 @@
         const double sw = huber_weight_sqrt(r[0] * r[0] + r[1] * r[1], delta);
 #pragma unroll
         for (int a = 0; a < D; ++a) { Jc[0][a] *= sw; Jc[1][a] *= sw; }
-        r[0] *= sw; r[1] *= sw;
-        int m = 0;
-#pragma unroll
-        for (int a = 0; a < D; ++a)
-#pragma unroll
-            for (int b = a; b < D; ++b, ++m) acc[m] += Jc[0][a] * Jc[0][b] + Jc[1][a] * Jc[1][b];
-#pragma unroll
-        for (int a = 0; a < D; ++a) acc[NU + a] -= Jc[0][a] * r[0] + Jc[1][a] * r[1];
+        if constexpr (SELF) {
+#pragma unroll
+            for (int k = 0; k < 3; ++k) { Jp[0][k] *= sw; Jp[1][k] *= sw; }
+            double w[3 * D];
+            w_from_jac<D>(Jc, Jp, w);
+            y_from_w<D>(w, Ri);
+            int m = OS;
+#pragma unroll
+            for (int a = 0; a < D; ++a)
+#pragma unroll
+                for (int b = a; b < D; ++b, ++m) acc[m] += w[a] * w[b] + w[D + a] * w[D + b] + w[2 * D + a] * w[2 * D + b];
+        }
+        if constexpr (CAMU) {
+            r[0] *= sw; r[1] *= sw;
+            int m = 0;
+#pragma unroll
+            for (int a = 0; a < D; ++a)
+#pragma unroll
+                for (int b = a; b < D; ++b, ++m) acc[m] += Jc[0][a] * Jc[0][b] + Jc[1][a] * Jc[1][b];
+#pragma unroll
+            for (int a = 0; a < D; ++a) acc[NU + a] -= Jc[0][a] * r[0] + Jc[1][a] * r[1];
+        }
         X[0] = Xn[0]; X[1] = Xn[1]; X[2] = Xn[2];
+#pragma unroll
+        for (int k = 0; k < NR; ++k) Ri[k] = Rin[k];
         z = zn; pn = pnn; zn = znn;
     }
 #pragma unroll
@@ -351,14 +392,15 @@
         double s = red[0][m];
 #pragma unroll
         for (int w = 1; w < NW; ++w) s += red[w][m];
-        if (m < NU) {
-            int a = 0, rem = m;
+        if (CAMU && m >= NU && m < NU + D) {
+            gc[(size_t)c * D + (m - NU)] = s;
+        } else {
+            double* out = m >= OS && SELF ? Dself : U;
+            int a = 0, rem = m >= OS ? m - OS : m;
             while (rem >= D - a) { rem -= D - a; ++a; }
             const int b = a + rem;
-            U[(size_t)c * D * D + a * D + b] = s;
-            U[(size_t)c * D * D + b * D + a] = s;
-        } else {
-            gc[(size_t)c * D + (m - NU)] = s;
+            out[(size_t)c * D * D + a * D + b] = s;
+            out[(size_t)c * D * D + b * D + a] = s;
         }
     }
 }
diff --git a/instantsfm_amd/csrc/ba_pcg.h b/instantsfm_amd/csrc/ba_pcg.h
--- a/instantsfm_amd/csrc/ba_pcg.h
+++ b/instantsfm_amd/csrc/ba_pcg.h
@@ -6,11 +6,12 @@
 
 namespace {
 
-template <int D>
+template <int D, bool SELF = false>
 __device__ __forceinline__ void factor_camera(int i, int lane, const int* __restrict__ row_ptr, double* __restrict__ S,
                                               double* __restrict__ b, double* __restrict__ Lf, double* __restrict__ Li,
                                               CgBufs& cg, const double* __restrict__ Ul, const double* __restrict__ gcl,
-                                              double f, double cmin, double cmax, double (&a)[D], double (&x)[D],
+                                              const double* __restrict__ Dsl, double f, double cmin, double cmax,
+                                              double (&a)[D], double (&x)[D],
                                               double& r0out, bool& okout) {
     constexpr int DD = D * D;
     const int rl = min(lane, D - 1);
@@ -25,6 +26,11 @@
             double u = Ui[c];
             if (c == rl) u = clampd(u, cmin, cmax) * f;
             a[c] += u;
+        }
+        if constexpr (SELF) {
+            const double* Di = Dsl + (size_t)i * DD + rl * D;
+#pragma unroll
+            for (int c = 0; c < D; ++c) a[c] -= Di[c];
         }
         bl = gcl[(size_t)i * D + rl] + bl;
         if (lane < D) {
@@ -85,28 +91,28 @@
     r0out = ok ? r0 : 0.0;
 }
 
-template <int D>
+template <int D, bool SELF = false>
 __global__ __launch_bounds__(kThreads) void k_cg_factor(int C, const int* __restrict__ row_ptr, double* __restrict__ S,
                                                         double* __restrict__ b, double* __restrict__ Lf,
                                                         double* __restrict__ Li, CgBufs cg, const double* __restrict__ Ul,
-                                                        const double* __restrict__ gcl, double f, double cmin, double cmax,
-                                                        long long* stp = nullptr) {
+                                                        const double* __restrict__ gcl, const double* __restrict__ Dsl,
+                                                        double f, double cmin, double cmax, long long* stp = nullptr) {
     const StampScope stamp_(stp);
     const int lane = threadIdx.x & 63, wv = threadIdx.x >> 6;
     const int i = blockIdx.x * kWaves + wv;
     if (i >= C) return;
     double a[D], x[D], r0;
     bool ok;
-    factor_camera<D>(i, lane, row_ptr, S, b, Lf, Li, cg, Ul, gcl, f, cmin, cmax, a, x, r0, ok);
-}
-
-template <int D>
+    factor_camera<D, SELF>(i, lane, row_ptr, S, b, Lf, Li, cg, Ul, gcl, Dsl, f, cmin, cmax, a, x, r0, ok);
+}
+
+template <int D, bool SELF = false>
 __global__ __launch_bounds__(kThreads) void k_cg_factor_basis(int C, const int* __restrict__ row_ptr, double* __restrict__ S,
                                                               double* __restrict__ b, double* __restrict__ Lf,
                                                               double* __restrict__ Li, CgBufs cg,
                                                               const double* __restrict__ Ul, const double* __restrict__ gcl,
-                                                              double f, double cmin, double cmax,
-                                                              const double* __restrict__ cams, TlBufs tl,
+                                                              const double* __restrict__ Dsl, double f, double cmin,
+                                                              double cmax, const double* __restrict__ cams, TlBufs tl,
                                                               double* __restrict__ runs, long long* stp = nullptr) {
     static_assert(kWaves == kCgpRows, "k_cg_factor_basis's workgroups are k_tl_cgp's");
     const StampScope stamp_(stp);
@@ -121,7 +127,7 @@
     if (has) {
         double a[D], x[D], r0;
         bool ok;
-        factor_camera<D>(i, lane, row_ptr, S, b, Lf, Li, cg, Ul, gcl, f, cmin, cmax, a, x, r0, ok);
+        factor_camera<D, SELF>(i, lane, row_ptr, S, b, Lf, Li, cg, Ul, gcl, Dsl, f, cmin, cmax, a, x, r0, ok);
         const int k = min(lane, MC - 1);
         double col[D];
         basis_column<D>(k, cams + (size_t)i * ST, tl.alone[i] != 0, col);
diff --git a/instantsfm_amd/csrc/ba_schur.h b/instantsfm_amd/csrc/ba_schur.h
--- a/instantsfm_amd/csrc/ba_schur.h
+++ b/instantsfm_amd/csrc/ba_schur.h
@@ -59,8 +59,8 @@
                                                       const int* __restrict__ cam, const double* __restrict__ W,
                                                       const double* __restrict__ Vinv, const double* __restrict__ y,
                                                       const double* __restrict__ U, const double* __restrict__ gc, double f,
-                                                      double cmin, double cmax, int add_diag, double* __restrict__ S,
-                                                      double* __restrict__ b, long long* stp) {
+                                                      double cmin, double cmax, int add_diag, int skip_self,
+                                                      double* __restrict__ S, double* __restrict__ b, long long* stp) {
     const StampScope stamp_(stp);
     constexpr int DD = D * D;
     constexpr int BS = schur_bs(D);
@@ -110,7 +110,7 @@
             const int en = e + WAVES * NG;
             if (active && en < oe) dnext = sdesc[en];
         }
-        const int qs = has ? dcur.z : 0, qe = has ? dcur.w : 0;
+        const int qs = has ? dcur.z + ((!GPW && !RETRY && !ORD) ? skip_self : 0) : 0, qe = has ? dcur.w : 0;
         const int n = qe - qs;
         double w0 = 0.0, w1 = 0.0, w2 = 0.0, v00 = 0.0, v01 = 0.0, v02 = 0.0, v11 = 0.0, v12 = 0.0, v22 = 0.0;
         if (has) {
diff --git a/instantsfm_amd/csrc/ba_solve.h b/instantsfm_amd/csrc/ba_solve.h
--- a/instantsfm_amd/csrc/ba_solve.h
+++ b/instantsfm_amd/csrc/ba_solve.h
@@ -72,6 +72,7 @@
     pp1.Vinv = h->Vinv;
     pp1.y = h->y;
     pp1.R = h->d.optimize_poses ? h->Rf : nullptr;
+    pp1.Ri = h->self_on ? h->Rinv : nullptr;
     pp1.flags = h->flags;
     pp1.status = h->cg.status;
     return pp1;
@@ -85,11 +86,15 @@
 }
 
 template <int M>
-void launch_lin_cams(insfm_ba* h, hipStream_t stream, const double* cams, const double* pts_local) {
+void launch_lin_cams(insfm_ba* h, hipStream_t stream, const double* cams, const double* pts_local, bool self = false) {
     constexpr int D = kD<M>;
     if constexpr (D <= 9) {
         k_lin_cams_reg<M><<<h->C, LIN_CAMS_NT, 0, stream>>>(h->cam_ptr, h->cm_pt, h->cm_uv, h->pp, cams, pts_local,
-                                                         h->d.huber_delta, h->U, h->gc);
+                                                         nullptr, h->d.huber_delta, h->U, h->gc, nullptr);
+        if (self)
+            k_lin_cams_reg<M, true><<<h->C, LIN_CAMS_NT, 0, stream>>>(h->cam_ptr, h->cm_pt, h->cm_uv, h->pp, cams,
+                                                                       pts_local, h->Rinv, h->d.huber_delta, nullptr,
+                                                                       nullptr, h->Dself);
     } else {
         const size_t lds = sizeof(double) * kThreads * (2 * D + 2);
         k_lin_cams<M><<<h->C, kThreads, lds, stream>>>(h->cam_ptr, h->cm_pt, h->cm_uv, h->pp, cams, pts_local,
@@ -116,6 +121,7 @@
     if (int rc0 = lin_join(h)) return rc0;
     const PointPrep pp1 = first_trial_prep(h);
     h->ss.prep_valid = false;
+    h->ss.dself_valid = false;
     if (h->kind == 0 && h->Pl > 0) {
         if (h->ss.flags_dirty) {
             if (int e = launch_zero_words(h)) return e;
@@ -133,8 +139,9 @@
         }
         HIPCHK(hipEventRecord(h->ev_lin0, h->stream));
         HIPCHK(hipStreamWaitEvent(h->aux, h->ev_lin0, 0));
-        launch_lin_cams<M>(h, h->aux, cams, pts_local);
+        launch_lin_cams<M>(h, h->aux, cams, pts_local, pp1.Ri != nullptr);
         if (int e = launch_err(h, "k_lin_cams")) return e;
+        h->ss.dself_valid = pp1.Ri != nullptr;
         HIPCHK(hipEventRecord(h->ev_lc, h->aux));
         h->ss.lin_pending = true;
         return launch_err(h, "k_lin_points");
@@ -354,7 +361,8 @@
     return k;
 }
 
-int launch_schur(insfm_ba* h, double sf, double smin, double smax, int sdiag, bool retry, int w0 = 0, int w1 = -1) {
+int launch_schur(insfm_ba* h, double sf, double smin, double smax, int sdiag, bool retry, bool skip_self = false,
+                 int w0 = 0, int w1 = -1) {
     const bool det = h->d.deterministic != 0, gpk = h->kind == 1;
     const double *Uin = gpk ? h->Up : h->U, *gcin = gpk ? h->gpc : h->gc;
     if (w1 < 0) w1 = h->nwork;
@@ -369,7 +377,7 @@
     if (!gpk && w1 <= w0) return 0;
     hipLaunchKernelGGL(kern, dim3(w1 - w0), dim3(nt), h->schur_lds, h->stream, h->work + w0, h->row_ptr, h->col, h->C,
                        h->cam_ptr, h->cam_obs, h->ptl, h->pt_ptr, h->ustart, h->sdesc, h->cam, h->W,
-                       gpk ? h->Vinv : h->Mp, h->y, Uin, gcin, sf, smin, smax, sdiag, h->S, h->b,
+                       gpk ? h->Vinv : h->Mp, h->y, Uin, gcin, sf, smin, smax, sdiag, skip_self ? 1 : 0, h->S, h->b,
                        gpk ? nullptr : stamp_ptr(h, kStSchur));
     return launch_err(h, "k_schur");
 }
@@ -640,20 +648,26 @@
 }
 
 template <int DV>
-void launch_factor(insfm_ba* h, double f, bool add_U, const double* basis_cams, bool first = false) {
+void launch_factor(insfm_ba* h, double f, bool add_U, const double* basis_cams, bool first = false, bool self = false) {
     const double *U = add_U ? h->U : nullptr, *gc = add_U ? h->gc : nullptr;
+    const double* Ds = add_U && self ? h->Dself : nullptr;
     const double cmin = first ? h->d.clamp_min : 0.0, cmax = first ? h->d.clamp_max : 0.0;
     long long* stamp = first ? stamp_ptr(h, kStFactor) : nullptr;
     if constexpr (DV != 3) {
         if (basis_cams) {
-            k_cg_factor_basis<DV><<<cdiv(h->C, kWaves), kThreads, 0, h->stream>>>(
-                h->C, h->row_ptr, h->S, h->b, h->Lf, h->Li, h->cg, U, gc, f, cmin, cmax, basis_cams, h->tl,
+            (Ds ? k_cg_factor_basis<DV, true> : k_cg_factor_basis<DV>)<<<cdiv(h->C, kWaves), kThreads, 0, h->stream>>>(
+                h->C, h->row_ptr, h->S, h->b, h->Lf, h->Li, h->cg, U, gc, Ds, f, cmin, cmax, basis_cams, h->tl,
                 h->cgp_runs + (size_t)h->cgp_grid * kCgpRows * 12, stamp);
             return;
         }
+        if (Ds) {
+            k_cg_factor<DV, true><<<cdiv(h->C, kWaves), kThreads, 0, h->stream>>>(
+                h->C, h->row_ptr, h->S, h->b, h->Lf, h->Li, h->cg, U, gc, Ds, f, cmin, cmax, stamp);
+            return;
+        }
     }
     k_cg_factor<DV><<<cdiv(h->C, kWaves), kThreads, 0, h->stream>>>(h->C, h->row_ptr, h->S, h->b, h->Lf, h->Li, h->cg, U,
-                                                                   gc, f, cmin, cmax, stamp);
+                                                                   gc, Ds, f, cmin, cmax, stamp);
 }
 
 int solve_tail(insfm_ba* h, double f, const double* cams, const double* pts_local, const double* dcp) {
@@ -715,6 +729,7 @@
     s.clamp_min = h->d.clamp_min; s.clamp_max = h->d.clamp_max;
     s.flags_dirty = h->ss.flags_dirty; s.prep_valid = h->ss.prep_valid; s.prep_f = h->ss.prep_f;
     s.tl_solves = h->ss.tl_solves; s.tl_fresh = h->ss.tl_fresh; s.async_status = async_status;
+    s.self_from_lin = h->self_on && h->ss.dself_valid;
     return s;
 }
 
@@ -743,7 +758,8 @@
         if (h->xstream) {
             const int K = (int)h->xw.size() - 1;
             for (int c = 0; c < K; ++c) {
-                if ((rc = launch_schur(h, p.sf, p.smin, p.smax, p.sdiag, !p.prepared, h->xw[c], h->xw[c + 1]))) return rc;
+                if ((rc = launch_schur(h, p.sf, p.smin, p.smax, p.sdiag, !p.prepared, false, h->xw[c], h->xw[c + 1])))
+                    return rc;
                 const int64_t b0 = h->rptr_host[h->xr[c]], b1 = h->rptr_host[h->xr[c + 1]];
                 HIPCHK(hipEventRecord(h->ev_x, h->stream));
                 HIPCHK(hipStreamWaitEvent(h->xstream, h->ev_x, 0));
@@ -756,7 +772,7 @@
             HIPCHK(hipStreamWaitEvent(h->stream, h->ev_xdone, 0));
             rec(h, kEvSchurEnd);
         } else {
-            if ((rc = launch_schur(h, p.sf, p.smin, p.smax, p.sdiag, !p.prepared))) return rc;
+            if ((rc = launch_schur(h, p.sf, p.smin, p.smax, p.sdiag, !p.prepared, p.self_from_lin))) return rc;
             hmark(h, "schur");
             rec(h, kEvSchurEnd);
             if ((rc = allreduce(h, h->S, (int64_t)h->nnzb * D * D + (int64_t)h->C * D))) return rc;
@@ -768,7 +784,7 @@
         if ((rc = lin_join(h))) return rc;
         rc = with_D(D, [&](auto dc_) -> int {
             constexpr int DV = decltype(dc_)::value;
-            launch_factor<DV>(h, f, p.add_U_in_factor, p.basis_by_factor ? cams : nullptr, true);
+            launch_factor<DV>(h, f, p.add_U_in_factor, p.basis_by_factor ? cams : nullptr, true, p.self_from_lin);
             if (p.scale) launch_scale<DV>(h);
             return launch_err(h, "k_cg_factor/scale");
         });
diff --git a/instantsfm_amd/csrc/create_plan.h b/instantsfm_amd/csrc/create_plan.h
--- a/instantsfm_amd/csrc/create_plan.h
+++ b/instantsfm_amd/csrc/create_plan.h
@@ -64,6 +64,14 @@
         }
     });
     return t;
+}
+
+template <class Cams>
+inline bool plan_distinct_track_cams(int Pl, const std::vector<int>& lptr, const Cams& lcam) {
+    for (int p = 0; p < Pl; ++p)
+        for (int o = lptr[p] + 1; o < lptr[p + 1]; ++o)
+            if (lcam[o] == lcam[o - 1]) return false;
+    return true;
 }
 
 struct CamMajor {
diff --git a/instantsfm_amd/csrc/solve_policy.h b/instantsfm_amd/csrc/solve_policy.h
--- a/instantsfm_amd/csrc/solve_policy.h
+++ b/instantsfm_amd/csrc/solve_policy.h
@@ -20,6 +20,7 @@
     long long tl_solves = 0;
     bool tl_fresh = false;
     bool async_status = false;
+    bool self_from_lin = false;
 };
 
 enum CgRun {
@@ -36,6 +37,7 @@
     double sf = 1.0, smin = 0.0, smax = 0.0;
     int sdiag = 0;
     bool add_U_in_factor = false;
+    bool self_from_lin = false;
     bool scale = true;
     bool basis_by_factor = false;
     CgRun cg = kCgNone;
@@ -54,6 +56,7 @@
     p.smax = gpk ? 1.0e308 : s.clamp_max;
     p.sdiag = gpk ? 1 : (s.u_late ? 0 : (s.rank0 ? 1 : 0));
     p.add_U_in_factor = s.u_late && !gpk;
+    p.self_from_lin = s.self_from_lin && p.prepared && p.add_U_in_factor;
     p.scale = !(s.tlon && s.cgp && s.tl_solves > 0 && s.tl_fresh && !s.keep_S);
     p.basis_by_factor = s.tlon && s.cgp && !gpk;
     if (!s.optimize_poses) p.cg = kCgNone;
diff --git a/instantsfm_amd/engine.py b/instantsfm_amd/engine.py
--- a/instantsfm_amd/engine.py
+++ b/instantsfm_amd/engine.py
@@ -290,6 +290,12 @@
     def debug_solve(self, f):
         return _capi.check(self._h, _capi.load().insfm_ba_debug_solve(self._h, float(f)))
 
+    def debug_self_diag(self):
+        return bool(_capi.check(self._h, _capi.load().insfm_ba_debug_self_diag(self._h)))
+
+    def debug_set_self_diag(self, on):
+        _capi.check(self._h, _capi.load().insfm_ba_debug_set_self_diag(self._h, int(bool(on))))
+
     def debug_time_kernel(self, which, reps=50):
         us = ctypes.c_double()
         _capi.check(self._h, _capi.load().insfm_ba_debug_time_kernel(self._h, int(which), int(reps), ctypes.byref(us)))
```

New measurement: 565.4. 25.2% lower.
